# mantasu/face-crop-plus

Measured on AMD Instinct MI355X. Metric: faces/sec end-to-end (detect+align+crop), higher is better.
Workload: dtype f16x3; 1 GPU; RetinaFace detect + 5-pt align/crop, batch=32/GPU synthetic 1024x1024 RGB, strategy=largest, det_threshold=0.6, output 256x256, detector on 2 HIP streams x 16 images; global_batch=32, image_size=1024, parallelism=dp1

## Files before the change

### face-crop-plus_amd/_native.py

```python
from __future__ import annotations

import ctypes as C
import os

_HERE = os.path.dirname(os.path.abspath(__file__))
LIB_PATH = os.path.join(_HERE, "csrc", "libfcp_hip.so")
ABI_VERSION = 15

c_f32p = C.c_void_p
_lib = None


class ConvDesc(C.Structure):
    _fields_ = [
        ("in_", C.c_void_p), ("w", C.c_void_p), ("bias", C.c_void_p), ("out", C.c_void_p),
        ("res1", C.c_void_p), ("res2", C.c_void_p), ("wscale", C.c_void_p), ("in2", C.c_void_p),
        ("n", C.c_int32), ("in_h", C.c_int32), ("in_w", C.c_int32),
        ("cin", C.c_int32), ("in_ld", C.c_int32), ("in_up2", C.c_int32),
        ("cout", C.c_int32), ("kh", C.c_int32), ("kw", C.c_int32),
        ("stride", C.c_int32), ("pad", C.c_int32),
        ("out_h", C.c_int32), ("out_w", C.c_int32), ("out_ld", C.c_int32),
        ("tile_n", C.c_int32), ("cin4", C.c_int32),
        ("act_slope", C.c_float), ("alpha", C.c_float), ("alpha2", C.c_float),
        ("res1_pre", C.c_int32), ("res1_ld", C.c_int32), ("res1_h", C.c_int32),
        ("res1_w", C.c_int32), ("res2_ld", C.c_int32), ("precision", C.c_int32),
        ("in_fmt", C.c_int32), ("out_fmt", C.c_int32), ("res1_fmt", C.c_int32), ("res2_fmt", C.c_int32),
        ("tile_m", C.c_int32), ("cin2", C.c_int32), ("in2_ld", C.c_int32), ("in2_h", C.c_int32),
        ("in2_w", C.c_int32), ("in2_stride", C.c_int32), ("flags", C.c_int32), ("cu_budget", C.c_int32),
        ("band_top", C.c_int32), ("band_bottom", C.c_int32),
    ]


CONV_FLAT_ADDR = 1
CONV_BALANCE_TAIL = 2
CHAIN_OUT_EVEN_ONLY = 1


class ChainDesc(C.Structure):
    _fields_ = [(k, C.c_void_p) for k in ("t1", "w2", "ws2", "b2", "w3", "ws3", "b3", "res", "out", "w1n", "ws1n",
                                          "b1n", "t1n", "t1b")] + \
               [(k, C.c_int32) for k in ("n", "h", "w", "c", "cn", "t1_ld", "res_ld", "out_ld", "t1n_ld", "nout", "tile_m", "flags",
                                         "cb", "t1b_ld", "t1b_h", "t1b_w", "t1b_stride")]


_P, _I, _F, _L = C.c_void_p, C.c_int, C.c_float, C.c_int64
SIGNATURES = {
    "fcp_conv2d_nhwc_f32": [C.POINTER(ConvDesc), _P],
    "fcp_bottleneck_chain_f16x3": [C.POINTER(ChainDesc), _P],
    "fcp_u8_to_nhwc4_f32": [_P, _P, _L, C.POINTER(C.c_float), _F, _P],
    "fcp_f32nchw_to_nhwc4_f32": [_P, _P, _I, _I, _I, C.POINTER(C.c_float), _F, _P],
    "fcp_maxpool3x3s2_nhwc_f32": [_P, _P, _I, _I, _I, _I, _I, _I, _I, _P],
    "fcp_maxpool3x3s2_split32": [_P, _P, _I, _I, _I, _I, _I, _I, _I, _P],
    "fcp_stem7x7s2_relu_pool_u8": [_P, _I, _I, _I, C.POINTER(C.c_int32), _P, _P, _P, _P, _I, _I, _P],
    "fcp_stem7x7s2_relu_pool_conv1_u8": [_P, _I, _I, _I, C.POINTER(C.c_int32), _P, _P, _P, _P, _I, _I, _P, _P, _P, _P, _I, _P],
    "fcp_stem7x7s2_relu_pool_f32": [_P, _I, _I, _I, _P, _P, _P, _P, _I, _I, _P],
    "fcp_f32_to_split32": [_P, _P, _L, _I, _P],
    "fcp_split32_to_f32": [_P, _P, _L, _I, _P],
    "fcp_absmax_nhwc": [_P, _L, _I, _I, _I, _P, _P],
    "fcp_retina_decode": [_P, _P, _P, _I, _I, _I, _F, _F, _F, _P, _P, _P, _P, _P, _P, _P, _P, _P],
    "fcp_retina_nms_select": [_P, _P, _P, _I, _I, _F, _I, _P, _P, _P, _P, _P, _P],
    "fcp_retina_gather_faces": [_P, _P, _P, _I, _I, _P, _I, _P, _P, _P, _P],
    "fcp_estimate_transform": [_P, _P, _I, _I, _I, _P, _P, _P],
    "fcp_estimate_transform_counted": [_P, _P, _I, _I, _I, _P, _P, _P, _P, _P],
    "fcp_bise_preprocess_u8": [_P, _I, _I, _I, _P, _I, _I, C.POINTER(C.c_float), C.POINTER(C.c_float), _P],
    "fcp_avgpool_nhwc_f32": [_P, _I, _I, _I, _I, _P, _P],
    "fcp_fc_f32": [_P, _P, _P, _P, _I, _I, _I, _I, _P, _P],
    "fcp_scale_add_nhwc_f32": [_P, _I, _P, _P, _P, _I, _I, _I, _I, _P, _I, _P],
    "fcp_parse_tail": [_P, _I, _I, _I, _I, _I, _I, _I, _I, _I, _P, _P, _P],
    "fcp_label_mask_u8": [_P, _L, C.c_uint32, _P, _P],
    "fcp_bicubic_down4_u8": [_P, _I, _I, _I, _P, _P],
    "fcp_warp_affine_u8": [_P, _I, _I, _I, _P, _P, _P, _P, _I, _I, _I, _I, _P, _P],
    "fcp_warp_affine_u8_float": [_P, _I, _I, _I, _P, _P, _P, _P, _I, _I, _I, _I, _P, _P],
    "fcp_build_batch_u8": [_P, _L, _P, _P, _I, _I, _I, _I, _P, _P],
    "fcp_warp_affine_u8_ragged": [_P, _L, _P, _P, _P, _P, _I, _I, _I, _I, _P, _P],
    "fcp_warp_affine_u8_float_ragged": [_P, _L, _P, _P, _P, _P, _I, _I, _I, _I, _P, _P],
    "fcp_resize_area_ragged_u8": [_P, _L, _P, _P, _I, _P, _L, _P],
    "fcp_warp_affine_u8_interp": [_P, _I, _I, _I, _P, _P, _P, _P, _I, _I, _I, _I, _I, _P, _P],
    "fcp_warp_affine_u8_interp_ragged": [_P, _L, _P, _P, _P, _P, _I, _I, _I, _I, _I, _P, _P],
    "fcp_warp_interp_weights": [_I, _P],
    "fcp_crop_sharpness_u8": [_P, _I, _I, _I, _P, _P, _P],
    "fcp_jpeg_encode_u8": [_P, _I, _I, _I, _I, _I, _I, _P, _L, _L, _P, _P, _L, _P],
    "fcp_jpeg_encode_ex_u8": [_P, _I, _I, _I, _I, _I, _I, _I, _P, _L, _L, _P, _P, _P, _L, _P],
    "fcp_jpeg_huffman_tables": [_P, _I, _P, _P, _P],
    "fcp_png_encode_u8": [_P, _I, _I, _I, _I, _P, _L, _L, _P, _P, _L, _P],
    "fcp_png_huffman_lengths": [_P, _I, _P, _P, _P],
    "fcp_matte_u8": [_P, _P, _I, _I, _I, C.c_uint32, _I, _I, _I, _I, _P, _P, _P],
    "fcp_clahe_u8": [_P, _I, _I, _I, _I, C.c_double, _P, _P, _P],
    "fcp_matte_blur_u8": [_P, _P, _I, _I, _I, C.c_uint32, _I, _P, _I, _P, _P, _P, _L, _P],
    "fcp_matte_refine_u8": [_P, _P, _I, _I, _I, C.c_uint32, _I, _I, _P, _P, _L, _P],
    "fcp_matte_alpha_u8": [_P, _P, _I, _I, _I, _I, _I, _I, _P, _P],
    "fcp_matte_blur_alpha_u8": [_P, _P, _P, _I, _I, _I, C.c_uint32, _P, _I, _P, _P, _L, _P],
    "fcp_subject_mask_u8": [_P, _I, _I, _I, C.c_uint32, _I, _I, _P, _P, _L, _P],
    "fcp_feather_alpha_u8": [_P, _I, _I, _I, C.c_uint32, _I, _P, _P],
    "fcp_cutout_u8": [_P, _P, _I, _I, _I, _I, _I, _I, _I, _P, _I, _P, _P, _L, _P],
    "fcp_mask_shift_u8": [_P, _I, _I, _I, C.c_uint32, _I, _P, _P],
    "fcp_nlm_denoise_u8": [_P, _I, _I, _I, _P, _I, _I, _P, _P],
    "fcp_unsharp_u8": [_P, _I, _I, _I, _P, _I, _I, _I, _P, _P],
    "fcp_matte_image_u8": [_P, _P, _I, _I, _I, C.c_uint32, _I, _P, _I, _P, _P, _P, _P],
    "fcp_matte_image_alpha_u8": [_P, _P, _I, _I, _I, _P, _I, _P, _P, _P],
    "fcp_cutout_image_u8": [_P, _P, _I, _I, _I, _P, _I, _P, _P, _I, _P, _P, _L, _P],
}
EXPORTS = ["fcp_abi_version", "fcp_last_error", "fcp_retina_nms_workspace_bytes", "fcp_jpeg_workspace_bytes",
           "fcp_jpeg_workspace_bytes_ex", "fcp_matte_blur_workspace_bytes", "fcp_matte_refine_workspace_bytes",
           "fcp_subject_mask_workspace_bytes", "fcp_png_workspace_bytes", "fcp_cutout_workspace_bytes"] + list(SIGNATURES)


def lib():
    global _lib
    if _lib is not None:
        return _lib
    if not os.path.isfile(LIB_PATH):
        raise RuntimeError(
            f"HIP extension not built: {LIB_PATH} is missing. Run "
            f"`python face-crop-plus_amd/build_native.py` (needs hipcc). There is no CPU fallback.")
    l = C.CDLL(LIB_PATH)
    l.fcp_abi_version.restype = C.c_int
    l.fcp_last_error.restype = C.c_char_p
    if l.fcp_abi_version() != ABI_VERSION:
        raise RuntimeError(f"libfcp_hip.so ABI {l.fcp_abi_version()} != expected {ABI_VERSION}; rebuild")
    l.fcp_retina_nms_workspace_bytes.argtypes = [C.c_int, C.c_int]
    l.fcp_retina_nms_workspace_bytes.restype = C.c_int64
    l.fcp_jpeg_workspace_bytes.argtypes = [C.c_int, C.c_int, C.c_int, C.c_int]
    l.fcp_jpeg_workspace_bytes.restype = C.c_int64
    l.fcp_jpeg_workspace_bytes_ex.argtypes = [C.c_int] * 6
    l.fcp_jpeg_workspace_bytes_ex.restype = C.c_int64
    l.fcp_png_workspace_bytes.argtypes = [C.c_int, C.c_int, C.c_int, C.c_int]
    l.fcp_png_workspace_bytes.restype = C.c_int64
    l.fcp_matte_blur_workspace_bytes.argtypes = [C.c_int, C.c_int, C.c_int]
    l.fcp_matte_blur_workspace_bytes.restype = C.c_int64
    l.fcp_matte_refine_workspace_bytes.argtypes = [C.c_int, C.c_int, C.c_int]
    l.fcp_matte_refine_workspace_bytes.restype = C.c_int64
    l.fcp_subject_mask_workspace_bytes.argtypes = [C.c_int, C.c_int, C.c_int]
    l.fcp_subject_mask_workspace_bytes.restype = C.c_int64
    l.fcp_cutout_workspace_bytes.argtypes = [C.c_int, C.c_int, C.c_int]
    l.fcp_cutout_workspace_bytes.restype = C.c_int64
    for name, args in SIGNATURES.items():
        fn = getattr(l, name)
        fn.argtypes = args
        fn.restype = C.c_int
    _lib = l
    return l


def check(rc: int, what: str = ""):
    if rc != 0:
        msg = lib().fcp_last_error().decode(errors="replace")
        raise RuntimeError(f"{what or 'fcp_hip'} failed ({rc}): {msg}")


def stream_ptr():
    import torch
    return C.c_void_p(torch.cuda.current_stream().cuda_stream)


def ptr(t, byte_offset: int = 0):
    if t is None:
        return C.c_void_p(0)
    return C.c_void_p(t.data_ptr() + byte_offset)


def encode_slots(who: str, entry: str, pixels_dev, out, op, workspace_bytes, call):
    import torch
    assert pixels_dev.dtype == torch.uint8 and pixels_dev.is_contiguous() and pixels_dev.dim() in (3, 4)
    assert out.dtype == torch.uint8 and out.dim() == 2 and out.shape[0] == pixels_dev.shape[0]
    if op is not None:
        return op()
    f, h, w = pixels_dev.shape[:3]
    c = pixels_dev.shape[3] if pixels_dev.dim() == 4 else 1
    capacity = out.shape[1]
    if capacity and out.stride(1) != 1:
        raise RuntimeError(f"{who}: the bytes of a row of out must be contiguous")
    lengths = torch.empty((f,), dtype=torch.int32, device=pixels_dev.device)
    need = workspace_bytes(f, h, w, c)
    check(-1 if need < 0 else 0, entry)
    work = torch.empty((need,), dtype=torch.uint8, device=pixels_dev.device)
    check(call((f, h, w, c), (ptr(out) if capacity else None, out.stride(0) if f > 1 else capacity, capacity, ptr(lengths)),
               (ptr(work), need, stream_ptr())), entry)
    return lengths
```

### face-crop-plus_amd/csrc/fcp_conv.hip

```cpp
#include "fcp_conv_common.h"

#include <cstdlib>

using namespace fcp_conv;

namespace {

constexpr int LDK = 32;


template <int BN, bool CIN4, bool BUF>
__global__ void __launch_bounds__(256, (BN == 128 ? 2 : (BN == 64 ? 3 : 4))) conv_igemm_f32(const ConvK p) {
  constexpr int WAVES_N = (BN == 32) ? 1 : 2;
  constexpr int WAVES_M = 4 / WAVES_N;
  constexpr int WTM = BM / WAVES_M;
  constexpr int WTN = BN / WAVES_N;
  constexpr int TM = WTM / 32, TN = WTN / 32;
  constexpr int A_LD = BM / 32;
  constexpr int B_LD = BN / 32;

  extern __shared__ __attribute__((aligned(16))) float smem[];
  float* As = smem;
  float* Bs = smem + 2 * BM * LDK;

  const int logical = xcd_tile_order(gridDim.x, blockIdx.x);
  const int tile_n = logical % p.grid_n;
  const int tile_m = logical / p.grid_n;

  const int tid = threadIdx.x;
  const int lane = tid & 63;
  const int wave = tid >> 6;
  const int wm = wave / WAVES_N, wn = wave % WAVES_N;
  const int chunk = tid & 7;
  const int lrow = tid >> 3;

  long nbase[A_LD];
  RowPiece pc[A_LD];
  const int hw = p.out_h * p.out_w;
#pragma unroll
  for (int i = 0; i < A_LD; ++i) {
    const ConvRow r = conv_row(p, tile_m * BM + lrow + 32 * i, p.M, hw, 0u);
    nbase[i] = (long)r.ni * p.ph * p.pw;
    pc[i] = make_row_piece<CIN4>(p, r, chunk, (unsigned)(chunk * 4));
  }
  const float* wbase = p.w + (long)(tile_n * BN + lrow) * p.wrow + chunk * 4;

  __amdgpu_buffer_rsrc_t rs_in, rs_w;
  unsigned rowoff[A_LD];
  unsigned woff[B_LD];
  if (BUF) {
    rs_in = __builtin_amdgcn_make_buffer_rsrc(const_cast<float*>(p.in), 0, p.in_bytes, 0x00020000);
    rs_w = __builtin_amdgcn_make_buffer_rsrc(const_cast<float*>(p.w), 0, p.w_bytes, 0x00020000);
#pragma unroll
    for (int i = 0; i < B_LD; ++i)
      woff[i] = (unsigned)(((tile_n * BN + lrow + 32 * i) * p.wrow + chunk * 4) * 4);
  }

  f32x4 ra0[A_LD], rb0[B_LD], ra1[A_LD], rb1[B_LD];

  auto load_slice = [&](f32x4 (&ra)[A_LD], f32x4 (&rb)[B_LD], int kt, int kh_i, int kw_i, int c0) {
    if (BUF) {
#pragma unroll
      for (int i = 0; i < A_LD; ++i) {
        const unsigned vo = rowoff[i] == 0xFFFFFFFFu ? 0xFFFFFFFFu : rowoff[i] + (unsigned)(c0 * 4);
        ra[i] = buf_load16(rs_in, vo);
      }
#pragma unroll
      for (int i = 0; i < B_LD; ++i) rb[i] = buf_load16(rs_w, woff[i] + (unsigned)(kt * BK * 4));
    } else {
#pragma unroll
      for (int i = 0; i < A_LD; ++i) {
        int hi = pc[i].hi0 + kh_i;
        int wi = pc[i].wi0 + (CIN4 ? chunk : kw_i);
        const bool ok = (unsigned)hi < (unsigned)p.in_h && (unsigned)wi < (unsigned)p.in_w;
        if (p.in_up2) { hi >>= 1; wi >>= 1; }
        const long pix = nbase[i] + (long)hi * p.pw + wi;
        const float* src = CIN4 ? p.in + pix * p.in_ld : p.in + pix * p.in_ld + c0 + chunk * 4;
        ra[i] = ok ? *reinterpret_cast<const f32x4*>(src) : f32x4{0.f, 0.f, 0.f, 0.f};
      }
#pragma unroll
      for (int i = 0; i < B_LD; ++i)
        rb[i] = *reinterpret_cast<const f32x4*>(wbase + (long)(32 * i) * p.wrow + kt * BK);
    }
  };
  const int schunk = chunk ^ ((lrow >> 1) & 7);
  auto store_slice = [&](const f32x4 (&ra)[A_LD], const f32x4 (&rb)[B_LD], int buf) {
    float* a = As + buf * BM * LDK + lrow * LDK + schunk * 4;
    float* b = Bs + buf * BN * LDK + lrow * LDK + schunk * 4;
#pragma unroll
    for (int i = 0; i < A_LD; ++i) *reinterpret_cast<f32x4*>(a + 32 * i * LDK) = ra[i];
#pragma unroll
    for (int i = 0; i < B_LD; ++i) *reinterpret_cast<f32x4*>(b + 32 * i * LDK) = rb[i];
  };

  f32x16 acc[TM][TN];
  clear_acc(acc);

  TapWalk tw;
  auto advance = [&]() {
    if (BUF) next_tap<CIN4, true>(p, tw, pc, rowoff);
    else tw.advance<CIN4>(p);
  };

  const int aoff = (wm * WTM + (lane & 31)) * LDK;
  const int boff = (wn * WTN + (lane & 31)) * LDK;
  const int rsw = ((lane & 31) >> 1) & 7;
  int koff[4];
#pragma unroll
  for (int pp = 0; pp < 4; ++pp) koff[pp] = (((2 * pp + (lane >> 5)) ^ rsw)) * 4;

  auto compute = [&](int buf) {
    const float* Ab = As + buf * BM * LDK + aoff;
    const float* Bb = Bs + buf * BN * LDK + boff;
#pragma unroll
    for (int pp = 0; pp < 4; ++pp) {
      f32x4 a[TM], b[TN];
#pragma unroll
      for (int i = 0; i < TM; ++i) a[i] = *reinterpret_cast<const f32x4*>(Ab + (i * 32 * LDK + koff[pp]));
#pragma unroll
      for (int j = 0; j < TN; ++j) b[j] = *reinterpret_cast<const f32x4*>(Bb + (j * 32 * LDK + koff[pp]));
#pragma unroll
      for (int e = 0; e < 4; ++e)
#pragma unroll
        for (int i = 0; i < TM; ++i)
#pragma unroll
          for (int j = 0; j < TN; ++j)
            acc[i][j] = __builtin_amdgcn_mfma_f32_32x32x2f32(a[i][e], b[j][e], acc[i][j], 0, 0, 0);
    }
  };
  auto step = [&](int kt, f32x4 (&ra_ld)[A_LD], f32x4 (&rb_ld)[B_LD], const f32x4 (&ra_st)[A_LD],
                  const f32x4 (&rb_st)[B_LD]) {
    if (kt + 2 < p.ktiles) {
      advance();
      load_slice(ra_ld, rb_ld, kt + 2, tw.kh_i, tw.kw_i, tw.c0);
    }
    compute(kt & 1);
    if (kt + 1 < p.ktiles) store_slice(ra_st, rb_st, (kt + 1) & 1);
    __syncthreads();
  };

  if (BUF) set_tap<CIN4, true>(p, tw, pc, rowoff);
  load_slice(ra0, rb0, 0, tw.kh_i, tw.kw_i, tw.c0);
  store_slice(ra0, rb0, 0);
  if (p.ktiles > 1) {
    advance();
    load_slice(ra1, rb1, 1, tw.kh_i, tw.kw_i, tw.c0);
  }
  __syncthreads();
  for (int kt = 0; kt < p.ktiles; kt += 2) {
    step(kt, ra0, rb0, ra1, rb1);
    if (kt + 1 < p.ktiles) step(kt + 1, ra1, rb1, ra0, rb0);
  }

  conv_epilogue<BN, TM, TN, WTM, WTN>(p, acc, smem, tile_m, tile_n, tid, lane, wm, wn, hw);
}

template <int BN, bool CIN4, bool BUF>
int launch(const ConvK& k, hipStream_t s) {
  const size_t lds = (size_t)2 * (BM + BN) * LDK * sizeof(float);
  FCP_LDS_OPT_IN((&conv_igemm_f32<BN, CIN4, BUF>), lds);
  const int blocks = k.grid_m * k.grid_n;
  hipLaunchKernelGGL((conv_igemm_f32<BN, CIN4, BUF>), dim3(blocks), dim3(256), lds, s, k);
  FCP_LAUNCH_OK();
  return 0;
}

}

extern "C" int fcp_conv2d_nhwc_f32(const fcp_conv_desc* d, fcp_stream_t stream) {
  FCP_REQUIRE(d != nullptr, "conv: null descriptor");
  FCP_REQUIRE(d->in && d->w && d->out, "conv: null tensor pointer");
  FCP_REQUIRE(d->n > 0 && d->in_h > 0 && d->in_w > 0 && d->cout > 0, "conv: bad sizes");
  const bool big = d->tile_m == 256, halo = d->tile_m == 1;
  FCP_REQUIRE(d->tile_m == 0 || d->tile_m == 128 || big || halo, "conv: tile_m must be 0/128/256 (or 1: halo-tile 3x3)");
  const bool halo_wide = halo && d->tile_n != 32;
  if (halo)
    FCP_REQUIRE(d->precision == 1 && d->in_fmt == 1 && !d->cin4 && d->kh == 3 && d->kw == 3 && d->stride == 1 &&
                d->pad == 1 && d->cout <= 64 && d->cout % 8 == 0 && d->cin >= 64 && !d->in2 &&
                (!d->res1 || (d->res1_h == d->out_h && d->res1_w == d->out_w)) || halo_wide,
                "conv: the halo-tile kernel needs a 3x3 / stride 1 / pad 1 conv with cin >= 64, cout <= 64 (cout %% 8 == 0) on the "
                "fp16x3 path with a split32 input, no second source, no resized residual");
  if (halo_wide)
    FCP_REQUIRE(d->precision == 1 && d->in_fmt == 1 && !d->cin4 && d->kh == 3 && d->kw == 3 && d->stride == 1 &&
                d->pad == 1 && d->cout % 8 == 0 && d->cin >= 64 && d->cin % 64 == 0 && !d->in2 &&
                ((d->tile_n == 64 && d->cout <= 64 && (!d->res1 || (d->res1_h == d->out_h && d->res1_w == d->out_w))) ||
                 (d->tile_n == 128 && d->cout <= 128 && !d->res1 && !d->res2)),
                "conv: the wide halo-tile kernel (tile_m 1, tile_n 64 / 128) needs a 3x3 / stride 1 / pad 1 conv with cin %% 64 == 0, "
                "cout <= tile_n (cout %% 8 == 0; no residuals above 64 filters) on the fp16x3 path with a split32 input");
  FCP_REQUIRE(d->tile_n == 32 || d->tile_n == 64 || d->tile_n == 128 || (big && (d->tile_n == 256 || d->tile_n == 192)),
              "conv: tile_n must be 32/64/128 (or 192 / 256 with tile_m 256)");
  if (big)
    FCP_REQUIRE(d->precision == 1 && d->in_fmt == 1 && !d->cin4 && !d->in_up2 && d->cout % 8 == 0 && d->tile_n >= 128,
                "conv: 256-row tiles need the fp16x3 path on a split32 input (no cin4 / in_up2), cout %% 8 == 0, tile_n 128/256");
  FCP_REQUIRE(d->kh >= 1 && d->kw >= 1 && d->stride >= 1 && d->pad >= 0, "conv: bad filter geometry");
  FCP_REQUIRE(d->kh * d->kw <= 32 || d->cin4, "conv: at most 32 filter taps (kh*kw) outside cin4 mode");
  FCP_REQUIRE(d->in_ld % 4 == 0 && ((uintptr_t)d->in & 15) == 0, "conv: input must be 16-byte aligned, in_ld %% 4 == 0");
  FCP_REQUIRE(((uintptr_t)d->w & 15) == 0, "conv: filter must be 16-byte aligned");
  if (d->cin4) {
    FCP_REQUIRE(d->cin <= 4 && d->in_ld == 4 && d->kw <= 8, "conv: cin4 mode needs cin<=4, in_ld==4, kw<=8");
  } else {
    FCP_REQUIRE(d->cin % 32 == 0 && d->cin > 0, "conv: cin must be a multiple of 32 (got %d)", d->cin);
  }
  FCP_REQUIRE(d->band_top >= 0 && d->band_bottom >= 0 && d->band_top <= d->pad && d->band_bottom <= d->pad &&
              ((d->band_top | d->band_bottom) == 0 || (d->stride == 1 && !d->in2)),
              "conv: band_top / band_bottom must lie in 0..pad (stride-1 convs without a second source only)");
  const int eh = (d->in_h - d->band_top - d->band_bottom + 2 * d->pad - d->kh) / d->stride + 1;
  const int ew = (d->in_w + 2 * d->pad - d->kw) / d->stride + 1;
  FCP_REQUIRE(eh == d->out_h && ew == d->out_w, "conv: output size %dx%d does not match geometry %dx%d",
              d->out_h, d->out_w, eh, ew);
  if (d->in_up2) FCP_REQUIRE(d->in_h % 2 == 0 && d->in_w % 2 == 0, "conv: in_up2 needs even logical size");
  const long M = (long)d->n * d->out_h * d->out_w;
  FCP_REQUIRE(M < (1L << 31), "conv: too many output pixels");

  ConvK k;
  k.in = d->in; k.w = reinterpret_cast<const float*>(d->w); k.bias = d->bias; k.wscale = d->wscale; k.out = d->out; k.res1 = d->res1; k.res2 = d->res2;
  k.n = d->n; k.in_h = d->in_h; k.in_w = d->in_w;
  k.ph = d->in_up2 ? d->in_h / 2 : d->in_h;
  k.pw = d->in_up2 ? d->in_w / 2 : d->in_w;
  k.cin = d->cin; k.in_ld = d->in_ld; k.in_up2 = d->in_up2;
  k.cout = d->cout; k.kh = d->kh; k.kw = d->kw; k.stride = d->stride; k.pad = d->pad; k.pad_h = d->pad - d->band_top;
  k.out_h = d->out_h; k.out_w = d->out_w; k.out_ld = d->out_ld;
  k.M = (int)M;
  if (d->cin4) {
    k.ktiles = d->kh; k.ctiles = 1; k.wrow = d->kh * 32;
  } else {
    k.ctiles = d->cin / 32; k.ktiles = d->kh * d->kw * k.ctiles; k.wrow = d->kh * d->kw * d->cin;
  }
  k.act_slope = d->act_slope; k.alpha = d->alpha; k.alpha2 = d->alpha2;
  k.res1_pre = d->res1_pre; k.res1_ld = d->res1_ld; k.res2_ld = d->res2_ld;
  k.res1_h = d->res1_h; k.res1_w = d->res1_w;
  k.res1_resize = 0; k.res1_sh = 1.f; k.res1_sw = 1.f;
  k.in_fmt = d->in_fmt; k.out_fmt = d->out_fmt; k.res1_fmt = d->res1 ? d->res1_fmt : 0; k.res2_fmt = d->res2 ? d->res2_fmt : 0;
  const int any_split = k.in_fmt | k.out_fmt | k.res1_fmt | k.res2_fmt;
  FCP_REQUIRE((unsigned)any_split <= 1u, "conv: tensor formats must be 0 (fp32) or 1 (split32)");
  if (any_split) {
    FCP_REQUIRE(d->precision == 1, "conv: split32 tensors need precision 1 (fp16x3 kernel)");
    FCP_REQUIRE(d->cout % 8 == 0, "conv: split32 epilogue needs cout %% 8 == 0");
    FCP_REQUIRE(!k.in_fmt || (!d->cin4 && d->in_ld % 32 == 0 && ((uintptr_t)d->in & 127) == 0),
                "conv: split32 input must be a 32-channel-group aligned view (in_ld %% 32 == 0), not cin4");
    FCP_REQUIRE(!k.out_fmt || (d->out_ld % 32 == 0 && ((uintptr_t)d->out & 127) == 0 && d->cout % 32 == 0),
                "conv: split32 output must be a 32-channel-group aligned view with cout %% 32 == 0");
    FCP_REQUIRE(!k.res1_fmt || (d->res1_ld % 32 == 0 && ((uintptr_t)d->res1 & 127) == 0), "conv: misaligned split32 res1");
    FCP_REQUIRE(!k.res2_fmt || (d->res2_ld % 32 == 0 && ((uintptr_t)d->res2 & 127) == 0), "conv: misaligned split32 res2");
    FCP_REQUIRE(((uintptr_t)d->out & 15) == 0 && d->out_ld % 4 == 0 && (!d->res1 || (((uintptr_t)d->res1 & 15) == 0 && d->res1_ld % 4 == 0)) &&
                (!d->res2 || (((uintptr_t)d->res2 & 15) == 0 && d->res2_ld % 4 == 0)), "conv: 8-channel epilogue needs 16-byte aligned tensors");
  }
  if (d->res1) {
    FCP_REQUIRE(d->res1_h > 0 && d->res1_w > 0 && d->res1_ld > 0, "conv: res1 geometry missing");
    if (d->res1_h != d->out_h || d->res1_w != d->out_w) {
      k.res1_resize = 1;
      k.res1_sh = (float)d->res1_h / (float)d->out_h;
      k.res1_sw = (float)d->res1_w / (float)d->out_w;
    }
  }
  if (d->res2) FCP_REQUIRE(d->res2_ld > 0, "conv: res2_ld missing");
  k.vec_ok = (d->out_ld % 4 == 0) && (((uintptr_t)d->out & 15) == 0);
  if (d->res1) k.vec_ok = k.vec_ok && (d->res1_ld % 4 == 0) && (((uintptr_t)d->res1 & 15) == 0);
  if (d->res2) k.vec_ok = k.vec_ok && (d->res2_ld % 4 == 0) && (((uintptr_t)d->res2 & 15) == 0);
  static const int nt_env = getenv("FCP_NT_STORE") ? atoi(getenv("FCP_NT_STORE")) : 1;
  k.nt_store = nt_env;
  k.balance = (d->flags & FCP_CONV_BALANCE_TAIL) ? 1 : 0;
  k.cu_budget = d->cu_budget;
  k.mfull = 0; k.tail_rows = 0; k.round_size = 0;
  k.in2 = nullptr; k.in2_bytes = 0; k.csplit = d->cin; k.in2_ld = 0; k.ph2 = 0; k.pw2 = 0; k.stride2 = 1;
  if (d->in2) {
    FCP_REQUIRE(d->precision == 1 && d->in_fmt == 1 && !d->cin4 && !d->in_up2 && d->kh == 1 && d->kw == 1 && d->pad == 0,
                "conv: a second source needs a 1x1 / pad 0 conv on the fp16x3 path with split32 inputs");
    FCP_REQUIRE(d->cin2 > 0 && d->cin2 < d->cin && d->cin2 % 32 == 0 && d->in2_ld % 32 == 0 && d->in2_ld >= d->cin2 &&
                ((uintptr_t)d->in2 & 127) == 0, "conv: in2 must be a 32-channel-group aligned split32 view, 0 < cin2 < cin");
    FCP_REQUIRE(d->in2_stride >= 1 && d->in2_h > 0 && d->in2_w > 0 && (long)(d->out_h - 1) * d->in2_stride < d->in2_h &&
                (long)(d->out_w - 1) * d->in2_stride < d->in2_w, "conv: in2 geometry does not cover the output grid");
    const unsigned long in2_bytes = (unsigned long)d->n * d->in2_h * d->in2_w * d->in2_ld * 4ul;
    FCP_REQUIRE(in2_bytes < 0xFFFFFFF0ul, "conv: in2 must be below 4 GiB");
    k.in2 = d->in2; k.in2_bytes = (unsigned)in2_bytes; k.csplit = d->cin - d->cin2; k.in2_ld = d->in2_ld;
    k.ph2 = d->in2_h; k.pw2 = d->in2_w; k.stride2 = d->in2_stride;
  }
  k.grid_m = fcp_cdiv(M, BM);
  k.grid_n = fcp_cdiv(d->cout, d->tile_n);
  hipStream_t s = (hipStream_t)stream;
  const unsigned long in_bytes = (unsigned long)d->n * k.ph * k.pw * d->in_ld * 4ul;
  const unsigned long w_bytes = (unsigned long)(k.grid_n * d->tile_n) * k.wrow * 4ul;
  FCP_REQUIRE(!(d->flags & FCP_CONV_FLAT_ADDR) || d->precision == 0, "conv: FCP_CONV_FLAT_ADDR is a precision-0 (fp32 kernel) option");
  const bool buf = in_bytes < 0xFFFFFFF0ul && w_bytes < 0xFFFFFFF0ul && !(d->flags & FCP_CONV_FLAT_ADDR);
  FCP_REQUIRE(d->precision == 0 || d->precision == 1, "conv: precision must be 0 (fp32) or 1 (fp16x3)");
  if (d->precision == 1) {
    FCP_REQUIRE(buf, "conv: the fp16x3 path needs tensors below 4 GiB (pack this layer with precision 0)");
    FCP_REQUIRE(d->wscale != nullptr, "conv: precision 1 needs wscale");
    k.in_bytes = (unsigned)in_bytes;
    k.w_bytes = (unsigned)w_bytes;
    if (halo) {
      k.grid_n = 1;
      const unsigned long out_bytes = (unsigned long)M * d->out_ld * 4ul;
      FCP_REQUIRE(out_bytes < 0xFFFFFFF0ul, "conv(halo): the output view must span less than 4 GiB");
      FCP_REQUIRE(d->wscale != nullptr && ((uintptr_t)d->wscale & 15) == 0 && ((uintptr_t)d->bias & 15) == 0,
                  "conv(halo): wscale / bias must be 16-byte aligned");
      k.in2_bytes = (unsigned)out_bytes;
      k.w_bytes = (unsigned)((unsigned long)fcp_cdiv(d->cout, 128) * 128ul * k.wrow * 4ul);
      return halo_wide ? launch_f16x3_halo_wide(k, s) : launch_f16x3_halo(k, s);
    }
    if (big) {
      k.w_bytes = (unsigned)((unsigned long)fcp_cdiv(d->cout, 128) * 128ul * k.wrow * 4ul);
      return launch_f16x3_big(k, d->tile_n, s);
    }
    if (k.in_fmt == 1 && !d->cin4) return launch_f16x3_dma(k, d->tile_n, s);
    return launch_f16x3(k, d->tile_n, d->cin4 != 0, s);
  }
  k.in_bytes = buf ? (unsigned)in_bytes : 0u;
  k.w_bytes = buf ? (unsigned)w_bytes : 0u;
#define FCP_DISPATCH(BN_)                                                             \
  do {                                                                                \
    if (d->cin4) return buf ? launch<BN_, true, true>(k, s) : launch<BN_, true, false>(k, s); \
    return buf ? launch<BN_, false, true>(k, s) : launch<BN_, false, false>(k, s);   \
  } while (0)
  switch (d->tile_n) {
    case 32: FCP_DISPATCH(32);
    case 64: FCP_DISPATCH(64);
    default: FCP_DISPATCH(128);
  }
#undef FCP_DISPATCH
}
```

### face-crop-plus_amd/csrc/fcp_conv_common.h

```cpp
#pragma once
#include <type_traits>
#include "fcp_common.h"
#include "fcp_hip.h"

typedef float f32x16 __attribute__((ext_vector_type(16)));
typedef float f32x4 __attribute__((ext_vector_type(4)));


constexpr int FCP_AUX_A = 0;
constexpr int FCP_AUX_B = 0;

namespace fcp_conv {

constexpr int BM = 128;
constexpr int BK = 32;

struct ConvK {
  const float* in;
  const float* w;
  const float* bias;
  float* out;
  const float* res1;
  const float* res2;
  int n, in_h, in_w, ph, pw, cin, in_ld, in_up2;
// ... 264 lines not shown
    float* dst = base + pix * ld + c;
    *reinterpret_cast<u32x4_t*>(dst) = a;
    *reinterpret_cast<u32x4_t*>(dst + 4) = b;
  }
}
__device__ __forceinline__ void pack_store8(float* base, long pix, int ld, int c, int fmt, int nt, const float (&v)[8]) {
  u32x4_t a, b;
  if (fmt == 1) {
    pack8(v, 1, a, b);
    store8(base, pix, ld, c, 1, nt, a, b);
  } else {
    pack8(v, 0, a, b);
    store8(base, pix, ld, c, 0, 0, a, b);
  }
}

__device__ __forceinline__ float conv_scale_bias(float acc, float ws, float b) { return acc * ws + b; }

struct ConvEpi {
  bool res1, res1_pre, res2;
  float act_slope, alpha, alpha2;
};
template <typename E>
__device__ __forceinline__ float conv_finish(const E e, float x, float r1, float r2) {
  if (e.res1 && e.res1_pre) x += r1;
  x = x >= 0.f ? x : x * e.act_slope;
  x = x * e.alpha;
  if (e.res1 && !e.res1_pre) x += r1;
  if (e.res2) x = x * e.alpha2 + r2;
  return x;
}
template <typename E>
__device__ __forceinline__ float conv_value(const E& e, float acc, float ws, float b, float r1, float r2) {
  return conv_finish(e, conv_scale_bias(acc, ws, b), r1, r2);
}
__device__ __forceinline__ float conv_finish_relu(float x) { return conv_finish(ConvEpi{false, false, false, 0.f, 1.f, 1.f}, x, 0.f, 0.f); }
__device__ __forceinline__ float conv_finish_relu(float x, float r1) { return conv_finish(ConvEpi{true, true, false, 0.f, 1.f, 1.f}, x, r1, 0.f); }
__device__ __forceinline__ float conv_value_relu(float acc, float ws, float b) { return conv_finish_relu(conv_scale_bias(acc, ws, b)); }

__device__ __forceinline__ long res1_pixel(const ConvK& p, long m, int hw) {
  int ni, ho, wo;
  conv_out_pixel(p, m, hw, ni, ho, wo);
  int sh = (int)floorf(ho * p.res1_sh);
  int sw = (int)floorf(wo * p.res1_sw);
  sh = sh < p.res1_h - 1 ? sh : p.res1_h - 1;
  sw = sw < p.res1_w - 1 ? sw : p.res1_w - 1;
  return ((long)ni * p.res1_h + sh) * p.res1_w + sw;
}

__device__ __forceinline__ constexpr int mfma_c_row(int rr, int half) { return (rr & 3) + 8 * (rr >> 2) + 4 * half; }

template <int BN, int TM, int TN, int WTM, int WTN>
__device__ __forceinline__ void stage_acc_tile(const f32x16 (&acc)[TM][TN], float* Cs, int lane, int wm, int wn) {
  const int half = lane >> 5;
#pragma unroll
  for (int i = 0; i < TM; ++i)
#pragma unroll
    for (int j = 0; j < TN; ++j)
#pragma unroll
      for (int rr = 0; rr < 16; ++rr) {
        const int row = wm * WTM + i * 32 + mfma_c_row(rr, half);
        Cs[row * BN + wn * WTN + j * 32 + (lane & 31)] = acc[i][j][rr];
      }
  __syncthreads();
}

template <int BN, int TM, int TN, int WTM, int WTN>
__device__ __forceinline__ void conv_epilogue(const ConvK& p, f32x16 (&acc)[TM][TN], float* smem, int tile_m,
                                              int tile_n, int tid, int lane, int wm, int wn, int hw) {
  constexpr int CPR = BN / 4;
  constexpr int RPP = 256 / CPR;
  constexpr int PASSES = BM / RPP;
  float* Cs = smem;
  const int ccol = (tid % CPR) * 4;
  const int crow = tid / CPR;
  const int co = tile_n * BN + ccol;
  const bool vec = p.vec_ok && (co + 3 < p.cout);
  const long m0 = (long)tile_m * BM + crow;

  const bool pre1 = p.res1 != nullptr && !p.res1_resize && vec;
  const bool pre2 = p.res2 != nullptr && vec;
  stage_acc_tile<BN, TM, TN, WTM, WTN>(acc, Cs, lane, wm, wn);

  f32x4 bias4 = {0.f, 0.f, 0.f, 0.f}, ws4 = {1.f, 1.f, 1.f, 1.f};
  if (p.bias != nullptr) {
#pragma unroll
    for (int e = 0; e < 4; ++e)
      if (co + e < p.cout) bias4[e] = p.bias[co + e];
  }
  if (p.wscale != nullptr) {
#pragma unroll
    for (int e = 0; e < 4; ++e)
      if (co + e < p.cout) ws4[e] = p.wscale[co + e];
  }
  constexpr int EPC = PASSES < 4 ? PASSES : 4;
#pragma unroll 1
  for (int g = 0; g < PASSES; g += EPC) {
    f32x4 r1v[EPC], r2v[EPC];
    if (pre1) {
#pragma unroll
      for (int i = 0; i < EPC; ++i) {
        const long m = m0 + (long)(g + i) * RPP;
        r1v[i] = m < p.M ? *reinterpret_cast<const f32x4*>(p.res1 + m * p.res1_ld + co) : f32x4{0.f, 0.f, 0.f, 0.f};
      }
    }
    if (pre2) {
#pragma unroll
      for (int i = 0; i < EPC; ++i) {
        const long m = m0 + (long)(g + i) * RPP;
        r2v[i] = m < p.M ? *reinterpret_cast<const f32x4*>(p.res2 + m * p.res2_ld + co) : f32x4{0.f, 0.f, 0.f, 0.f};
      }
    }
#pragma unroll
    for (int i = 0; i < EPC; ++i) {
      const int row = crow + (g + i) * RPP;
      const long m = m0 + (long)(g + i) * RPP;
      if (m >= p.M || co >= p.cout) continue;
      f32x4 v = *reinterpret_cast<const f32x4*>(Cs + row * BN + ccol);
      f32x4 r1 = {0.f, 0.f, 0.f, 0.f}, r2 = {0.f, 0.f, 0.f, 0.f};
      if (pre1) {
        r1 = r1v[i];
      } else if (p.res1 != nullptr) {
        const long roff = (p.res1_resize ? res1_pixel(p, m, hw) : m) * p.res1_ld + co;
        if (vec) {
          r1 = *reinterpret_cast<const f32x4*>(p.res1 + roff);
        } else {
#pragma unroll
          for (int e = 0; e < 4; ++e)
            if (co + e < p.cout) r1[e] = p.res1[roff + e];
        }
      }
      if (pre2) {
        r2 = r2v[i];
      } else if (p.res2 != nullptr) {
#pragma unroll
        for (int e = 0; e < 4; ++e)
          if (co + e < p.cout) r2[e] = p.res2[m * p.res2_ld + co + e];
      }
#pragma unroll
      for (int e = 0; e < 4; ++e) v[e] = conv_value(p, v[e], ws4[e], bias4[e], r1[e], r2[e]);
      float* dst = p.out + m * p.out_ld + co;
      if (vec) {
        *reinterpret_cast<f32x4*>(dst) = v;
      } else {
#pragma unroll
        for (int e = 0; e < 4; ++e)
          if (co + e < p.cout) dst[e] = v[e];
      }
    }
  }
}


template <int I, int N, typename F>
__device__ __forceinline__ void fcp_static_for(F&& f) {
  if constexpr (I < N) {
    f(std::integral_constant<int, I>{});
    fcp_static_for<I + 1, N>(f);
  }
}

template <int TM, int TN, int WTM, int WTN>
__device__ __forceinline__ void conv_epilogue_regs(const ConvK& p, f32x16 (&acc)[TM][TN], int m_start, int m_end, int tm_act, int co_tile,
                                                   int co_end, int wm, int wn, int lane, int hw) {
    const int lp = lane & 15, lg = lane >> 4;
  auto swap32 = [](float& x, float& y) {
    const auto r = __builtin_amdgcn_permlane32_swap(__float_as_uint(x), __float_as_uint(y), false, false);
    const unsigned r0 = r[0], r1 = r[1];
    x = __uint_as_float(r0); y = __uint_as_float(r1);
  };
  auto swap16 = [](float& x, float& y) {
    const auto r = __builtin_amdgcn_permlane16_swap(__float_as_uint(x), __float_as_uint(y), false, false);
    const unsigned r0 = r[0], r1 = r[1];
    x = __uint_as_float(r0); y = __uint_as_float(r1);
  };
  constexpr int GI = TM < 2 ? TM : 2;
  constexpr int NGI = (TM + GI - 1) / GI;
  constexpr int NG = TN * NGI;
  u32x4_t pend_a[GI][2], pend_b[GI][2];
  auto row_of = [&](int i, int set) { return m_start + wm * WTM + i * 32 + 16 * set + lp; };
  auto chan_of = [&](int jj) { return co_tile + wn * WTN + jj * 32 + 8 * lg; };
  auto flush = [&](auto gc) {
    constexpr int g = decltype(gc)::value, jj = g / NGI, i0 = (g % NGI) * GI;
    const int co = chan_of(jj);
    fcp_static_for<0, GI>([&](auto ic) {
      constexpr int i = i0 + decltype(ic)::value;
      if constexpr (i < TM) {
        fcp_static_for<0, 2>([&](auto sc) {
          constexpr int set = decltype(sc)::value;
          const int mi = row_of(i, set);
          if (i < tm_act && mi < m_end && co < co_end) store8(p.out, mi, p.out_ld, co, p.out_fmt, 0, pend_a[i - i0][set], pend_b[i - i0][set]);
        });
      }
    });
  };
  fcp_static_for<0, NG>([&](auto gc) {
    constexpr int g = decltype(gc)::value, j = g / NGI, i0 = (g % NGI) * GI;
    const int co = chan_of(j);
    const bool cok = co < co_end;
    const int cc = cok ? co : co_tile;
    u32x4_t r1a[GI][2], r1b[GI][2];
    if (p.res1 != nullptr) {
      fcp_static_for<0, GI>([&](auto ic) {
        constexpr int i = i0 + decltype(ic)::value;
        if constexpr (i < TM) {
          fcp_static_for<0, 2>([&](auto sc) {
            constexpr int set = decltype(sc)::value;
            const int mi = row_of(i, set);
            const long m = (i < tm_act && mi < m_end && cok) ? (long)mi : (long)m_start;
            const long rpix = p.res1_resize ? res1_pixel(p, m, hw) : m;
            if (p.res1_fmt == 1) {
              const char* pb = reinterpret_cast<const char*>(p.res1) + rpix * p.res1_ld * 4 + split_chan_off(cc);
              r1a[i - i0][set] = *reinterpret_cast<const u32x4_t*>(pb);
              r1b[i - i0][set] = *reinterpret_cast<const u32x4_t*>(pb + 64);
            } else {
              r1a[i - i0][set] = *reinterpret_cast<const u32x4_t*>(p.res1 + rpix * p.res1_ld + cc);
              r1b[i - i0][set] = *reinterpret_cast<const u32x4_t*>(p.res1 + rpix * p.res1_ld + cc + 4);
            }
          });
        }
      });
    }
    __builtin_amdgcn_sched_barrier(0);
    if constexpr (g > 0) flush(std::integral_constant<int, g - 1>{});
    __builtin_amdgcn_sched_barrier(0);
    float bias8[8], ws8[8];
    {
      const f32x4 w0 = *reinterpret_cast<const f32x4*>(p.wscale + cc), w1 = *reinterpret_cast<const f32x4*>(p.wscale + cc + 4);
      f32x4 b0 = {0.f, 0.f, 0.f, 0.f}, b1 = b0;
      if (p.bias != nullptr) { b0 = *reinterpret_cast<const f32x4*>(p.bias + cc); b1 = *reinterpret_cast<const f32x4*>(p.bias + cc + 4); }
#pragma unroll
      for (int e = 0; e < 4; ++e) { ws8[e] = w0[e]; ws8[4 + e] = w1[e]; bias8[e] = b0[e]; bias8[4 + e] = b1[e]; }
    }
    fcp_static_for<0, GI>([&](auto ic) {
      constexpr int i = i0 + decltype(ic)::value;
      if constexpr (i < TM) {
        float va[8], vb[8];
        fcp_static_for<0, 4>([&](auto ec) {
          constexpr int e = decltype(ec)::value;
          float q0 = acc[i][j][e], q1 = acc[i][j][4 + e], q2 = acc[i][j][8 + e], q3 = acc[i][j][12 + e];
          swap32(q0, q1);
          swap32(q2, q3);
          swap32(q0, q2); swap16(q0, q2);
          swap32(q1, q3); swap16(q1, q3);
          va[e] = q0; va[4 + e] = q1; vb[e] = q2; vb[4 + e] = q3;
        });
        fcp_static_for<0, 2>([&](auto sc) {
          constexpr int set = decltype(sc)::value;
          float (&v)[8] = set == 0 ? va : vb;
          float r1[8], r2[8];
          if (p.res1 != nullptr) {
            if (p.res1_fmt == 1) {
              join8(r1a[i - i0][set], r1b[i - i0][set], r1);
            } else {
              const f32x4 fa = __builtin_bit_cast(f32x4, r1a[i - i0][set]), fb = __builtin_bit_cast(f32x4, r1b[i - i0][set]);
              r1[0] = fa[0]; r1[1] = fa[1]; r1[2] = fa[2]; r1[3] = fa[3]; r1[4] = fb[0]; r1[5] = fb[1]; r1[6] = fb[2]; r1[7] = fb[3];
            }
          }
          if (p.res2 != nullptr) {
            const int mi = row_of(i, set);
            load8(p.res2, (i < tm_act && mi < m_end && cok) ? (long)mi : (long)m_start, p.res2_ld, cc, p.res2_fmt, r2);
          }
#pragma unroll
          for (int e = 0; e < 8; ++e) v[e] = conv_value(p, v[e], ws8[e], bias8[e], r1[e], r2[e]);
          pack8(v, p.out_fmt, pend_a[i - i0][set], pend_b[i - i0][set]);
        });
      }
    });
  });
  flush(std::integral_constant<int, NG - 1>{});
}

template <int BN, int TM, int TN, int WTM, int WTN>
__device__ __forceinline__ void conv_epilogue8(const ConvK& p, f32x16 (&acc)[TM][TN], float* smem, int tile_m,
                                               int tile_n, int tid, int lane, int wm, int wn, int hw) {
  constexpr int CPR = BN / 8;
  constexpr int RPP = 256 / CPR;
  constexpr int PASSES = BM / RPP;
  float* Cs = smem;
  const int ccol = (tid % CPR) * 8;
  const int crow = tid / CPR;
  const int co = tile_n * BN + ccol;
  const long m0 = (long)tile_m * BM + crow;
  stage_acc_tile<BN, TM, TN, WTM, WTN>(acc, Cs, lane, wm, wn);
  if (co >= p.cout) return;
  float bias8[8], ws8[8];
#pragma unroll
  for (int e = 0; e < 8; ++e) {
    bias8[e] = p.bias != nullptr ? p.bias[co + e] : 0.f;
    ws8[e] = p.wscale != nullptr ? p.wscale[co + e] : 1.f;
  }
#pragma unroll
  for (int g = 0; g < PASSES; ++g) {
    const int row = crow + g * RPP;
    const long m = m0 + (long)g * RPP;
    if (m >= p.M) continue;
    float v[8], r1[8], r2[8];
    {
      const f32x4 a = *reinterpret_cast<const f32x4*>(Cs + row * BN + ccol);
      const f32x4 b = *reinterpret_cast<const f32x4*>(Cs + row * BN + ccol + 4);
      v[0] = a[0]; v[1] = a[1]; v[2] = a[2]; v[3] = a[3]; v[4] = b[0]; v[5] = b[1]; v[6] = b[2]; v[7] = b[3];
    }
    if (p.res1 != nullptr) load8(p.res1, p.res1_resize ? res1_pixel(p, m, hw) : m, p.res1_ld, co, p.res1_fmt, r1);
    if (p.res2 != nullptr) load8(p.res2, m, p.res2_ld, co, p.res2_fmt, r2);
#pragma unroll
    for (int e = 0; e < 8; ++e) v[e] = conv_value(p, v[e], ws8[e], bias8[e], r1[e], r2[e]);
    pack_store8(p.out, m, p.out_ld, co, p.out_fmt, p.nt_store, v);
  }
}

int launch_f16x3(const ConvK& k, int tile_n, bool cin4, hipStream_t s);
int launch_f16x3_dma(const ConvK& k, int tile_n, hipStream_t s);
int launch_f16x3_halo(const ConvK& k, hipStream_t s);
int launch_f16x3_halo_wide(const ConvK& k, hipStream_t s);
int launch_f16x3_big(const ConvK& k, int tile_n, hipStream_t s);

}
```

### face-crop-plus_amd/csrc/fcp_conv_f16x3_big.hip

```cpp
#include "fcp_conv_common.h"

#include <type_traits>

using namespace fcp_conv;

namespace {

constexpr int BMB = 256;
constexpr int NT = 512;
constexpr int ROWB = 128;
constexpr int STAGE = 1 << 16;

template <int BN>
__global__ void __launch_bounds__(NT, 1) conv_igemm_f16x3_big(const ConvK p) {
  constexpr int WAVES_N = BN == 256 ? 4 : 2;
  constexpr int WAVES_M = 8 / WAVES_N;
  constexpr int WTM = BMB / WAVES_M, WTN = BN / WAVES_N;
  constexpr int TM = WTM / 32, TN = WTN / 32;
  constexpr int A_LD = BMB / 64, B_LD = BN / 64;

  extern __shared__ __attribute__((aligned(16))) float smem[];
  char* lds = reinterpret_cast<char*>(smem);

  const int nb = p.big_tiles;
  int vb = blockIdx.x;
  int tile_n = 0, m_start = 0, m_end = 0;
  auto decode = [&](int bid) {
    const int rbase = (bid / p.round_size) * p.round_size;
    const int nr = nb - rbase < p.round_size ? nb - rbase : p.round_size;
    const int bi = bid - rbase;
    const int logical = rbase + xcd_tile_order(nr, bi);
    tile_n = logical % p.grid_n;
    const int tile_m = logical / p.grid_n;
    m_start = tile_m < p.mfull ? tile_m * BMB : p.mfull * BMB + (tile_m - p.mfull) * p.tail_rows;
    const int m_rows = tile_m < p.mfull ? BMB : p.tail_rows;
    m_end = m_start + m_rows < p.M ? m_start + m_rows : p.M;
  };
  decode(vb);

  const int tid = threadIdx.x;
  const int lane = tid & 63;
  const int wave_u = __builtin_amdgcn_readfirstlane(tid >> 6);
  const int wm = wave_u / WAVES_N, wn = wave_u % WAVES_N;
  const int lrow = tid >> 3;
  const int csrc = (tid & 7) ^ (((lrow >> 1) & 7) ^ ((lrow & 1) << 2));

  const int hw = p.out_h * p.out_w;
  RowPiece pc[A_LD];
  unsigned base2[A_LD];
  unsigned rowoff[A_LD], woff[B_LD];
  auto setup_tile = [&]() {
#pragma unroll
    for (int i = 0; i < A_LD; ++i) {
      const int m = m_start + lrow + 64 * i;
      unsigned pbase = 0;
      int hi0 = -(1 << 28), wi0 = 0;
      base2[i] = 0xFFFFFFFFu;
      if (m < m_end) {
        int ni, ho, wo;
        conv_out_pixel(p, m, hw, ni, ho, wo);
        pbase = (unsigned)(ni * p.ph * p.pw);
        hi0 = ho * p.stride - p.pad_h;
        wi0 = wo * p.stride - p.pad;
        if (p.in2 != nullptr)
          base2[i] = (((unsigned)(ni * p.ph2 + ho * p.stride2) * (unsigned)p.pw2 + (unsigned)(wo * p.stride2)) * (unsigned)p.in2_ld +
                      (unsigned)(csrc * 4)) * 4u;
      }
      pc[i].tp = make_tap_piece<false>(p, pbase, hi0, wi0, (unsigned)(csrc * 4));
    }
#pragma unroll
    for (int i = 0; i < B_LD; ++i) woff[i] = (unsigned)(((tile_n * BN + lrow + 64 * i) * p.wrow + csrc * 4) * 4);
  };
  setup_tile();
  __amdgpu_buffer_rsrc_t rs_in2 = __builtin_amdgcn_make_buffer_rsrc(const_cast<float*>(p.in2 ? p.in2 : p.in), 0, p.in2_bytes, 0x00020000);
  __amdgpu_buffer_rsrc_t rs_in = __builtin_amdgcn_make_buffer_rsrc(const_cast<float*>(p.in), 0, p.in_bytes, 0x00020000);
  __amdgpu_buffer_rsrc_t rs_w = __builtin_amdgcn_make_buffer_rsrc(const_cast<float*>(p.w), 0, p.w_bytes, 0x00020000);
  TapWalk tw;
  auto advance = [&]() { next_tap<false, false>(p, tw, pc, rowoff); };
  auto dma = [&](int kt, int stage) {
    char* a = lds + stage * STAGE + wave_u * 8 * ROWB;
    dma_slice<64>(p, rs_in, rs_in2, rs_w, a, a + BMB * ROWB, rowoff, base2, woff, tw.c0, kt);
  };

  f32x16 acc[TM][TN];

  const unsigned lds0 = (unsigned)(size_t)(__attribute__((address_space(3))) char*)lds;
  int offH[2], offL[2];
  frag_offsets(lane, offH, offL);
  const unsigned arow = lds0 + (unsigned)((wm * WTM + (lane & 31)) * ROWB);
  const unsigned brow = lds0 + (unsigned)((BMB + wn * WTN + (lane & 31)) * ROWB);
  unsigned aH[2], aL[2], bH[2], bL[2];
#pragma unroll
  for (int s = 0; s < 2; ++s) {
    aH[s] = arow + (unsigned)offH[s]; aL[s] = arow + (unsigned)offL[s];
    bH[s] = brow + (unsigned)offH[s]; bL[s] = brow + (unsigned)offL[s];
  }

  auto prefetch_tile = [&]() {
    tw = TapWalk();
    set_tap<false, false>(p, tw, pc, rowoff);
    dma(0, 0);
    if (p.ktiles > 1) {
      advance();
      dma(1, 1);
    }
  };
  prefetch_tile();
  int tm_act = 0;
  auto main_loop = [&](auto tma_c) {
    constexpr int TMA = decltype(tma_c)::value;
    f16x8 fah[2][TMA > 0 ? TMA : 1], fal[2][TMA > 0 ? TMA : 1], fbh[2][TN], fbl[2][TN];
  auto read_frags = [&](auto set_c, unsigned stage_xor) {
    constexpr int set = decltype(set_c)::value;
    fcp_static_for<0, TMA>([&](auto ic) {
      constexpr int i = decltype(ic)::value;
      fah[set][i] = lds_read128i<i * 32 * ROWB>(aH[set] ^ stage_xor);
      fal[set][i] = lds_read128i<i * 32 * ROWB>(aL[set] ^ stage_xor);
    });
    fcp_static_for<0, TN>([&](auto jc) {
      constexpr int j = decltype(jc)::value;
      fbh[set][j] = lds_read128i<j * 32 * ROWB>(bH[set] ^ stage_xor);
      fbl[set][j] = lds_read128i<j * 32 * ROWB>(bL[set] ^ stage_xor);
    });
  };
  constexpr std::integral_constant<int, 0> SET0{};
  constexpr std::integral_constant<int, 1> SET1{};
  auto mfmas_reads = [&](auto cs_c, auto ls_c, unsigned stage_xor) {
    constexpr int cs = decltype(cs_c)::value, ls = decltype(ls_c)::value;
    constexpr int NM = 3 * TMA * TN, NR = 2 * TMA + 2 * TN;
    fcp_static_for<0, NM>([&](auto mc) {
      constexpr int m = decltype(mc)::value;
      constexpr int g = m / (TMA * TN), i = (m % (TMA * TN)) / TN, j = m % TN;
      if constexpr (g == 0) acc[i][j] = __builtin_amdgcn_mfma_f32_32x32x16_f16(fbh[cs][j], fal[cs][i], acc[i][j], 0, 0, 0);
      else if constexpr (g == 1) acc[i][j] = __builtin_amdgcn_mfma_f32_32x32x16_f16(fbl[cs][j], fah[cs][i], acc[i][j], 0, 0, 0);
      else acc[i][j] = __builtin_amdgcn_mfma_f32_32x32x16_f16(fbh[cs][j], fah[cs][i], acc[i][j], 0, 0, 0);
      __builtin_amdgcn_sched_barrier(0);
      fcp_static_for<0, NR>([&](auto rc) {
        constexpr int r = decltype(rc)::value;
        if constexpr (((r + 1) * NM) / NR - 1 == m
        ) {
          if constexpr (r < 2 * TMA) {
            constexpr int ii = r / 2;
            if constexpr (r % 2 == 0) fah[ls][ii] = lds_read128i<ii * 32 * ROWB>(aH[ls] ^ stage_xor);
            else fal[ls][ii] = lds_read128i<ii * 32 * ROWB>(aL[ls] ^ stage_xor);
          } else {
            constexpr int jj = (r - 2 * TMA) / 2;
            if constexpr (r % 2 == 0) fbh[ls][jj] = lds_read128i<jj * 32 * ROWB>(bH[ls] ^ stage_xor);
            else fbl[ls][jj] = lds_read128i<jj * 32 * ROWB>(bL[ls] ^ stage_xor);
          }
          __builtin_amdgcn_sched_barrier(0);
        }
      });
    });
  };

  read_frags(SET0, 0u);
  asm volatile("s_waitcnt lgkmcnt(0)" ::: "memory");
  __builtin_amdgcn_sched_barrier(0);

  unsigned sx = 0u;
  for (int kt = 0; kt < p.ktiles; ++kt) {
    mfmas_reads(SET0, SET1, sx);
    __builtin_amdgcn_sched_barrier(0);
    asm volatile("s_waitcnt lgkmcnt(0)" ::: "memory");
    asm volatile("s_waitcnt vmcnt(0)" ::: "memory");
    __builtin_amdgcn_s_barrier();
    __builtin_amdgcn_sched_barrier(0);
    const bool dma_first = wave_u >= 4;
    if (dma_first && kt + 2 < p.ktiles) {
      advance();
      dma(kt + 2, kt & 1);
    }
    __builtin_amdgcn_sched_barrier(0);
    mfmas_reads(SET1, SET0, sx ^ (unsigned)STAGE);
    __builtin_amdgcn_sched_barrier(0);
    if (!dma_first && kt + 2 < p.ktiles) {
      advance();
      dma(kt + 2, kt & 1);
    }
    __builtin_amdgcn_sched_barrier(0);
    asm volatile("s_waitcnt lgkmcnt(0)" ::: "memory");
    __builtin_amdgcn_sched_barrier(0);
    sx ^= (unsigned)STAGE;
  }
  };
  for (;;) {
  asm volatile("s_waitcnt vmcnt(0)" ::: "memory");
  __builtin_amdgcn_s_barrier();
  __builtin_amdgcn_sched_barrier(0);
  tm_act = (m_end - m_start - wm * WTM + 31) >> 5;
  tm_act = __builtin_amdgcn_readfirstlane(tm_act < 0 ? 0 : (tm_act > TM ? TM : tm_act));
  clear_acc(acc);
  fcp_static_for<0, TM + 1>([&](auto tc) {
    if (tm_act == decltype(tc)::value) main_loop(tc);
  });
  asm volatile("s_waitcnt vmcnt(0)" ::: "memory");
  __builtin_amdgcn_s_barrier();

  const int e_tile_n = tile_n, e_m_start = m_start, e_m_end = m_end, e_tm_act = tm_act;
  const bool more = p.big_persist && vb + p.round_size < nb;
  if (more) {
    vb += p.round_size;
    decode(vb);
    setup_tile();
    prefetch_tile();
  }
  conv_epilogue_regs<TM, TN, WTM, WTN>(p, acc, e_m_start, e_m_end, e_tm_act, e_tile_n * BN,
                                       (e_tile_n + 1) * BN < p.cout ? (e_tile_n + 1) * BN : p.cout, wm, wn, lane, hw);
  if (!more) break;
  }
}

template <int BN>
int launch(ConvK k, hipStream_t s) {
  const size_t lds = 2 * (size_t)STAGE;
  FCP_LDS_OPT_IN((&conv_igemm_f16x3_big<BN>), lds);
  k.grid_n = fcp_cdiv(k.cout, BN);
  int cus = k.cu_budget > 0 ? k.cu_budget : fcp_cu_count();
  cus = cus < 8 ? 8 : (cus & ~7);
  k.round_size = cus;
  const int mt = fcp_cdiv(k.M, BMB);
  k.mfull = mt;
  k.tail_rows = BMB;
  k.grid_m = mt;
  if (k.balance) {
    const long tiles = (long)mt * k.grid_n;
    const long full_rounds = tiles / cus;
    const int mfull = (int)((full_rounds * cus) / k.grid_n);
    const long rem = (long)k.M - (long)mfull * BMB;
    if (rem > 0) {
      const long slots = cus / k.grid_n > 0 ? cus / k.grid_n : 1;
      long r = ((rem + slots - 1) / slots + 31) / 32 * 32;
      r = r < 32 ? 32 : r;
      if (r < BMB) {
        k.mfull = mfull;
        k.tail_rows = (int)r;
        k.grid_m = mfull + (int)((rem + r - 1) / r);
      }
    }
  }
  k.big_tiles = k.grid_m * k.grid_n;
  static const int persist_env = getenv("FCP_BIG_PERSIST") ? atoi(getenv("FCP_BIG_PERSIST")) : -1;
  k.big_persist = persist_env < 0 ? (k.cu_budget == 0) : (persist_env != 0);
  hipLaunchKernelGGL((conv_igemm_f16x3_big<BN>), dim3(k.big_persist && k.big_tiles > k.round_size ? k.round_size : k.big_tiles), dim3(NT), lds, s, k);
  FCP_LAUNCH_OK();
  return 0;
}

}

namespace fcp_conv {

int launch_f16x3_big(const ConvK& k, int tile_n, hipStream_t s) {
  return tile_n == 256 ? launch<256>(k, s) : tile_n == 192 ? launch<192>(k, s) : launch<128>(k, s);
}

}
```

### face-crop-plus_amd/csrc/fcp_conv_f16x3_dma.hip

```cpp
#include "fcp_conv_common.h"

using namespace fcp_conv;

namespace {

constexpr int NST = 2;

template <int BN, bool EP8>
__global__ void __launch_bounds__(256, (BN == 128 ? 2 : 3)) conv_igemm_f16x3_dma(const ConvK p) {
  constexpr int WAVES_N = (BN == 32) ? 1 : 2;
  constexpr int WAVES_M = 4 / WAVES_N;
  constexpr int WTM = BM / WAVES_M;
  constexpr int WTN = BN / WAVES_N;
  constexpr int TM = WTM / 32, TN = WTN / 32;
  constexpr int A_LD = BM / 32;
  constexpr int B_LD = BN / 32;
  constexpr int ROWB = 128;
  constexpr int STAGE = (BM + BN) * ROWB;

  extern __shared__ __attribute__((aligned(16))) float smem[];
  char* lds = reinterpret_cast<char*>(smem);

  const int logical = xcd_tile_order(gridDim.x, blockIdx.x);
  const int tile_n = logical % p.grid_n;
  const int tile_m = logical / p.grid_n;

  const int tid = threadIdx.x;
  const int lane = tid & 63;
  const int wave = tid >> 6;
  const int wave_u = __builtin_amdgcn_readfirstlane(wave);
  const int wm = wave / WAVES_N, wn = wave % WAVES_N;
  const int lrow = tid >> 3;
  const int csrc = (tid & 7) ^ (((lrow >> 1) & 7) ^ ((lrow & 1) << 2));

  const int hw = p.out_h * p.out_w;
  __amdgpu_buffer_rsrc_t rs_in = __builtin_amdgcn_make_buffer_rsrc(const_cast<float*>(p.in), 0, p.in_bytes, 0x00020000);
  __amdgpu_buffer_rsrc_t rs_w = __builtin_amdgcn_make_buffer_rsrc(const_cast<float*>(p.w), 0, p.w_bytes, 0x00020000);
  __amdgpu_buffer_rsrc_t rs_in2 = __builtin_amdgcn_make_buffer_rsrc(const_cast<float*>(p.in2 ? p.in2 : p.in), 0, p.in2_bytes, 0x00020000);
  RowPiece pc[A_LD];
  unsigned base2[A_LD], rowoff[A_LD], woff[B_LD];
#pragma unroll
  for (int i = 0; i < A_LD; ++i) {
    const ConvRow r = conv_row(p, tile_m * BM + lrow + 32 * i, p.M, hw, (unsigned)(csrc * 4));
    pc[i] = make_row_piece<false>(p, r, 0, (unsigned)(csrc * 4));
    base2[i] = r.base2;
  }
#pragma unroll
  for (int i = 0; i < B_LD; ++i) woff[i] = (unsigned)(((tile_n * BN + lrow + 32 * i) * p.wrow + csrc * 4) * 4);
  TapWalk tw;
  auto dma = [&](int kt, int stage) {
    char* a = lds + stage * STAGE + wave_u * 8 * ROWB;
    dma_slice<32>(p, rs_in, rs_in2, rs_w, a, a + BM * ROWB, rowoff, base2, woff, tw.c0, kt);
  };

  f32x16 acc[TM][TN];
  clear_acc(acc);

  const int aoff = (wm * WTM + (lane & 31)) * ROWB;
  const int boff = BM * ROWB + (wn * WTN + (lane & 31)) * ROWB;
  int offH[2], offL[2];
  frag_offsets(lane, offH, offL);

  set_tap<false, true>(p, tw, pc, rowoff);
  dma(0, 0);
  asm volatile("s_waitcnt vmcnt(0)" ::: "memory");
  __builtin_amdgcn_s_barrier();

  int stage = 0;
  const int kt_end = p.ktiles;
  for (int kt = 0; kt < kt_end; ++kt) {
    const char* Ab = lds + stage * STAGE + aoff;
    const char* Bb = lds + stage * STAGE + boff;
    f16x8 ah[2][TM], al[2][TM], bh[2][TN], bl[2][TN];
#pragma unroll
    for (int s = 0; s < 2; ++s) {
#pragma unroll
      for (int i = 0; i < TM; ++i) {
        ah[s][i] = *reinterpret_cast<const f16x8*>(Ab + i * 32 * ROWB + offH[s]);
        al[s][i] = *reinterpret_cast<const f16x8*>(Ab + i * 32 * ROWB + offL[s]);
      }
#pragma unroll
      for (int j = 0; j < TN; ++j) {
        bh[s][j] = *reinterpret_cast<const f16x8*>(Bb + j * 32 * ROWB + offH[s]);
        bl[s][j] = *reinterpret_cast<const f16x8*>(Bb + j * 32 * ROWB + offL[s]);
      }
    }
    asm volatile("s_waitcnt lgkmcnt(0)" ::: "memory");
    __builtin_amdgcn_sched_barrier(0);
    const int ahead = kt + NST - 1;
    const bool issue = ahead < p.ktiles;
    if (issue) {
      next_tap<false, true>(p, tw, pc, rowoff);
      int st = stage + NST - 1;
      if (st >= NST) st -= NST;
      dma(ahead, st);
    }
    __builtin_amdgcn_sched_barrier(0);
#pragma unroll
    for (int s = 0; s < 2; ++s)
#pragma unroll
      for (int i = 0; i < TM; ++i)
#pragma unroll
        for (int j = 0; j < TN; ++j) {
          if constexpr (EP8) {
            acc[i][j] = __builtin_amdgcn_mfma_f32_32x32x16_f16(bh[s][j], al[s][i], acc[i][j], 0, 0, 0);
            acc[i][j] = __builtin_amdgcn_mfma_f32_32x32x16_f16(bl[s][j], ah[s][i], acc[i][j], 0, 0, 0);
            acc[i][j] = __builtin_amdgcn_mfma_f32_32x32x16_f16(bh[s][j], ah[s][i], acc[i][j], 0, 0, 0);
          } else {
            acc[i][j] = __builtin_amdgcn_mfma_f32_32x32x16_f16(al[s][i], bh[s][j], acc[i][j], 0, 0, 0);
            acc[i][j] = __builtin_amdgcn_mfma_f32_32x32x16_f16(ah[s][i], bl[s][j], acc[i][j], 0, 0, 0);
            acc[i][j] = __builtin_amdgcn_mfma_f32_32x32x16_f16(ah[s][i], bh[s][j], acc[i][j], 0, 0, 0);
          }
        }
    __builtin_amdgcn_sched_barrier(0);
    asm volatile("s_waitcnt vmcnt(0)" ::: "memory");
    __builtin_amdgcn_s_barrier();
    __builtin_amdgcn_sched_barrier(0);
    if (++stage >= NST) stage = 0;
  }

  if constexpr (EP8) {
    const int m_end = (tile_m + 1) * BM < p.M ? (tile_m + 1) * BM : p.M;
    conv_epilogue_regs<TM, TN, WTM, WTN>(p, acc, tile_m * BM, m_end, TM, tile_n * BN, (tile_n + 1) * BN < p.cout ? (tile_n + 1) * BN : p.cout,
                                         wm, wn, lane, hw);
  } else {
    conv_epilogue<BN, TM, TN, WTM, WTN>(p, acc, smem, tile_m, tile_n, tid, lane, wm, wn, hw);
  }
}

template <int BN, bool EP8>
int launch_ep(const ConvK& k, hipStream_t s) {
  size_t lds = (size_t)NST * (BM + BN) * 128;
  const size_t epi = EP8 ? 0 : (size_t)BM * BN * 4;
  if (lds < epi) lds = epi;
  FCP_LDS_OPT_IN((&conv_igemm_f16x3_dma<BN, EP8>), lds);
  hipLaunchKernelGGL((conv_igemm_f16x3_dma<BN, EP8>), dim3(k.grid_m * k.grid_n), dim3(256), lds, s, k);
  FCP_LAUNCH_OK();
  return 0;
}
template <int BN>
int launch(const ConvK& k, hipStream_t s) {
  const bool ep8 = (k.out_fmt | k.res1_fmt | k.res2_fmt) != 0;
  return ep8 ? launch_ep<BN, true>(k, s) : launch_ep<BN, false>(k, s);
}

}

namespace fcp_conv {

int launch_f16x3_dma(const ConvK& k, int tile_n, hipStream_t s) {
  switch (tile_n) {
    case 32: return launch<32>(k, s);
    case 64: return launch<64>(k, s);
    default: return launch<128>(k, s);
  }
}

}
```

### face-crop-plus_amd/csrc/fcp_conv_f16x3_halo.hip

```cpp
#include "fcp_conv_common.h"

#include <type_traits>

using namespace fcp_conv;

namespace {

constexpr int TH = 8, TW = 32;
constexpr int HW_ = TW + 2;
constexpr int HROWS = 344;
constexpr int ROWB = 128;
constexpr int A_BYTES = HROWS * ROWB;
constexpr int B_BYTES = 9 * 32 * ROWB;
constexpr int B_OFF = 2 * A_BYTES;
constexpr int LDS_TOTAL = 2 * A_BYTES + 2 * B_BYTES;
constexpr int A_LD = 11;
constexpr int HALO_I = A_LD - 1;

__device__ __forceinline__ void lds_write32(unsigned addr, float v) { asm volatile("ds_write_b32 %0, %1" ::"v"(addr), "v"(v) : "memory"); }
__device__ __forceinline__ f32x4 lds_read128f(unsigned addr) {
  f32x4 v;
  asm volatile("ds_read_b128 %0, %1" : "=v"(v) : "v"(addr));
  return v;
}


struct HaloTiles {
  int tiles_x, tiles_y, ntiles, per_x, xcd, slot, slots;
  struct Next { int nit, ntile; bool more; };
  __device__ __forceinline__ HaloTiles(const ConvK& p, int nb, int bid)
      : tiles_x((p.out_w + TW - 1) / TW), tiles_y((p.out_h + TH - 1) / TH), ntiles(p.n * tiles_x * tiles_y), per_x((ntiles + 7) / 8),
        xcd(bid & 7), slot(bid >> 3), slots((nb + 7 - xcd) / 8) {}
  __device__ __forceinline__ int tile(int it) const { return xcd * per_x + it; }
  __device__ __forceinline__ bool has(int it) const { return it < per_x && tile(it) < ntiles; }
  __device__ __forceinline__ Next next(int it) const { return {it + slots, tile(it + slots), has(it + slots)}; }
  __device__ __forceinline__ void coords(int tile, int& ni, int& y0, int& x0) const {
    const int tx = tile % tiles_x;
    const int ty = (tile / tiles_x) % tiles_y;
    ni = tile / (tiles_x * tiles_y);
    y0 = ty * TH; x0 = tx * TW;
  }
};

__device__ __forceinline__ void halo_frag_addrs(unsigned (&aaddr)[4][3], unsigned lds0, int wave_u, int xl, int half) {
#pragma unroll
  for (int d = 0; d < 4; ++d)
#pragma unroll
    for (int kw = 0; kw < 3; ++kw) {
      const int hr = (2 * wave_u + d) * HW_ + xl + kw;
      aaddr[d][kw] = lds0 + (unsigned)(hr * ROWB + ((half ^ swz(hr)) << 4));
    }
}

__device__ __forceinline__ void halo_epi_consts(const ConvK& p, int ccol, bool cvalid, f32x4 (&b8)[2], f32x4 (&w8)[2]) {
  b8[0] = b8[1] = w8[0] = w8[1] = f32x4{0.f, 0.f, 0.f, 0.f};
  if (cvalid) {
    if (p.bias != nullptr) { b8[0] = *reinterpret_cast<const f32x4*>(p.bias + ccol); b8[1] = *reinterpret_cast<const f32x4*>(p.bias + ccol + 4); }
    w8[0] = *reinterpret_cast<const f32x4*>(p.wscale + ccol); w8[1] = *reinterpret_cast<const f32x4*>(p.wscale + ccol + 4);
  }
}

template <int TN>
__global__ void __launch_bounds__(512, 1) conv3x3_halo_f16x3(const ConvK p) {
  extern __shared__ __attribute__((aligned(16))) float smem[];
  char* lds = reinterpret_cast<char*>(smem);
  const unsigned lds0 = (unsigned)(size_t)(__attribute__((address_space(3))) char*)lds;

  const HaloTiles ts(p, gridDim.x, blockIdx.x);

  const int lane = threadIdx.x & 63;
  const int wave8 = __builtin_amdgcn_readfirstlane(threadIdx.x >> 6);
  const bool loader = wave8 >= 4;
  const int wave_u = wave8 & 3;
  const int tid = threadIdx.x & 255;
  const int nslices = p.ctiles;
  const int nblocks = nslices * TN;

  int it = ts.slot;
  if (!ts.has(it)) return;

  if (loader) {
    const int lrow = tid >> 3;
    const int csrc = (tid & 7) ^ swz(lrow);
    __amdgpu_buffer_rsrc_t rs_in = __builtin_amdgcn_make_buffer_rsrc(const_cast<float*>(p.in), 0, p.in_bytes, 0x00020000);
    __amdgpu_buffer_rsrc_t rs_w = __builtin_amdgcn_make_buffer_rsrc(const_cast<float*>(p.w), 0, p.w_bytes, 0x00020000);
    const unsigned wbase = (unsigned)((lrow * p.wrow) * 4 + csrc * 16);
    unsigned abase[A_LD];
    int hyx[A_LD];
#pragma unroll
    for (int i = 0; i < A_LD; ++i) {
      const int hr = lrow + 32 * i;
      const int hy = hr / HW_, hx = hr - hy * HW_;
      hyx[i] = hr < (TH + 2) * HW_ ? (hy << 8 | hx) : -1;
    }
    auto tile_setup = [&](int tile) {
      int ni, y0, x0;
      ts.coords(tile, ni, y0, x0);
#pragma unroll
      for (int i = 0; i < A_LD; ++i) {
        const int y = y0 - p.pad_h + (hyx[i] >> 8), x = x0 - 1 + (hyx[i] & 255);
        const bool ok = hyx[i] >= 0 && (unsigned)y < (unsigned)p.in_h && (unsigned)x < (unsigned)p.in_w;
        const int yp = p.in_up2 ? y >> 1 : y, xp = p.in_up2 ? x >> 1 : x;
        abase[i] = ok ? ((unsigned)((ni * p.ph + yp) * p.pw + xp) * (unsigned)p.in_ld + (unsigned)(csrc * 4)) * 4u : 0xFFFFFFFFu;
      }
    };
    auto dma_halo = [&](int cs, int stage) {
      char* a = lds + stage * A_BYTES + wave_u * 8 * ROWB;
#pragma unroll
      for (int i = 0; i < A_LD - 1; ++i) {
        const unsigned ro = abase[i];
        __builtin_amdgcn_raw_ptr_buffer_load_lds(rs_in, (__attribute__((address_space(3))) void*)(a + 32 * i * ROWB), 16,
                                                 (int)(ro == 0xFFFFFFFFu ? 0xFFFFFFFFu : ro + (unsigned)(cs * 128)), 0, 0, 0);
      }
      if (wave_u < 3) {
        const unsigned ro = abase[A_LD - 1];
        __builtin_amdgcn_raw_ptr_buffer_load_lds(rs_in, (__attribute__((address_space(3))) void*)(a + 32 * (A_LD - 1) * ROWB), 16,
                                                 (int)(ro == 0xFFFFFFFFu ? 0xFFFFFFFFu : ro + (unsigned)(cs * 128)), 0, 0, 0);
      }
    };
    auto dma_filter = [&](int blk, int buf) {
      const int cs = blk / TN, pass = blk - cs * TN;
      char* b = (lds + wave_u * 8 * ROWB) + B_OFF + buf * B_BYTES;
      const unsigned wo = wbase + (unsigned)(pass * 32 * p.wrow * 4 + cs * 9 * 128);
#pragma unroll
      for (int t = 0; t < 9; ++t)
        __builtin_amdgcn_raw_ptr_buffer_load_lds(rs_w, (__attribute__((address_space(3))) void*)(b + 32 * t * ROWB), 16,
                                                 (int)(wo + (unsigned)(t * 128)), 0, 0, 0);
    };

    tile_setup(ts.tile(it));
    dma_halo(0, 0);
    dma_filter(0, 0);
    dma_halo(1, 1);
    dma_filter(1, 1);
    int blk = 0;
    unsigned bbuf = 0, astage = 0;
    asm volatile("s_waitcnt vmcnt(0)" ::: "memory");
    __builtin_amdgcn_s_barrier();
    for (;;) {
      const bool new_slice = TN == 1 || (blk & 1) != 0;
      const int cs = blk / TN;
      const bool last_of_tile = blk == nblocks - 1;
      const HaloTiles::Next nx = ts.next(it);
      asm volatile("s_waitcnt vmcnt(0)" ::: "memory");
      __builtin_amdgcn_s_barrier();
      bool halo_delayed = false;
      const int b2 = blk + 2;
      if (b2 < nblocks) dma_filter(b2, (int)bbuf);
      else if (nx.more) dma_filter(b2 - nblocks, (int)bbuf);
      if (new_slice) {
        const int s2 = cs + 2;
        if (s2 < nslices) dma_halo(s2, (int)astage);
        else if (nx.more) {
          if (s2 == nslices) {
            tile_setup(nx.ntile);
            dma_halo(0, (int)astage);
          } else {
            halo_delayed = true;
          }
        }
      }
      const unsigned freed = astage;
      bbuf ^= 1u;
      if (new_slice) astage ^= 1u;
      ++blk;
      if (new_slice && last_of_tile) {
        __builtin_amdgcn_s_barrier();
        if (!nx.more) return;
        if (halo_delayed) dma_halo(1, (int)freed);
        it = nx.nit;
        blk = 0;
      }
    }
  }

  const int xl = lane & 31, half = lane >> 5;
  unsigned aaddr[4][3];
  halo_frag_addrs(aaddr, lds0, wave_u, xl, half);
  const unsigned baddr0 = lds0 + (unsigned)(B_OFF + xl * ROWB + ((half ^ swz(xl)) << 4));

  f16x8 fah[2][2], fal[2][2], fbh[2], fbl[2];

  auto read_one = [&](auto tap_c, auto idx_c, unsigned aoff, unsigned boff) {
    constexpr int tap = decltype(tap_c)::value, idx = decltype(idx_c)::value;
    constexpr int kh = tap / 3, kw = tap % 3;
    constexpr int s = idx / 6, r = idx % 6;
    if constexpr (r == 0) fbh[s] = lds_read128i<tap * 4096>((baddr0 + boff) ^ (unsigned)(s ? 0x20 : 0));
    else if constexpr (r == 3) fbl[s] = lds_read128i<tap * 4096>((baddr0 + boff) ^ (unsigned)(s ? 0x60 : 0x40));
    else {
      constexpr int i = (r == 1 || r == 4) ? 0 : 1;
      constexpr bool lo = r < 3;
      const unsigned a = (aaddr[i + kh][kw] + aoff) ^ (unsigned)((lo ? 0x40 : 0) | (s ? 0x20 : 0));
      if constexpr (lo) fal[i][s] = lds_read128i<0>(a);
      else fah[i][s] = lds_read128i<0>(a);
    }
  };

  __amdgpu_buffer_rsrc_t rs_out = __builtin_amdgcn_make_buffer_rsrc(p.out, 0, p.in2_bytes, 0x00020000);

  int e_ni = 0, e_y0 = 0, e_x0 = 0;
  ts.coords(ts.tile(it), e_ni, e_y0, e_x0);

  f32x16 acc[TN][2];
  clear_acc(acc);

  __builtin_amdgcn_s_barrier();
  __builtin_amdgcn_sched_barrier(0);

  fcp_static_for<0, 12>([&](auto ic) { read_one(std::integral_constant<int, 0>{}, ic, 0u, 0u); });

  auto tap_step = [&](auto tap_c, auto pass_c, unsigned aoff_n, unsigned boff_n) {
    constexpr int tap = decltype(tap_c)::value, pass = decltype(pass_c)::value;
    constexpr int ntap = (tap + 1) % 9;
    fcp_static_for<0, 2>([&](auto sc) {
      constexpr int s = decltype(sc)::value;
      asm volatile("s_waitcnt lgkmcnt(6)" ::: "memory");
      __builtin_amdgcn_sched_barrier(0);
      auto rd = [&](auto rc) {
        read_one(std::integral_constant<int, ntap>{}, std::integral_constant<int, 6 * s + decltype(rc)::value>{}, aoff_n, boff_n);
        __builtin_amdgcn_sched_barrier(0);
      };
      auto mm = [&](int i, const f16x8& a, const f16x8& b) {
        acc[pass][i] = __builtin_amdgcn_mfma_f32_32x32x16_f16(a, b, acc[pass][i], 0, 0, 0);
        __builtin_amdgcn_sched_barrier(0);
      };
      mm(0, fal[0][s], fbh[s]); rd(std::integral_constant<int, 1>{});
      mm(1, fal[1][s], fbh[s]); rd(std::integral_constant<int, 2>{});
      mm(0, fah[0][s], fbl[s]);
      mm(1, fah[1][s], fbl[s]); rd(std::integral_constant<int, 3>{});
      mm(0, fah[0][s], fbh[s]); rd(std::integral_constant<int, 4>{});
      mm(1, fah[1][s], fbh[s]); rd(std::integral_constant<int, 5>{}); rd(std::integral_constant<int, 0>{});
    });
  };

  auto epilogue = [&](int stage) {
    const unsigned cs0 = lds0 + (unsigned)(stage * A_BYTES + wave_u * 64 * 128);
    const int eq = lane & 3, er = lane >> 2;
#pragma unroll
    for (int n = 0; n < TN; ++n) {
      const int ccol = n * 32 + eq * 8;
      const bool cvalid = ccol < p.cout;
      f32x4 b8[2], w8[2];
      halo_epi_consts(p, ccol, cvalid, b8, w8);
#pragma unroll
      for (int i = 0; i < 2; ++i)
#pragma unroll
        for (int rr = 0; rr < 16; ++rr) {
          const int row = i * 32 + mfma_c_row(rr, half);
          lds_write32(cs0 + (unsigned)((row * 32 + xl) * 4), acc[n][i][rr]);
        }
      __builtin_amdgcn_sched_barrier(0);
#pragma unroll
      for (int gp = 0; gp < 2; ++gp) {
        f32x4 va[2], vb[2];
#pragma unroll
        for (int g = 0; g < 2; ++g) {
          const unsigned ra = cs0 + (unsigned)(((er + 16 * (2 * gp + g)) * 32 + eq * 8) * 4);
          va[g] = lds_read128f(ra);
          vb[g] = lds_read128f(ra + 16);
        }
        asm volatile("s_waitcnt lgkmcnt(0)" ::: "memory");
        __builtin_amdgcn_sched_barrier(0);
#pragma unroll
        for (int g = 0; g < 2; ++g) {
          const int row = wave_u * 64 + er + 16 * (2 * gp + g);
          const int y = e_y0 + (row >> 5), x = e_x0 + (row & 31);
          const bool ok = cvalid && y < p.out_h && x < p.out_w;
          const long m = ok ? ((long)e_ni * p.out_h + y) * p.out_w + x : 0;
          float v[8] = {va[g][0], va[g][1], va[g][2], va[g][3], vb[g][0], vb[g][1], vb[g][2], vb[g][3]};
          float r1[8], r2[8];
          if (p.res1 != nullptr) load8(p.res1, m, p.res1_ld, cvalid ? ccol : 0, p.res1_fmt, r1);
          if (p.res2 != nullptr) load8(p.res2, m, p.res2_ld, cvalid ? ccol : 0, p.res2_fmt, r2);
#pragma unroll
          for (int e = 0; e < 8; ++e) v[e] = conv_value(p, v[e], w8[e >> 2][e & 3], b8[e >> 2][e & 3], r1[e], r2[e]);
          u32x4_t s0, s1;
          unsigned o0, o1;
          if (p.out_fmt == 1) {
            pack8(v, 1, s0, s1);
            o0 = (unsigned)(m * p.out_ld * 4 + split_chan_off(ccol));
            o1 = o0 + 64u;
          } else {
            pack8(v, 0, s0, s1);
            o0 = (unsigned)((m * p.out_ld + ccol) * 4);
            o1 = o0 + 16u;
          }
          __builtin_amdgcn_raw_buffer_store_b128(s0, rs_out, ok ? o0 : 0xFFFFFFFFu, 0, 0);
          __builtin_amdgcn_raw_buffer_store_b128(s1, rs_out, ok ? o1 : 0xFFFFFFFFu, 0, 0);
        }
      }
      __builtin_amdgcn_sched_barrier(0);
    }
    __builtin_amdgcn_s_barrier();
    __builtin_amdgcn_sched_barrier(0);
  };

  int blk = 0;
  unsigned bbuf = 0, astage = 0;
  auto run_block = [&](auto pass_c) -> bool {
    constexpr int pass = decltype(pass_c)::value;
    constexpr bool new_slice = pass == TN - 1;
    const unsigned aoff = astage * (unsigned)A_BYTES, boff = bbuf * (unsigned)B_BYTES;
    const bool last_of_tile = blk == nblocks - 1;
    const HaloTiles::Next nx = ts.next(it);
    fcp_static_for<0, 8>([&](auto tc) { tap_step(tc, pass_c, aoff, boff); });
    asm volatile("s_waitcnt lgkmcnt(0)" ::: "memory");
    __builtin_amdgcn_s_barrier();
    __builtin_amdgcn_sched_barrier(0);
    const unsigned aoff_next = new_slice ? (astage ^ 1u) * (unsigned)A_BYTES : aoff;
    const unsigned boff_next = (bbuf ^ 1u) * (unsigned)B_BYTES;
    tap_step(std::integral_constant<int, 8>{}, pass_c, aoff_next, boff_next);
    const unsigned freed = astage;
    bbuf ^= 1u;
    if constexpr (new_slice) astage ^= 1u;
    ++blk;
    if constexpr (new_slice) {
      if (last_of_tile) {
        __builtin_amdgcn_sched_barrier(0);
        epilogue((int)freed);
        if (!nx.more) return true;
        it = nx.nit;
        blk = 0;
        ts.coords(nx.ntile, e_ni, e_y0, e_x0);
        clear_acc(acc);
      }
    }
    return false;
  };
  for (;;) {
    if constexpr (TN == 2) {
      if (run_block(std::integral_constant<int, 0>{})) break;
      if (run_block(std::integral_constant<int, 1>{})) break;
    } else {
      if (run_block(std::integral_constant<int, 0>{})) break;
    }
  }
}


template <int TN, bool RES, int BT, int RS>
__global__ void __launch_bounds__(512, 1) conv3x3_halo_wide_f16x3(const ConvK p) {
  constexpr int TAPB = TN * 32 * ROWB;
  constexpr int PRE = RS - BT;
  constexpr bool SLACK2 = (RS - BT - 1) / BT >= 2;
  static_assert(18 % BT == 0 && 18 % RS == 2 && (RS & (RS - 1)) == 0 && PRE >= BT + 1, "block / ring geometry");
  extern __shared__ __attribute__((aligned(16))) float smem[];
  char* lds = reinterpret_cast<char*>(smem);
  const unsigned lds0 = (unsigned)(size_t)(__attribute__((address_space(3))) char*)lds;

  const HaloTiles ts(p, gridDim.x, blockIdx.x);

  const int lane = threadIdx.x & 63;
  const int wave8 = __builtin_amdgcn_readfirstlane(threadIdx.x >> 6);
  const bool loader = wave8 >= 4;
  const int wave_u = wave8 & 3;
  const int tid = threadIdx.x & 255;
  const int nslices = p.ctiles;
  const int T = 9 * nslices;

  int it = ts.slot;
  if (!ts.has(it)) return;

  if (loader) {
    const int lrow = tid >> 3;
    const int csrc = (tid & 7) ^ swz(lrow);
    __amdgpu_buffer_rsrc_t rs_in = __builtin_amdgcn_make_buffer_rsrc(const_cast<float*>(p.in), 0, p.in_bytes, 0x00020000);
    __amdgpu_buffer_rsrc_t rs_w = __builtin_amdgcn_make_buffer_rsrc(const_cast<float*>(p.w), 0, p.w_bytes, 0x00020000);
    const unsigned wbase = (unsigned)((lrow * p.wrow) * 4 + csrc * 16);
    unsigned abase[A_LD];
    int hyx[A_LD];
#pragma unroll
    for (int i = 0; i < A_LD; ++i) {
      const int hr = lrow + 32 * i;
      const int hy = hr / HW_, hx = hr - hy * HW_;
      hyx[i] = hr < (TH + 2) * HW_ ? (hy << 8 | hx) : -1;
    }
    auto tile_setup = [&](int tile) {
      int ni, y0, x0;
      ts.coords(tile, ni, y0, x0);
#pragma unroll
      for (int i = 0; i < A_LD; ++i) {
        const int y = y0 - p.pad_h + (hyx[i] >> 8), x = x0 - 1 + (hyx[i] & 255);
        const bool ok = hyx[i] >= 0 && (unsigned)y < (unsigned)p.in_h && (unsigned)x < (unsigned)p.in_w;
        const int yp = p.in_up2 ? y >> 1 : y, xp = p.in_up2 ? x >> 1 : x;
        abase[i] = ok ? ((unsigned)((ni * p.ph + yp) * p.pw + xp) * (unsigned)p.in_ld + (unsigned)(csrc * 4)) * 4u : 0xFFFFFFFFu;
      }
    };
    auto dma_halo = [&](int cs, int stage) {
      char* a = lds + stage * A_BYTES + wave_u * 8 * ROWB;
#pragma unroll
      for (int i = 0; i < A_LD - 1; ++i) {
        const unsigned ro = abase[i];
        __builtin_amdgcn_raw_ptr_buffer_load_lds(rs_in, (__attribute__((address_space(3))) void*)(a + 32 * i * ROWB), 16,
                                                 (int)(ro == 0xFFFFFFFFu ? 0xFFFFFFFFu : ro + (unsigned)(cs * 128)), 0, 0, 0);
      }
      if (wave_u < 3) {
        const unsigned ro = abase[A_LD - 1];
        __builtin_amdgcn_raw_ptr_buffer_load_lds(rs_in, (__attribute__((address_space(3))) void*)(a + 32 * (A_LD - 1) * ROWB), 16,
                                                 (int)(ro == 0xFFFFFFFFu ? 0xFFFFFFFFu : ro + (unsigned)(cs * 128)), 0, 0, 0);
      }
    };
    auto dma_tap = [&](int gt, int rs) {
      const int cs = gt / 9, tap = gt - cs * 9;
      char* b = (lds + wave_u * 8 * ROWB) + B_OFF + rs * TAPB;
      const unsigned wo = wbase + (unsigned)(cs * 9 * 128 + tap * 128);
#pragma unroll
      for (int k = 0; k < TN; ++k)
        __builtin_amdgcn_raw_ptr_buffer_load_lds(rs_w, (__attribute__((address_space(3))) void*)(b + 32 * k * ROWB), 16,
                                                 (int)(wo + (unsigned)(k * 32 * p.wrow * 4)), 0, 0, 0);
    };

    tile_setup(ts.tile(it));
    dma_halo(0, 0);
    dma_halo(1, 1);
#pragma unroll
    for (int e = 0; e < PRE; ++e) dma_tap(e, e);
    int g = 0;
    unsigned G = 0;
    int pend = 0;
    asm volatile("s_waitcnt vmcnt(0)" ::: "memory");
    __builtin_amdgcn_s_barrier();
    for (;;) {
      const HaloTiles::Next nx = ts.next(it);
      if constexpr (SLACK2) {
        if (pend >= BT * TN + HALO_I) asm volatile("s_waitcnt vmcnt(%0)" ::"n"(BT * TN + HALO_I) : "memory");
        else if (pend >= BT * TN) asm volatile("s_waitcnt vmcnt(%0)" ::"n"(BT * TN) : "memory");
        else asm volatile("s_waitcnt vmcnt(0)" ::: "memory");
      } else {
        asm volatile("s_waitcnt vmcnt(0)" ::: "memory");
      }
      __builtin_amdgcn_s_barrier();
      pend = 0;
#pragma unroll
      for (int e = 0; e < BT; ++e) {
        const int ta = g + PRE + e;
        if (ta < T) { dma_tap(ta, (int)((G + (unsigned)(PRE + e)) & (unsigned)(RS - 1))); pend += TN; }
        else if (nx.more) { dma_tap(ta - T, (int)((G + (unsigned)(PRE + e)) & (unsigned)(RS - 1))); pend += TN; }
      }
      const int t8 = (g / 9) * 9 - 1;
      if (t8 >= 0 && t8 >= g - BT) {
        const int died = t8 / 9, s2 = died + 2, stage = died & 1;
        if (s2 < nslices) { dma_halo(s2, stage); pend += HALO_I; }
        else if (nx.more) {
          tile_setup(nx.ntile);
          dma_halo(0, stage);
          pend += HALO_I;
        }
      }
      g += BT; G += (unsigned)BT;
      if (g == T) {
        __builtin_amdgcn_s_barrier();
        if (!nx.more) return;
        dma_halo(1, 1);
        pend += HALO_I;
        it = nx.nit;
        g = 0;
      }
    }
  }

  const int xl = lane & 31, half = lane >> 5;
  unsigned aaddr[4][3];
  auto make_aaddr = [&]() {
    int xo = xl;
    asm volatile("" : "+v"(xo));
    halo_frag_addrs(aaddr, lds0, wave_u, xo, half);
  };
  make_aaddr();
  unsigned bslot[RS];
#pragma unroll
  for (int k = 0; k < RS; ++k) bslot[k] = lds0 + (unsigned)(B_OFF + k * TAPB + xl * ROWB + ((half ^ swz(xl)) << 4));

  f16x8 fah[2][2], fal[2][2], fbh[2], fbl[2];

  auto read_a = [&](auto tap_c, auto s_c, auto i_c, auto lo_c, auto aoff_c) {
    constexpr int tap = decltype(tap_c)::value, sk = decltype(s_c)::value, i = decltype(i_c)::value;
    constexpr bool lo = decltype(lo_c)::value != 0;
    constexpr int kh = tap / 3, kw = tap % 3;
    const unsigned a = aaddr[i + kh][kw] ^ (unsigned)((lo ? 0x40 : 0) | (sk ? 0x20 : 0));
    if constexpr (lo) fal[sk][i] = lds_read128i<decltype(aoff_c)::value>(a);
    else fah[sk][i] = lds_read128i<decltype(aoff_c)::value>(a);
  };
  auto read_b = [&](unsigned base, auto j_c, auto s_c, auto lo_c, auto set_c) {
    constexpr int j = decltype(j_c)::value, sk = decltype(s_c)::value, set = decltype(set_c)::value;
    constexpr bool lo = decltype(lo_c)::value != 0;
    const unsigned b = base ^ (unsigned)((lo ? 0x40 : 0) | (sk ? 0x20 : 0));
    if constexpr (lo) fbl[set] = lds_read128i<j * 4096>(b);
    else fbh[set] = lds_read128i<j * 4096>(b);
  };

  __amdgpu_buffer_rsrc_t rs_out = __builtin_amdgcn_make_buffer_rsrc(p.out, 0, p.in2_bytes, 0x00020000);

  f32x16 acc[TN][2];
  clear_acc(acc);

  __builtin_amdgcn_s_barrier();
  __builtin_amdgcn_sched_barrier(0);

  using I0 = std::integral_constant<int, 0>;
  using I1 = std::integral_constant<int, 1>;
  auto first_frags = [&]() {
    read_a(I0{}, I0{}, I0{}, I1{}, I0{}); read_a(I0{}, I0{}, I1{}, I1{}, I0{});
    read_a(I0{}, I0{}, I0{}, I0{}, I0{}); read_a(I0{}, I0{}, I1{}, I0{}, I0{});
    read_b(bslot[0], I0{}, I0{}, I0{}, I0{}); read_b(bslot[0], I0{}, I0{}, I1{}, I0{});
  };
  first_frags();

  auto tap_step = [&](auto first_c, auto tap_c, auto aoff_x, unsigned bx, auto ntap_c, auto aoff_n, unsigned bn) {
    if constexpr (decltype(first_c)::value != 0) {
      __builtin_amdgcn_s_barrier();
      __builtin_amdgcn_sched_barrier(0);
    }
    fcp_static_for<0, 2>([&](auto sc) {
      constexpr int s = decltype(sc)::value;
      fcp_static_for<0, TN>([&](auto jc) {
        constexpr int j = decltype(jc)::value;
        constexpr int gi = s * TN + j, set = gi & 1, nset = set ^ 1;
        if constexpr (j == 1 || (j == 2 && TN == 4)) asm volatile("s_waitcnt lgkmcnt(2)" ::: "memory");
        else asm volatile("s_waitcnt lgkmcnt(0)" ::: "memory");
        __builtin_amdgcn_sched_barrier(0);
        auto mm = [&](int i, const f16x8& a, const f16x8& b) {
          acc[j][i] = __builtin_amdgcn_mfma_f32_32x32x16_f16(a, b, acc[j][i], 0, 0, 0);
          __builtin_amdgcn_sched_barrier(0);
        };
        auto rd_b = [&](auto lo_c) {
          if constexpr (j + 1 < TN) read_b(bx, std::integral_constant<int, j + 1>{}, sc, lo_c, std::integral_constant<int, nset>{});
          else if constexpr (s == 0) read_b(bx, I0{}, I1{}, lo_c, std::integral_constant<int, nset>{});
          else read_b(bn, I0{}, I0{}, lo_c, std::integral_constant<int, nset>{});
          __builtin_amdgcn_sched_barrier(0);
        };
        auto rd_a = [&](auto idx_c) {
          constexpr int idx = decltype(idx_c)::value;
          if constexpr (idx < 4) {
            using IC = std::integral_constant<int, idx & 1>;
            using LO = std::integral_constant<int, idx < 2 ? 1 : 0>;
            if constexpr (s == 0) read_a(tap_c, I1{}, IC{}, LO{}, aoff_x);
            else read_a(ntap_c, I0{}, IC{}, LO{}, aoff_n);
            __builtin_amdgcn_sched_barrier(0);
          }
        };
        mm(0, fal[s][0], fbh[set]); rd_b(I0{});
        mm(1, fal[s][1], fbh[set]); rd_b(I1{});
        mm(0, fah[s][0], fbl[set]); rd_a(std::integral_constant<int, j < 2 ? 2 * j : 4>{});
        mm(1, fah[s][1], fbl[set]); rd_a(std::integral_constant<int, j < 2 ? 2 * j + 1 : 4>{});
        mm(0, fah[s][0], fbh[set]);
        mm(1, fah[s][1], fbh[set]);
      });
    });
  };

  auto epilogue = [&]() {
    int e_ni, e_y0, e_x0;
    ts.coords(ts.tile(it), e_ni, e_y0, e_x0);
    const unsigned cs0 = lds0 + (unsigned)(A_BYTES + wave_u * 64 * 128);
    const int eq = lane & 3, er = lane >> 2;
    asm volatile("s_waitcnt lgkmcnt(0)" ::: "memory");
#pragma unroll
    for (int n = 0; n < TN; ++n) {
      asm volatile("" ::: "memory");
      __builtin_amdgcn_sched_barrier(0);
      const int ccol = n * 32 + eq * 8;
      const bool cvalid = ccol < p.cout;
      f32x4 b8[2], w8[2];
      halo_epi_consts(p, ccol, cvalid, b8, w8);
#pragma unroll
      for (int i = 0; i < 2; ++i)
#pragma unroll
        for (int rr = 0; rr < 16; ++rr) {
          const int row = i * 32 + mfma_c_row(rr, half);
          lds_write32(cs0 + (unsigned)((row * 32 + xl) * 4), acc[n][i][rr]);
        }
      __builtin_amdgcn_sched_barrier(0);
#pragma unroll
      for (int gp = 0; gp < (RES ? 2 : 4); ++gp) {
        constexpr int GN = RES ? 2 : 1;
        f32x4 va[GN], vb[GN];
#pragma unroll
        for (int g = 0; g < GN; ++g) {
          const unsigned ra = cs0 + (unsigned)(((er + 16 * (GN * gp + g)) * 32 + eq * 8) * 4);
          va[g] = lds_read128f(ra);
          vb[g] = lds_read128f(ra + 16);
        }
        asm volatile("s_waitcnt lgkmcnt(0)" ::: "memory");
        __builtin_amdgcn_sched_barrier(0);
#pragma unroll
        for (int g = 0; g < GN; ++g) {
          const int row = wave_u * 64 + er + 16 * (GN * gp + g);
          const int y = e_y0 + (row >> 5), x = e_x0 + (row & 31);
          const bool ok = cvalid && y < p.out_h && x < p.out_w;
          const long m = ok ? ((long)e_ni * p.out_h + y) * p.out_w + x : 0;
          float v[8] = {va[g][0], va[g][1], va[g][2], va[g][3], vb[g][0], vb[g][1], vb[g][2], vb[g][3]};
          if constexpr (RES) {
            float r1[8], r2[8];
            if (p.res1 != nullptr) load8(p.res1, m, p.res1_ld, cvalid ? ccol : 0, p.res1_fmt, r1);
            if (p.res2 != nullptr) load8(p.res2, m, p.res2_ld, cvalid ? ccol : 0, p.res2_fmt, r2);
#pragma unroll
            for (int e = 0; e < 8; ++e) v[e] = conv_value(p, v[e], w8[e >> 2][e & 3], b8[e >> 2][e & 3], r1[e], r2[e]);
          } else {
            const ConvEpi plain{false, false, false, p.act_slope, p.alpha, 1.f};
#pragma unroll
            for (int e = 0; e < 8; ++e) v[e] = conv_value(plain, v[e], w8[e >> 2][e & 3], b8[e >> 2][e & 3], 0.f, 0.f);
          }
          u32x4_t s0, s1;
          unsigned o0, o1;
          if (p.out_fmt == 1) {
            pack8(v, 1, s0, s1);
            o0 = (unsigned)(m * p.out_ld * 4 + split_chan_off(ccol));
            o1 = o0 + 64u;
          } else {
            pack8(v, 0, s0, s1);
            o0 = (unsigned)((m * p.out_ld + ccol) * 4);
            o1 = o0 + 16u;
          }
          __builtin_amdgcn_raw_buffer_store_b128(s0, rs_out, ok ? o0 : 0xFFFFFFFFu, 0, 0);
          __builtin_amdgcn_raw_buffer_store_b128(s1, rs_out, ok ? o1 : 0xFFFFFFFFu, 0, 0);
        }
      }
      __builtin_amdgcn_sched_barrier(0);
    }
    __builtin_amdgcn_s_barrier();
    __builtin_amdgcn_sched_barrier(0);
  };

  int unit = 0;
  const int nunits = nslices / 2;
  for (;;) {
    if (unit != 0 || it != ts.slot) make_aaddr();
    fcp_static_for<0, 18>([&](auto tc) {
      constexpr int t = decltype(tc)::value, tn = (t + 1) % 18;
      using OX = std::integral_constant<int, (t / 9) * A_BYTES>;
      using ON = std::integral_constant<int, (tn / 9) * A_BYTES>;
      tap_step(std::integral_constant<int, t % BT == 0 ? 1 : 0>{}, std::integral_constant<int, t % 9>{}, OX{}, bslot[t % RS],
               std::integral_constant<int, tn % 9>{}, ON{}, bslot[(t + 1) % RS]);
    });
    {
      const unsigned b0 = bslot[0], b1 = bslot[1];
      fcp_static_for<0, RS - 2>([&](auto kc) { bslot[decltype(kc)::value] = bslot[decltype(kc)::value + 2]; });
      bslot[RS - 2] = b0; bslot[RS - 1] = b1;
    }
    if (++unit == nunits) {
      const HaloTiles::Next nx = ts.next(it);
      __builtin_amdgcn_sched_barrier(0);
      epilogue();
      if (!nx.more) break;
      it = nx.nit;
      unit = 0;
      clear_acc(acc);
      first_frags();
    }
  }
}

}

namespace fcp_conv {

static int halo_grid(const ConvK& k, unsigned* grid) {
  const long tiles = (long)k.n * ((k.out_h + TH - 1) / TH) * ((k.out_w + TW - 1) / TW);
  FCP_REQUIRE(tiles < (1L << 31), "conv(halo): too many tiles");
  const int cus = fcp_cu_count();
  *grid = (unsigned)(tiles < cus ? tiles : cus);
  return 0;
}

int launch_f16x3_halo(const ConvK& k, hipStream_t s) {
  const size_t lds = (size_t)LDS_TOTAL;
  unsigned grid = 0;
  if (const int e = halo_grid(k, &grid)) return e;
  if (k.cout <= 32) {
    FCP_LDS_OPT_IN(&conv3x3_halo_f16x3<1>, lds);
    hipLaunchKernelGGL(conv3x3_halo_f16x3<1>, dim3(grid), dim3(512), lds, s, k);
  } else {
    FCP_LDS_OPT_IN(&conv3x3_halo_f16x3<2>, lds);
    hipLaunchKernelGGL(conv3x3_halo_f16x3<2>, dim3(grid), dim3(512), lds, s, k);
  }
  FCP_LAUNCH_OK();
  return 0;
}

constexpr int WIDE2_BT = 2;

int launch_f16x3_halo_wide(const ConvK& k, hipStream_t s) {
  const int tn = k.cout <= 64 ? 2 : 4;
  const size_t lds = (size_t)(2 * A_BYTES + (tn == 2 ? 8 : 4) * tn * 32 * ROWB);
  unsigned grid = 0;
  if (const int e = halo_grid(k, &grid)) return e;
  FCP_REQUIRE(k.ctiles >= 2 && k.ctiles % 2 == 0 && k.cout <= 128, "conv(halo, wide): cin must be a multiple of 64, cout <= 128");
  FCP_REQUIRE(tn == 2 || (k.res1 == nullptr && k.res2 == nullptr), "conv(halo, wide): no residual inputs with more than 64 filters");
  if (tn == 2) {
    FCP_LDS_OPT_IN((&conv3x3_halo_wide_f16x3<2, true, WIDE2_BT, 8>), lds);
    hipLaunchKernelGGL((conv3x3_halo_wide_f16x3<2, true, WIDE2_BT, 8>), dim3(grid), dim3(512), lds, s, k);
  } else {
    FCP_LDS_OPT_IN((&conv3x3_halo_wide_f16x3<4, false, 1, 4>), lds);
    hipLaunchKernelGGL((conv3x3_halo_wide_f16x3<4, false, 1, 4>), dim3(grid), dim3(512), lds, s, k);
  }
  FCP_LAUNCH_OK();
  return 0;
}

}
```

### face-crop-plus_amd/engine.py

```python
from __future__ import annotations

import contextlib
import ctypes as C
import os
import threading
from dataclasses import dataclass

import numpy as np
import torch

from . import _native as N
from . import torch_ops as T

BN_EPS = 1e-5
COUT_PAD = 128


class Act:
    __slots__ = ("buf", "c0", "c", "fmt")

    def __init__(self, buf: torch.Tensor, c0: int = 0, c: int | None = None, fmt: int = 0):
        assert buf.dim() == 4 and buf.dtype == torch.float32 and buf.is_contiguous()
        self.buf, self.c0, self.fmt = buf, c0, fmt
        self.c = buf.shape[3] - c0 if c is None else c
# ... 388 lines not shown
                    e1.synchronize()
                    best_t = min(best_t, e0.elapsed_time(e1) / 2)
                times.append(best_t)
            tmin = min(times)
            best = next(c for c, t in zip(candidates, times) if t <= 1.02 * tmin)
            if os.environ.get("FCP_AUTOTUNE_LOG"):
                print("autotune", key, {str(c): round(t * 1e3, 1) for c, t in zip(candidates, times)}, "->", best, flush=True)
            cls.cache[key] = best
            cls._disk_dirty = True
        if os.environ.get("FCP_TUNE_CACHE") != "0":
            cls._save_soon()
        return best

    _last_save = 0.0
    _atexit = False

    @classmethod
    def _save_soon(cls):
        import time
        if not cls._atexit:
            import atexit
            cls._atexit = True
            atexit.register(cls._save_quietly)
        if time.monotonic() - cls._last_save >= 2.0:
            cls._save_quietly()

    @classmethod
    def _save_quietly(cls):
        import time
        if not cls._disk_dirty or os.environ.get("FCP_TUNE_CACHE") == "0":
            return
        try:
            cls.save()
        except Exception:
            pass
        cls._last_save = time.monotonic()


class ConvStats:
    timing = None
    replay = None


class RangeMonitor:
    active = None
    LIMIT = 32768.0

    def __init__(self):
        self.rows = []

    def __enter__(self):
        assert RangeMonitor.active is None, "RangeMonitor is not re-entrant"
        RangeMonitor.active = self
        return self

    def __exit__(self, *exc):
        RangeMonitor.active = None

    def see(self, label: str, t: Act):
        m = torch.zeros((), dtype=torch.float32, device=t.buf.device)
        N.check(N.lib().fcp_absmax_nhwc(t.ptr(), t.n * t.h * t.w, t.c, t.ld, t.fmt, N.ptr(m), N.stream_ptr()), "fcp_absmax_nhwc")
        self.rows.append((label, m))

    def report(self):
        return [(label, float(m.item())) for label, m in self.rows]

    def check(self, what: str):
        rep = self.report()
        bad = [(label, v) for label, v in rep if not v < self.LIMIT]
        if bad:
            worst = max(bad, key=lambda r: r[1])
            raise FloatingPointError(
                f"{what}: activations leave the range of the fp16x3 (split binary16) conv path: |x| reaches {worst[1]:.4g} "
                f"after '{worst[0]}' ({len(bad)} of {len(rep)} launches at or above 2^15 = {self.LIMIT:.0f}; binary16 "
                f"saturates at 65504).  Load the model with precision='f32' (exact fp32 MFMA path) for these weights.")
        return rep


def selfcheck_mode(weights) -> bool:
    mode = os.environ.get("FCP_SELFCHECK", "auto")
    from_checkpoint = weights is None or (isinstance(weights, str) and weights != "generated")
    return mode == "1" or (mode == "auto" and from_checkpoint)


SELFCHECK_HARD_TOL = 1e-2


def selfcheck_compare(what: str, got: torch.Tensor, ref: torch.Tensor, rel_tol: float) -> float:
    scale = float(ref.abs().max().item())
    diff = float((got - ref).abs().max().item()) / max(scale, 1e-30)
    if not diff <= rel_tol:
        msg = (f"{what}: the fp16x3 path and the exact-fp32 path disagree by {diff:.3g} of the output's "
               f"largest value (tolerance {rel_tol:g}, hard limit {SELFCHECK_HARD_TOL:g}) with these weights; load with precision='f32'.")
        if os.environ.get("FCP_SELFCHECK", "auto") == "1" or not diff <= SELFCHECK_HARD_TOL:
            raise FloatingPointError(msg)
        import warnings
        warnings.warn(msg)
    return diff


def selfcheck_at_load(model, sd, weights, precision, repack_f32):
    if model.precision != 1 or not selfcheck_mode(weights):
        return
    try:
        model.selfcheck(sd)
    except FloatingPointError as e:
        if precision is not None or os.environ.get("FCP_SELFCHECK", "auto") == "1":
            raise
        import warnings
        warnings.warn(f"{e}  Falling back to precision='f32' for this model.", RuntimeWarning)
        repack_f32()
        model.selfcheck_report = {"fallback": "f32", "reason": str(e)}


def _c_launch(fn: str, *args):
    N.check(getattr(N.lib(), fn)(*args, N.stream_ptr()), fn)


def _filter(pc: PackedConv | None):
    return (None, None, None) if pc is None else (pc.w, pc.wscale, pc.bias)


def _alias_safe_out(out: Act, *ins: Act | None) -> Act:
    st = out.buf.untyped_storage().data_ptr()
    if any(t is not None and t.buf.untyped_storage().data_ptr() == st and t.c0 < out.c0 + out.c and out.c0 < t.c0 + t.c
           for t in ins):
        return Act.empty(out.n, out.h, out.w, out.c, out.buf.device, out.fmt)
    return out


def _accounted(go, describe, relaunch):
    timing, replay = ConvStats.timing, ConvStats.replay
    if timing is not None:
        e0, e1 = torch.cuda.Event(enable_timing=True), torch.cuda.Event(enable_timing=True)
        e0.record()
    outs = go()
    if timing is None and replay is None and RangeMonitor.active is None:
        return outs
    label, mon_label, flops, byts = describe()
    if timing is not None:
        e1.record()
        timing.append((e0, e1, flops, label, byts))
    if replay is not None:
        fn, args, keep = relaunch(*outs)
        replay.append((label, flops, byts, lambda keep=keep: _c_launch(fn, *args)))
    mon = RangeMonitor.active
    if mon is not None:
        for i, t in enumerate(outs):
            if t is not None and t.c % 8 == 0:
                mon.see(mon_label if i == 0 else f"{mon_label} [output {i}]", t)
    return outs


def _conv_desc(pc: PackedConv, x: Act, out: Act, x2, x2_stride, res1, res1_pre, res2, alpha, alpha2, act_slope, in_up2, band,
               tile_m, tile_n, flags, cu_budget) -> N.ConvDesc:
    in_h, in_w = (x.h * 2, x.w * 2) if in_up2 else (x.h, x.w)
    d = N.ConvDesc()
    d.in_, d.w, d.out = x.ptr(), N.ptr(pc.w), out.ptr()
    if x2 is not None:
        d.in2, d.cin2, d.in2_ld, d.in2_h, d.in2_w, d.in2_stride = x2.ptr(), x2.c, x2.ld, x2.h, x2.w, x2_stride
    d.bias = N.ptr(pc.bias)
    d.wscale = N.ptr(pc.wscale)
    d.precision = pc.precision
    d.in_fmt, d.out_fmt = x.fmt, out.fmt
    d.res1_fmt = res1.fmt if res1 is not None else 0
    d.res2_fmt = res2.fmt if res2 is not None else 0
    d.res1 = res1.ptr() if res1 is not None else None
    d.res2 = res2.ptr() if res2 is not None else None
    d.n, d.in_h, d.in_w = x.n, in_h, in_w
    d.cin, d.in_ld, d.in_up2 = pc.cin, x.ld, int(in_up2)
    d.cout, d.kh, d.kw, d.stride, d.pad = pc.cout, pc.kh, pc.kw, pc.stride, pc.pad
    d.out_h, d.out_w, d.out_ld = out.h, out.w, out.ld
    d.tile_m, d.tile_n = tile_m, tile_n
    d.cin4 = int(pc.cin4)
    d.act_slope, d.alpha, d.alpha2 = act_slope, alpha, alpha2
    d.res1_pre = int(res1_pre)
    d.flags = flags
    d.cu_budget = cu_budget
    d.band_top, d.band_bottom = band
    if res1 is not None:
        d.res1_ld, d.res1_h, d.res1_w = res1.ld, res1.h, res1.w
    if res2 is not None:
        d.res2_ld = res2.ld
    return d


def conv(pc: PackedConv, x: Act, out: Act | None = None, *, act_slope: float = 1.0,
         alpha: float = 1.0, res1: Act | None = None, res1_pre: bool = True,
         res2: Act | None = None, alpha2: float = 1.0, in_up2: bool = False,
         tile_n: int | None = None, out_fmt: int = 0, tile_m: int | None = None,
         x2: Act | None = None, x2_stride: int = 1, flat: bool = False, balance_tail: bool = False,
         band: tuple[int, int] = (0, 0)) -> Act:
    assert x.c + (x2.c if x2 is not None else 0) == pc.cin, f"conv expects {pc.cin} input channels, got {x.c}"
    in_h, in_w = (x.h * 2, x.w * 2) if in_up2 else (x.h, x.w)
    oh = (in_h - band[0] - band[1] + 2 * pc.pad - pc.kh) // pc.stride + 1
    ow = (in_w + 2 * pc.pad - pc.kw) // pc.stride + 1
    if out is None:
        out = Act.empty(x.n, oh, ow, pc.cout, x.buf.device, out_fmt)
    assert (out.n, out.h, out.w, out.c) == (x.n, oh, ow, pc.cout), "conv: bad output view"
    if (x.fmt or out.fmt or (res1 is not None and res1.fmt) or (res2 is not None and res2.fmt)) and pc.precision != 1:
        raise ValueError("split32 tensors can only be used with filters packed for the fp16x3 path")
    assert x2 is None or (x2.fmt == 1 and x.fmt == 1 and x2.n == x.n), "two-source convs take split32 tensors"
    assert res1 is None or (res1.c == pc.cout and res1.n == x.n)
    assert res2 is None or (res2.n, res2.h, res2.w, res2.c) == (x.n, oh, ow, pc.cout)
    m = x.n * oh * ow
    tm, tn = tile_m or 128, tile_n or _pick_tile_n(pc.cout, m)
    flags = (N.CONV_FLAT_ADDR if flat else 0) | (N.CONV_BALANCE_TAIL if balance_tail else 0)
    cu = getattr(_budget, "cus", 0)
    desc = lambda o: _conv_desc(pc, x, o, x2, x2_stride, res1, res1_pre, res2, alpha, alpha2, act_slope, in_up2, band,
                                tm, tn, flags, cu)
    big_ok = (pc.precision == 1 and x.fmt == 1 and not pc.cin4 and not in_up2 and pc.cout % 8 == 0
              and pc.cout >= 128 and m >= 256 * 64)
    halo_ok = (pc.precision == 1 and x.fmt == 1 and not pc.cin4 and (pc.kh, pc.kw, pc.stride, pc.pad) == (3, 3, 1, 1)
               and pc.cout <= 64 and pc.cout % 8 == 0 and pc.cin >= 64 and x2 is None and (res1 is None or (res1.h, res1.w) == (oh, ow)))
    wide_ok = (pc.precision == 1 and x.fmt == 1 and not pc.cin4 and (pc.kh, pc.kw, pc.stride, pc.pad) == (3, 3, 1, 1)
               and pc.cout % 8 == 0 and pc.cin % 64 == 0 and x2 is None and 64 < pc.cout <= 128 and res1 is None and res2 is None)
    if tile_n is None and tile_m is None and (pc.cout > 64 or halo_ok):
        key = (pc.cin, pc.cout, pc.kh, pc.kw, pc.stride, m, int(in_up2), res1 is not None, res2 is not None,
               pc.precision, x.fmt, out.fmt, None if x2 is None else (x2.c, x2_stride), cu)
        best = Autotune.choose(key, tile_candidates(pc.cout, halo_ok, wide_ok, big_ok),
                               lambda: desc(_alias_safe_out(out, x, x2, res1, res2)))
        if best is not None:
            tm, tn = best[0], best[1]
            flags |= best[2] if len(best) > 2 else 0

    def go():
        if T.ENABLED:
            T.load().conv2d_out(x.buf, x.c0, pc.cin, pc.w, pc.bias, pc.wscale, None if res1 is None else res1.buf,
                                0 if res1 is None else res1.c0, None if res2 is None else res2.buf, 0 if res2 is None else res2.c0,
                                out.buf, out.c0, pc.cout, pc.kh, pc.kw, pc.stride, pc.pad, float(act_slope), float(alpha),
                                float(alpha2), bool(res1_pre), pc.precision, x.fmt, out.fmt, 0 if res1 is None else res1.fmt,
                                0 if res2 is None else res2.fmt, bool(in_up2), bool(pc.cin4), int(tm), int(tn),
                                None if x2 is None else x2.buf, 0 if x2 is None else x2.c0, 0 if x2 is None else x2.c,
                                int(x2_stride), int(flags), int(cu), int(band[0]), int(band[1]))
        else:
            _c_launch("fcp_conv2d_nhwc_f32", C.byref(desc(out)))
        return (out,)

    def describe():
        byts = 4 * (m * (pc.cout + (pc.cout if res1 is not None else 0) + (pc.cout if res2 is not None else 0))
                    + x.n * in_h * in_w * x.c // (4 if in_up2 else 1) + (m * x2.c if x2 is not None else 0)
                    + pc.cout * pc.cin * pc.kh * pc.kw)
        head = f"conv {pc.kh}x{pc.kw} s{pc.stride} {pc.cin}->{pc.cout} @{oh}x{ow}"
        return (f"{head} tile {tm}x{tn}{' bal' if flags & N.CONV_BALANCE_TAIL else ''}{' +res' if res1 is not None else ''}",
                head, pc.flops_per_pixel * m, byts)

    def relaunch(o):
        o = _alias_safe_out(o, x, x2, res1, res2)
        return "fcp_conv2d_nhwc_f32", (C.byref(desc(o)),), (pc, x, x2, res1, res2, o)
    return _accounted(go, describe, relaunch)[0]


def tile_candidates(cout: int, halo_ok: bool, wide_ok: bool, big_ok: bool):
    cands = [(128, 128), (128, 64)]
    if halo_ok:
        cands = ([(128, 32)] if cout <= 32 else []) + [(128, 64), (1, 32)]
    if wide_ok:
        cands = cands + [(1, 128)]
    if big_ok:
        big = [(256, 128)] + ([(256, 256)] if cout >= 256 else []) + ([(256, 192)] if 128 < cout <= 192 else [])
        cands += big
        cands += [(tm, tn, N.CONV_BALANCE_TAIL) for tm, tn in big]
    return cands


def chain_supported(pc2: PackedConv | None, pc3: PackedConv, pc1n: PackedConv | None, residual: bool = True, cb: int = 0) -> bool:
    convs = [pc for pc in (pc2, pc3, pc1n) if pc is not None]
    if not all(pc.precision == 1 and pc.bias is not None and not pc.cin4 for pc in convs):
        return False
    one = lambda pc, cin, cout: (pc.cin, pc.cout, pc.kh, pc.kw, pc.stride, pc.pad) == (cin, cout, 1, 1, 1, 0)
    if pc1n is None:
        return pc2 is None and residual and not cb and one(pc3, 256, 1024)
    if cb:
        return pc2 is None and not residual and cb == 256 and one(pc3, 384, 512) and one(pc1n, 512, 128)
    if pc2 is not None:
        return ((pc2.cin, pc2.cout, pc2.kh, pc2.kw, pc2.stride, pc2.pad) == (64, 64, 3, 3, 1, 1) and residual
                and one(pc3, 64, 256) and (one(pc1n, 256, 64) or one(pc1n, 256, 128)))
    if residual:
        return ((one(pc3, 128, 512) and (one(pc1n, 512, 128) or one(pc1n, 512, 256)))
                or (one(pc3, 256, 1024) and one(pc1n, 1024, 256)))
    return one(pc3, 128, 256) and one(pc1n, 256, 64)



def _chain_desc(pc2, pc3, pc1n, t1, res, out, t1n, tile_m, flags, t1b, t1b_stride) -> N.ChainDesc:
    d = N.ChainDesc()
    d.t1, d.res, d.out = t1.ptr(), (res.ptr() if res is not None else None), out.ptr()
    d.t1n = t1n.ptr() if t1n is not None else None
    d.w2, d.ws2, d.b2 = map(N.ptr, _filter(pc2))
    d.w3, d.ws3, d.b3 = map(N.ptr, _filter(pc3))
    d.w1n, d.ws1n, d.b1n = map(N.ptr, _filter(pc1n))
    d.n, d.h, d.w, d.c, d.nout = t1.n, t1.h, t1.w, pc3.cin, pc3.cout
    d.cn = pc1n.cout if pc1n is not None else 0
    d.t1_ld, d.res_ld, d.out_ld = t1.ld, (res.ld if res is not None else 0), out.ld
    d.t1n_ld = t1n.ld if t1n is not None else 0
    d.tile_m, d.flags = tile_m, flags
    if t1b is not None:
        d.t1b, d.cb, d.t1b_ld, d.t1b_h, d.t1b_w, d.t1b_stride = t1b.ptr(), t1b.c, t1b.ld, t1b.h, t1b.w, t1b_stride
    return d


def bottleneck_chain(pc2: PackedConv | None, pc3: PackedConv, pc1n: PackedConv, t1: Act, res: Act | None,
                     out: Act | None = None, t1n: Act | None = None, tile_m: int = 0, out_even_only: bool = False,
                     t1b: Act | None = None, t1b_stride: int = 1):
    cb = t1b.c if t1b is not None else 0
    assert chain_supported(pc2, pc3, pc1n, res is not None, cb), "bottleneck_chain: unsupported shapes"
    assert t1.fmt == 1 and t1.c + cb == pc3.cin and (res is None or (res.fmt == 1 and res.c == pc3.cout))
    assert t1b is None or (t1b.fmt == 1 and t1b.n == t1.n and (t1.h - 1) * t1b_stride < t1b.h and (t1.w - 1) * t1b_stride < t1b.w)
    assert res is None or (t1.n, t1.h, t1.w) == (res.n, res.h, res.w)
    c, nout, cn = pc3.cin, pc3.cout, (pc1n.cout if pc1n is not None else 0)
    flags = N.CHAIN_OUT_EVEN_ONLY if (out_even_only and pc2 is not None and RangeMonitor.active is None) else 0
    via_op = T.ENABLED and out is None and t1n is None
    if not via_op:
        if out is None:
            out = Act.empty(t1.n, t1.h, t1.w, nout, t1.buf.device, 1)
        if t1n is None and pc1n is not None:
            t1n = Act.empty(t1.n, t1.h, t1.w, cn, t1.buf.device, 1)
        assert out.fmt == 1 and (out.n, out.h, out.w, out.c) == (t1.n, t1.h, t1.w, nout)
        assert pc1n is None or (t1n.fmt == 1 and (t1n.n, t1n.h, t1n.w, t1n.c) == (t1.n, t1.h, t1.w, cn))
    desc = lambda o, o1n: _chain_desc(pc2, pc3, pc1n, t1, res, o, o1n, tile_m, flags, t1b, t1b_stride)

    def go():
        if not via_op:
            _c_launch("fcp_bottleneck_chain_f16x3", C.byref(desc(out, t1n)))
            return out, t1n
        o, t = T.load().bottleneck_chain(t1.buf, t1.c0, None if res is None else res.buf, 0 if res is None else res.c0,
                                         *_filter(pc2), *_filter(pc3), *_filter(pc1n), c, nout, cn, tile_m, flags,
                                         None if t1b is None else t1b.buf, 0 if t1b is None else t1b.c0, cb, int(t1b_stride))
        return Act(o, fmt=1), (Act(t, fmt=1) if pc1n is not None else None)

    def describe():
        m = t1.n * t1.h * t1.w
        flops = ((pc2.flops_per_pixel if pc2 is not None else 0) + pc3.flops_per_pixel
                 + (pc1n.flops_per_pixel if pc1n is not None else 0)) * m
        byts = 4 * (m * (c + (nout if not flags else nout // 4) + (nout if res is not None else 0) + cn) + (0 if pc2 is None else 9 * c * c)
                    + c * nout + nout * cn)
        if pc1n is None:
            head = f"expand {c}->{nout} @{t1.h}x{t1.w}"
            return f"{head} +res", head, flops, byts
        head = f"chain {'3x3 ' if pc2 is not None else ''}{c}->{nout}->{cn} @{t1.h}x{t1.w}"
        return (f"{head}{' +res' if res is not None else ''}{' out@even' if flags else ''}{' two-source' if t1b is not None else ''}",
                head, flops, byts)

    def relaunch(o, o1n):
        o = _alias_safe_out(o, t1, res, t1b)
        o1n = o1n if o1n is None else _alias_safe_out(o1n, t1, res, t1b)
        return "fcp_bottleneck_chain_f16x3", (C.byref(desc(o, o1n)),), (pc2, pc3, pc1n, t1, res, o, o1n, t1b)
    return _accounted(go, describe, relaunch)


def u8_to_nhwc4(images_u8: torch.Tensor, sub=(0.0, 0.0, 0.0), div: float = 1.0) -> Act:
    assert images_u8.dtype == torch.uint8 and images_u8.dim() == 4 and images_u8.shape[3] == 3
    assert images_u8.is_contiguous()
    n, h, w, _ = images_u8.shape
    out = Act.empty(n, h, w, 4, images_u8.device)
    sub_arr = (C.c_float * 3)(*[float(s) for s in sub])
    N.check(N.lib().fcp_u8_to_nhwc4_f32(N.ptr(images_u8), out.ptr(), n * h * w, sub_arr, float(div),
                                        N.stream_ptr()), "fcp_u8_to_nhwc4_f32")
    return out


@dataclass
class PackedStem:
    wfrag: torch.Tensor
    bias: torch.Tensor
    wscale: torch.Tensor
    flops_per_pixel: int


def pack_stem_fused(weight, bn, device, cin_perm=None) -> PackedStem:
    if isinstance(weight, torch.Tensor):
        weight = weight.detach().cpu().numpy()
    bn = {k: (v.detach().cpu().numpy() if isinstance(v, torch.Tensor) else np.asarray(v)) for k, v in bn.items()}
    w, b = fold_bn(weight, bn, None)
    if cin_perm is not None:
        w = w[:, cin_perm]
    assert w.shape == (64, 3, 7, 7), "the fused stem is the ResNet 7x7 / 64-filter stem"
    wk = np.zeros((64, 22 * 8), np.float32)
    wk.reshape(64, 22, 8)
    for kh in range(7):
        wk[:, kh * 24:kh * 24 + 21] = w[:, :, kh, :].transpose(0, 2, 1).reshape(64, 21)
    amax = np.abs(wk).max(1)
    e = np.where(amax > 0, np.floor(np.log2(np.maximum(amax, 1e-38))), 0.0)
    scale = np.exp2(e).astype(np.float32)
    ws = wk / scale[:, None]
    hi = ws.astype(np.float16)
    lo = (ws - hi.astype(np.float32)).astype(np.float16)
    frag = np.zeros((2, 11, 2, 64, 8), np.float16)
    lane = np.arange(64)
    for ct in range(2):
        n = ct * 32 + (lane & 31)
        for q in range(11):
            ch = 2 * q + (lane >> 5)
            k = ch[:, None] * 8 + np.arange(8)[None, :]
            frag[ct, q, 0] = hi[n[:, None], k]
            frag[ct, q, 1] = lo[n[:, None], k]
    return PackedStem(torch.from_numpy(np.ascontiguousarray(frag.view(np.int16))).to(device),
                      torch.from_numpy(np.ascontiguousarray(b)).to(device), torch.from_numpy(scale).to(device),
                      2 * 64 * 3 * 49)


def stem_conv1_supported(pc1: PackedConv | None) -> bool:
    return (pc1 is not None and pc1.precision == 1 and pc1.bias is not None and not pc1.cin4
# ... 99 lines not shown
```

### face-crop-plus_amd/retinaface.py

```python
from __future__ import annotations


import os
import threading

import numpy as np
import torch

from . import _native as N
from . import engine as E
from . import torch_ops as T
from .weights import load_state_dict

STRATEGIES = {"all": 0, "best": 1, "largest": 2}


class RetinaFace:
    WEIGHTS_FILENAME = "retinaface_detector.pth"

    def __init__(self, strategy: str = "all", vis: float = 0.6):
        self.strategy = strategy
        self.vis_threshold = vis
        self.nms_threshold = 0.4
        self.variance = [0.1, 0.2]
        self.device = None
        self._p = None
        self.precision = 0
        self.fused_chain = True
        self.streams = int(os.environ.get("FCP_DET_STREAMS", "2"))
        self.min_images_per_stream = 6
        self._tls = threading.local()

    def load(self, device: str | torch.device = "cuda:0", weights=None, precision=None):
        device = torch.device(device)
        if device.type != "cuda":
            raise RuntimeError("face_crop_plus_amd runs on an AMD GPU only (device must be cuda:N / hip); "
                               "there is no CPU fallback")
        N.lib()
        self.device = device
        sd = load_state_dict("retinaface", weights, device=device)
        self._repack(sd, precision)
        E.device_props(device)
        E.selfcheck_at_load(self, sd, weights, precision, lambda: self._repack(sd, "f32"))
        return self

    def _repack(self, sd, precision):
        with torch.cuda.device(self.device), E.default_precision(precision):
            self._p = self._pack(sd, self.device)
        self.precision = E.resolve_precision(precision)

    @torch.no_grad()
    def selfcheck(self, sd=None, images_u8: torch.Tensor | None = None, rel_tol: float = 1e-4):
        if self.precision != 1:
            self.selfcheck_report = {"skipped": "exact-fp32 path: nothing to guard"}
            return self.selfcheck_report
        dev = self.device
        with torch.cuda.device(dev):
            if images_u8 is None:
                g = torch.Generator(device="cpu").manual_seed(20260928)
                s = 256
                ramp = (torch.arange(s)[:, None] + torch.arange(s)[None, :]).clamp(max=255).to(torch.uint8)
                images_u8 = torch.stack([torch.randint(0, 256, (s, s, 3), generator=g, dtype=torch.uint8),
                                         torch.full((s, s, 3), 255, dtype=torch.uint8), torch.zeros((s, s, 3), dtype=torch.uint8),
                                         ramp[..., None].expand(s, s, 3).contiguous()]).to(dev)
            images_u8 = images_u8.to(dev).contiguous()
            tuning, E.Autotune.enabled = E.Autotune.enabled, False
            try:
                with E.RangeMonitor() as mon:
                    heads = self.forward_heads(None, images_u8) if "stem_fused" in self._p else \
                        self.forward_heads(E.u8_to_nhwc4(images_u8, sub=(123.0, 117.0, 104.0)))
                rep = {"launch_absmax": mon.check("RetinaFace"), "limit": E.RangeMonitor.LIMIT, "head_rel_diff": None}
                if sd is not None:
                    twin = RetinaFace(self.strategy, self.vis_threshold)
                    twin.device, twin.precision = dev, 0
                    with E.default_precision("f32"):
                        twin._p = self._pack(sd, dev)
                    ref = twin.forward_heads(E.u8_to_nhwc4(images_u8, sub=(123.0, 117.0, 104.0)))
                    rep["head_rel_diff"] = [E.selfcheck_compare("RetinaFace head maps", a.buf, b.buf, rel_tol)
                                            for a, b in zip(heads, ref)]
                    del twin, ref
                    torch.cuda.empty_cache()
            finally:
                E.Autotune.enabled = tuning
        self.selfcheck_report = rep
        return rep

    @staticmethod
    def _pack(sd, dev):
        p = {}
        pc, bn = E.pack_conv, E.bn_of
        p["stem"] = pc(sd["body.conv1.weight"], None, bn(sd, "body.bn1"), 2, 3, dev, cin_perm=[2, 1, 0])
        if E.DEFAULT_PRECISION == 1:
            p["stem_fused"] = E.pack_stem_fused(sd["body.conv1.weight"], bn(sd, "body.bn1"), dev, cin_perm=[2, 1, 0])
        blocks = []
        for li, nb in enumerate((3, 4, 6, 3), 1):
            for b in range(nb):
                pre = f"body.layer{li}.{b}"
                stride = 2 if (b == 0 and li > 1) else 1
                blk = {
                    "c1": pc(sd[pre + ".conv1.weight"], None, bn(sd, pre + ".bn1"), 1, 0, dev),
                    "c2": pc(sd[pre + ".conv2.weight"], None, bn(sd, pre + ".bn2"), stride, 1, dev),
                    "c3": pc(sd[pre + ".conv3.weight"], None, bn(sd, pre + ".bn3"), 1, 0, dev),
                    "ds": None, "feat": (b == nb - 1 and li >= 2),
                }
                if (pre + ".downsample.0.weight") in sd:
                    blk["ds"] = pc(sd[pre + ".downsample.0.weight"], None, bn(sd, pre + ".downsample.1"),
                                   stride, 0, dev)
                    if stride == 1 or E.DEFAULT_PRECISION == 1:
                        fold = lambda cw, cb: E.fold_bn(sd[pre + cw].numpy(), {q: v.numpy() for q, v in bn(sd, pre + cb).items()}, None)
                        (w3, b3), (wd, bd) = fold(".conv3.weight", ".bn3"), fold(".downsample.0.weight", ".downsample.1")
                        blk["c3ds"] = pc(np.concatenate([w3, wd], 1), b3 + bd, None, 1, 0, dev)
                blocks.append(blk)
        p["blocks"] = blocks
        for i in (1, 2, 3):
            p[f"fpn.output{i}"] = pc(sd[f"fpn.output{i}.0.weight"], None, bn(sd, f"fpn.output{i}.1"), 1, 0, dev)
        for i in (1, 2):
            p[f"fpn.merge{i}"] = pc(sd[f"fpn.merge{i}.0.weight"], None, bn(sd, f"fpn.merge{i}.1"), 1, 1, dev)
        head_perm = list(range(0, 128)) + list(range(192, 256)) + list(range(128, 192))
        for k in (1, 2, 3):
            def folded(nm):
                return E.fold_bn(sd[f"ssh{k}.{nm}.0.weight"].numpy(), {q: v.numpy() for q, v in bn(sd, f"ssh{k}.{nm}.1").items()}, None)
            w_b, b_b = folded("conv5X5_1")
            w_a, b_a = folded("conv3X3")
            p[f"ssh{k}.ab"] = pc(np.concatenate([w_b, w_a]), np.concatenate([b_b, b_a]), None, 1, 1, dev)
            w_c, b_c = folded("conv5X5_2")
            w_d, b_d = folded("conv7X7_2")
            p[f"ssh{k}.cd"] = pc(np.concatenate([w_c, w_d]), np.concatenate([b_c, b_d]), None, 1, 1, dev)
            w_e, b_e = folded("conv7x7_3")
            p[f"ssh{k}.e"] = pc(w_e, b_e, None, 1, 1, dev)
            i = k - 1
            hw = np.concatenate([sd[f"{h}.{i}.conv1x1.weight"].numpy() for h in ("ClassHead", "BboxHead", "LandmarkHead")])
            hb = np.concatenate([sd[f"{h}.{i}.conv1x1.bias"].numpy() for h in ("ClassHead", "BboxHead", "LandmarkHead")])
            p[f"head{k}"] = pc(hw, hb, None, 1, 0, dev, cin_perm=head_perm)
        return p

    def forward_heads(self, x4: E.Act | None, images_u8: torch.Tensor | None = None, heads_out=None):
        p = self._p
        f = 1 if self.precision == 1 else 0
        stem_t1 = None
        if images_u8 is not None and "stem_fused" in p:
            n, h, w, _ = images_u8.shape
            hp, wp = ((h - 1) // 2) // 2 + 1, ((w - 1) // 2) // 2 + 1
            cat = E.Act.empty(n, hp, wp, 128, images_u8.device, f)
            c1 = p["blocks"][0]["c1"]
            if f == 1 and E.stem_conv1_supported(c1):
                x, stem_t1 = E.stem_relu_pool_u8(p["stem_fused"], images_u8, cat.slice(64, 64), conv1=c1)
            else:
                x = E.stem_relu_pool_u8(p["stem_fused"], images_u8, cat.slice(64, 64))
        else:
            x = E.conv(p["stem"], x4, act_slope=0.0, out_fmt=f)
            cat = E.Act.empty(x.n, (x.h + 1) // 2, (x.w + 1) // 2, 2 * x.c, x.buf.device, f)
            x = E.maxpool3x3s2(x, cat.slice(x.c, x.c))
        feats = []
        blocks, pre = p["blocks"], stem_t1
        chain = bool(f) and self.fused_chain
        for bi, blk in enumerate(blocks):
            o = pre if pre is not None else E.conv(blk["c1"], x, act_slope=0.0, out_fmt=f)
            pre = None
            nxt = blocks[bi + 1] if bi + 1 < len(blocks) else None
            if (chain and blk["ds"] is None and not blk["feat"] and nxt is not None
                    and E.chain_supported(blk["c2"], blk["c3"], nxt["c1"])):
                sparse = "c3ds" in nxt and nxt["c2"].stride == 2 and not blk["feat"]
                x, pre = E.bottleneck_chain(blk["c2"], blk["c3"], nxt["c1"], o, x, out_even_only=sparse)
                continue
            if "c3ds" in blk and blk["c2"].stride == 1:
                E.conv(blk["c2"], o, cat.slice(0, o.c), act_slope=0.0)
                if chain and nxt is not None and E.chain_supported(None, blk["c3ds"], nxt["c1"], residual=False):
                    x, pre = E.bottleneck_chain(None, blk["c3ds"], nxt["c1"], cat, None)
                else:
                    x = E.conv(blk["c3ds"], cat, act_slope=0.0, out_fmt=f)
                del cat
                continue
            if "c3ds" in blk:
                o = E.conv(blk["c2"], o, act_slope=0.0, out_fmt=f)
                if (chain and not blk["feat"] and nxt is not None
                        and E.chain_supported(None, blk["c3ds"], nxt["c1"], residual=False, cb=x.c)):
                    x, pre = E.bottleneck_chain(None, blk["c3ds"], nxt["c1"], o, None, t1b=x, t1b_stride=blk["c2"].stride)
                    continue
                x = E.conv(blk["c3ds"], o, act_slope=0.0, out_fmt=f, x2=x, x2_stride=blk["c2"].stride)
                if blk["feat"]:
                    feats.append(x)
                continue
            o = E.conv(blk["c2"], o, act_slope=0.0, out_fmt=f)
            if (chain and blk["ds"] is None and nxt is not None and E.chain_supported(None, blk["c3"], nxt["c1"])):
                x, pre = E.bottleneck_chain(None, blk["c3"], nxt["c1"], o, x)
                if blk["feat"]:
                    feats.append(x)
                continue
            idt = x if blk["ds"] is None else E.conv(blk["ds"], x, out_fmt=f)
            x = E.conv(blk["c3"], o, act_slope=0.0, res1=idt, res1_pre=True, out_fmt=f)
            if blk["feat"]:
                feats.append(x)
        if getattr(self, "_debug_feats", None) is not None:
            self._debug_feats.extend(feats)
        o3 = E.conv(p["fpn.output3"], feats[2], act_slope=0.0, out_fmt=f)
        o2 = E.conv(p["fpn.output2"], feats[1], act_slope=0.0, res1=o3, res1_pre=False, out_fmt=f)
        o2 = E.conv(p["fpn.merge2"], o2, act_slope=0.0, out_fmt=f)
        o1 = E.conv(p["fpn.output1"], feats[0], act_slope=0.0, res1=o2, res1_pre=False, out_fmt=f)
        o1 = E.conv(p["fpn.merge1"], o1, act_slope=0.0, out_fmt=f)
        heads = []
        for k, ft in zip((1, 2, 3), (o1, o2, o3)):
            s = E.Act.empty(ft.n, ft.h, ft.w, 384, ft.buf.device, f)
            E.conv(p[f"ssh{k}.ab"], ft, s.slice(0, 192), act_slope=0.0)
            E.conv(p[f"ssh{k}.cd"], s.slice(0, 64), s.slice(256, 128), act_slope=0.0)
            E.conv(p[f"ssh{k}.e"], s.slice(320, 64), s.slice(192, 64), act_slope=0.0)
            heads.append(E.conv(p[f"head{k}"], s.slice(64, 256),
                                None if heads_out is None else heads_out[k - 1]))
        return heads

    def _side_streams(self, dev, k):
        main = E.thread_streams(dev)["main"]
        return E.thread_side_streams(dev, k, with_main=main is not None and torch.cuda.current_stream(dev) == main)

    MAX_OPERAND_BYTES = 0xFFFFFFF0

    def _images_per_launch(self, h: int, w: int) -> int | None:
        if self.precision != 1:
            return None
        hp, wp = ((h - 1) // 2) // 2 + 1, ((w - 1) // 2) // 2 + 1
        return max(1, (self.MAX_OPERAND_BYTES - 1) // (4 * 256 * hp * wp))

    def _streams_for(self, n: int) -> int:
        k = min(self.streams, n // max(1, self.min_images_per_stream))
        return 1 if k < 2 or torch.cuda.is_current_stream_capturing() else k

    def _chunked(self, n: int, h: int, w: int, dev, run, split: bool = True):
        per = self._images_per_launch(h, w)
        q = 1
        while True:
            bounds = [n * i // q for i in range(q + 1)]
            sub = lambda c: -(-c // (self._streams_for(c) if split else 1))
            if per is None or all(sub(b - a) <= per for a, b in zip(bounds[:-1], bounds[1:])):
                break
            q += 1
        if q == 1:
            return run(0, n, None)
        heads = [E.Act.empty(n, -(-h // s), -(-w // s), 32, dev) for s in (8, 16, 32)]
        for a, b in zip(bounds[:-1], bounds[1:]):
            run(a, b, [E.Act(hd.buf[a:b]) for hd in heads])
        return heads

    def _forward_heads_split(self, images_u8: torch.Tensor, heads_out=None):
        n, h, w, _ = images_u8.shape
        k = self._streams_for(n)
        if k < 2:
            return self.forward_heads(None, images_u8, heads_out)
        dev = images_u8.device
        heads = heads_out if heads_out is not None else [E.Act.empty(n, -(-h // s), -(-w // s), 32, dev) for s in (8, 16, 32)]
        cur = torch.cuda.current_stream(dev)
        bounds = [n * i // k for i in range(k + 1)]
        side = self._side_streams(dev, k)
        cus = E.device_props(dev).multi_processor_count // k
        for st, a, b in zip(side, bounds[:-1], bounds[1:]):
            tuned = len(E.Autotune.cache)
            if st != cur:
                st.wait_stream(cur)
            with torch.cuda.stream(st), E.cu_budget(cus):
                self.forward_heads(None, images_u8[a:b], [E.Act(hd.buf[a:b]) for hd in heads])
            if len(E.Autotune.cache) != tuned:
                st.synchronize()
        for st in side:
            if st != cur:
                cur.wait_stream(st)
        return heads

    def detect(self, images_u8: torch.Tensor | None = None, *, x4: E.Act | None = None,
               paddings: torch.Tensor | None = None, max_faces: int | None = None, want_dense: bool = False):
        if self.strategy not in STRATEGIES:
            raise ValueError(f"Unsupported startegy: {self.strategy}")
        fused = x4 is None and "stem_fused" in self._p
        if x4 is None and not fused:
            x4 = E.u8_to_nhwc4(images_u8, sub=(123.0, 117.0, 104.0))
        if fused:
            images_u8 = images_u8.contiguous()
            (n, h, w), dev = images_u8.shape[:3], images_u8.device
            heads = self._chunked(n, h, w, dev, lambda a, b, ho: self._forward_heads_split(images_u8[a:b], ho))
        else:
            n, h, w = x4.n, x4.h, x4.w
            dev = x4.buf.device
            heads = self._chunked(n, h, w, dev, lambda a, b, ho: self.forward_heads(x4 if (a, b) == (0, n) else E.Act(x4.buf[a:b]),
                                                                                    None, ho), split=False)
        P = sum(2 * (-(-h // s)) * (-(-w // s)) for s in (8, 16, 32))
        f32, i32 = torch.float32, torch.int32
        cand_score = torch.empty((n, P), dtype=f32, device=dev)
        cand_box = torch.empty((n, P, 4), dtype=f32, device=dev)
        cand_ldm = torch.empty((n, P, 10), dtype=f32, device=dev)
        cand_prior = torch.empty((n, P), dtype=i32, device=dev)
        cand_count = torch.empty((n,), dtype=i32, device=dev)
        dense = (None, None, None)
        if want_dense:
            dense = (torch.empty((n, P), dtype=f32, device=dev), torch.empty((n, P, 4), dtype=f32, device=dev),
                     torch.empty((n, P, 10), dtype=f32, device=dev))
        if T.ENABLED and not want_dense:
            return self._postprocess_ops(heads, n, h, w, P, paddings, max_faces)
        st = N.stream_ptr()
        lib = N.lib()
        N.check(lib.fcp_retina_decode(heads[0].ptr(), heads[1].ptr(), heads[2].ptr(), n, h, w,
                                      float(self.vis_threshold), float(self.variance[0]), float(self.variance[1]),
                                      N.ptr(cand_score), N.ptr(cand_box), N.ptr(cand_ldm), N.ptr(cand_prior),
                                      N.ptr(cand_count), N.ptr(dense[0]), N.ptr(dense[1]), N.ptr(dense[2]), st),
                "fcp_retina_decode")
        out = nms_select(cand_score, cand_box, cand_count, self.nms_threshold, self.strategy)
        if max_faces is None:
            max_faces = n if self.strategy != "all" else int(out["sel_count"].sum().item())
        max_faces = max(int(max_faces), 1)
        landmarks = torch.empty((max_faces, 5, 2), dtype=f32, device=dev)
        img_idx = torch.empty((max_faces,), dtype=i32, device=dev)
        face_offset = torch.empty((n + 1,), dtype=i32, device=dev)
        if paddings is not None:
            paddings = paddings.to(device=dev, dtype=i32).contiguous()
        N.check(lib.fcp_retina_gather_faces(N.ptr(cand_ldm), N.ptr(out["sel_pos"]), N.ptr(out["sel_count"]), n, P,
                                            N.ptr(paddings), max_faces, N.ptr(face_offset), N.ptr(landmarks),
                                            N.ptr(img_idx), st), "fcp_retina_gather_faces")
        out.update(landmarks=landmarks, img_idx=img_idx, face_offset=face_offset, cand_score=cand_score,
                   cand_box=cand_box, cand_ldm=cand_ldm, cand_prior=cand_prior, cand_count=cand_count,
                   heads=heads, dense=dense, max_faces=max_faces)
        return out

    def _postprocess_ops(self, heads, n, h, w, P, paddings, max_faces):
        ops = T.load()
        dev = heads[0].buf.device
        cand_score, cand_box, cand_ldm, cand_prior, cand_count = ops.retina_decode(
            heads[0].buf, heads[1].buf, heads[2].buf, h, w, float(self.vis_threshold), float(self.variance[0]),
            float(self.variance[1]))
        keep_pos, keep_count, sel_pos, sel_count = ops.nms_select(cand_score, cand_box, cand_count, float(self.nms_threshold),
                                                                  STRATEGIES[self.strategy])
        if max_faces is None:
            max_faces = n if self.strategy != "all" else int(sel_count.sum().item())
        max_faces = max(int(max_faces), 1)
        if paddings is not None:
            paddings = paddings.to(device=dev, dtype=torch.int32).contiguous()
        landmarks, img_idx, face_offset = ops.gather_faces(cand_ldm, sel_pos, sel_count, paddings, max_faces)
        return dict(keep_pos=keep_pos, keep_count=keep_count, sel_pos=sel_pos, sel_count=sel_count, landmarks=landmarks,
                    img_idx=img_idx, face_offset=face_offset, cand_score=cand_score, cand_box=cand_box, cand_ldm=cand_ldm,
                    cand_prior=cand_prior, cand_count=cand_count, heads=heads, dense=(None, None, None), max_faces=max_faces)

    def graphed(self, n: int, h: int, w: int, paddings: torch.Tensor | None = None):
        if self.strategy == "all":
            raise ValueError('graph capture needs a bounded face count: strategy "best" or "largest"')
        key = (n, h, w, None if paddings is None else tuple(paddings.flatten().tolist()))
        cache = self.__dict__.setdefault("_graphs", {})
        if key in cache:
            return cache[key]
        with torch.cuda.device(self.device):
            static = torch.zeros((n, h, w, 3), dtype=torch.uint8, device=self.device)
            prev, E.Autotune.enabled = E.Autotune.enabled, True
            side = torch.cuda.Stream(device=self.device)
            side.wait_stream(torch.cuda.current_stream())
            with torch.cuda.stream(side):
                for _ in range(2):
                    self.detect(static, paddings=paddings, max_faces=n)
            torch.cuda.current_stream().wait_stream(side)
            E.Autotune.enabled = False
            graph = torch.cuda.CUDAGraph()
            with torch.cuda.graph(graph):
                res = self.detect(static, paddings=paddings, max_faces=n)
            E.Autotune.enabled = prev
        cache[key] = (static, res, graph)
        return cache[key]

    @torch.no_grad()
# ... 32 lines not shown
```

### include/fcp_hip.h

```cpp
#ifndef FCP_HIP_H
#define FCP_HIP_H

#include <stdint.h>

#ifdef __cplusplus
extern "C" {
#endif

#define FCP_ABI_VERSION 15

typedef void* fcp_stream_t;

int fcp_abi_version(void);
const char* fcp_last_error(void);

typedef struct fcp_conv_desc {
  const float* in;
  const void* w;
  const float* bias;
  float* out;
  const float* res1;
  const float* res2;
  const float* wscale;
  const float* in2;
  int32_t n, in_h, in_w;
  int32_t cin, in_ld;
  int32_t in_up2;
  int32_t cout, kh, kw, stride, pad;
  int32_t out_h, out_w, out_ld;
  int32_t tile_n;
  int32_t cin4;
  float act_slope, alpha, alpha2;
  int32_t res1_pre, res1_ld, res1_h, res1_w, res2_ld;
  int32_t precision;
  int32_t in_fmt, out_fmt, res1_fmt, res2_fmt;
  int32_t tile_m;
  int32_t cin2, in2_ld, in2_h, in2_w, in2_stride;
  int32_t flags;
  int32_t cu_budget;
  int32_t band_top, band_bottom;
} fcp_conv_desc;

#define FCP_CONV_FLAT_ADDR 1
#define FCP_CONV_BALANCE_TAIL 2

int fcp_conv2d_nhwc_f32(const fcp_conv_desc* desc, fcp_stream_t stream);

typedef struct fcp_chain_desc {
  const float* t1;
  const void* w2;  const float* ws2;  const float* b2;
  const void* w3;  const float* ws3;  const float* b3;
  const float* res;
  float* out;
  const void* w1n; const float* ws1n; const float* b1n;
  float* t1n;
  const float* t1b;
  int32_t n, h, w, c, cn;
  int32_t t1_ld, res_ld, out_ld, t1n_ld;
  int32_t nout;
  int32_t tile_m;
  int32_t flags;
  int32_t cb, t1b_ld, t1b_h, t1b_w, t1b_stride;
} fcp_chain_desc;
#define FCP_CHAIN_OUT_EVEN_ONLY 1

int fcp_bottleneck_chain_f16x3(const fcp_chain_desc* desc, fcp_stream_t stream);

int fcp_u8_to_nhwc4_f32(const uint8_t* in, float* out, int64_t npix,
                        const float* sub_host, float div, fcp_stream_t stream);

int fcp_f32nchw_to_nhwc4_f32(const float* in, float* out, int n, int h, int w,
                             const float* sub_host, float div, fcp_stream_t stream);

int fcp_maxpool3x3s2_nhwc_f32(const float* in, float* out, int n, int h, int w, int c, int out_ld,
                              int out_h, int out_w, fcp_stream_t stream);
int fcp_maxpool3x3s2_split32(const float* in, float* out, int n, int h, int w, int c, int out_ld,
                             int out_h, int out_w, fcp_stream_t stream);
int fcp_stem7x7s2_relu_pool_u8(const uint8_t* images, int n, int h, int w, const int32_t* mean_rgb,
                               const void* wfrag, const float* bias, const float* wscale, float* out,
                               int out_ld, int out_fmt, fcp_stream_t stream);
int fcp_stem7x7s2_relu_pool_conv1_u8(const uint8_t* images, int n, int h, int w, const int32_t* mean_rgb,
                                     const void* wfrag, const float* bias, const float* wscale, float* out,
                                     int out_ld, int out_fmt, const void* w1, const float* ws1, const float* b1,
                                     float* t1, int t1_ld, fcp_stream_t stream);
int fcp_stem7x7s2_relu_pool_f32(const float* x4, int n, int h, int w, const void* wfrag, const float* bias,
                                const float* wscale, float* out, int out_ld, int out_fmt, fcp_stream_t stream);
int fcp_f32_to_split32(const float* in, float* out, int64_t npix, int c, fcp_stream_t stream);
int fcp_split32_to_f32(const float* in, float* out, int64_t npix, int c, fcp_stream_t stream);
int fcp_absmax_nhwc(const float* x, int64_t npix, int c, int ld, int fmt, float* out_max, fcp_stream_t stream);


int fcp_retina_decode(const float* head0, const float* head1, const float* head2,
                      int n, int img_h, int img_w, float vis_threshold,
                      float var0, float var1,
                      float* cand_score, float* cand_box, float* cand_ldm,
                      int32_t* cand_prior, int32_t* cand_count,
                      float* dense_score, float* dense_box, float* dense_ldm,
                      fcp_stream_t stream);

int64_t fcp_retina_nms_workspace_bytes(int n, int cap);
int fcp_retina_nms_select(const float* cand_score, const float* cand_box,
                          const int32_t* cand_count, int n, int cap,
                          float nms_threshold, int strategy, void* workspace,
                          int32_t* keep_pos, int32_t* keep_count,
                          int32_t* sel_pos, int32_t* sel_count, fcp_stream_t stream);

int fcp_retina_gather_faces(const float* cand_ldm, const int32_t* sel_pos,
                            const int32_t* sel_count, int n, int cap,
                            const int32_t* paddings, int max_faces,
                            int32_t* face_offset, float* out_ldm, int32_t* out_img,
                            fcp_stream_t stream);


int fcp_estimate_transform(const float* src, const float* dst, int f, int k,
                           int allow_skew, double* mat, int32_t* ok, fcp_stream_t stream);

int fcp_estimate_transform_counted(const float* src, const float* dst, int f, int k,
                                   int allow_skew, const int32_t* face_count,
                                   double* mat, int32_t* ok, int64_t* valid_total,
                                   fcp_stream_t stream);

int fcp_warp_affine_u8(const uint8_t* images, int n, int h, int w,
                       const int32_t* img_idx, const double* mat, const int32_t* ok,
                       const int32_t* paddings, int f, int out_h, int out_w, int border,
                       uint8_t* out, fcp_stream_t stream);

int fcp_warp_affine_u8_float(const uint8_t* images, int n, int h, int w,
                             const int32_t* img_idx, const double* mat, const int32_t* ok,
                             const int32_t* paddings, int f, int out_h, int out_w, int border,
                             uint8_t* out, fcp_stream_t stream);

typedef struct fcp_warp_src {
  int64_t off;
  int32_t h, w;
} fcp_warp_src;

int fcp_warp_affine_u8_ragged(const uint8_t* blob, int64_t blob_bytes,
                              const fcp_warp_src* srcs_host, const fcp_warp_src* srcs_dev,
                              const double* mat, const int32_t* ok, int f, int out_h, int out_w,
                              int border, uint8_t* out, fcp_stream_t stream);
int fcp_warp_affine_u8_float_ragged(const uint8_t* blob, int64_t blob_bytes,
                                    const fcp_warp_src* srcs_host, const fcp_warp_src* srcs_dev,
                                    const double* mat, const int32_t* ok, int f, int out_h,
                                    int out_w, int border, uint8_t* out, fcp_stream_t stream);

int fcp_warp_affine_u8_interp(const uint8_t* images, int n, int h, int w,
                              const int32_t* img_idx, const double* mat, const int32_t* ok,
                              const int32_t* paddings, int f, int out_h, int out_w, int border,
                              int interp, uint8_t* out, fcp_stream_t stream);
int fcp_warp_affine_u8_interp_ragged(const uint8_t* blob, int64_t blob_bytes,
                                     const fcp_warp_src* srcs_host, const fcp_warp_src* srcs_dev,
                                     const double* mat, const int32_t* ok, int f, int out_h,
                                     int out_w, int border, int interp, uint8_t* out,
                                     fcp_stream_t stream);

int fcp_warp_interp_weights(int interp, int16_t* out);

int fcp_crop_sharpness_u8(const uint8_t* crops, int f, int h, int w, const int32_t* ok,
                          int64_t* sums, fcp_stream_t stream);

int64_t fcp_jpeg_workspace_bytes(int f, int h, int w, int channels);
int fcp_jpeg_encode_u8(const uint8_t* crops, int f, int h, int w, int channels, int quality, int subsampling,
                       uint8_t* out, int64_t out_stride, int64_t capacity, int32_t* lengths,
                       void* workspace, int64_t workspace_bytes, fcp_stream_t stream);

int64_t fcp_jpeg_workspace_bytes_ex(int f, int h, int w, int channels, int subsampling, int optimize);
int fcp_jpeg_encode_ex_u8(const uint8_t* crops, int f, int h, int w, int channels, int quality,
                          int subsampling, int optimize,
                          uint8_t* out, int64_t out_stride, int64_t capacity, int32_t* lengths,
                          uint8_t* tables, void* workspace, int64_t workspace_bytes, fcp_stream_t stream);

int fcp_jpeg_huffman_tables(const uint32_t* freq, int n, uint8_t* tables, uint32_t* codes, fcp_stream_t stream);

int64_t fcp_png_workspace_bytes(int f, int h, int w, int channels);
int fcp_png_encode_u8(const uint8_t* pixels, int f, int h, int w, int channels,
                      uint8_t* out, int64_t out_stride, int64_t capacity, int32_t* lengths,
                      void* workspace, int64_t workspace_bytes, fcp_stream_t stream);

int fcp_png_huffman_lengths(const uint32_t* freq, int n, uint8_t* lengths, uint32_t* codes, fcp_stream_t stream);

int fcp_matte_u8(const uint8_t* crops, const uint8_t* labels, int f, int h, int w, uint32_t class_bits, int feather,
                 int bg_r, int bg_g, int bg_b, uint8_t* out, uint8_t* alpha, fcp_stream_t stream);

int64_t fcp_matte_blur_workspace_bytes(int f, int h, int w);
int fcp_matte_blur_u8(const uint8_t* crops, const uint8_t* labels, int f, int h, int w, uint32_t class_bits, int feather,
                      const uint16_t* taps, int radius, uint8_t* out, uint8_t* alpha, void* workspace, int64_t workspace_bytes,
                      fcp_stream_t stream);

int64_t fcp_matte_refine_workspace_bytes(int f, int h, int w);
int fcp_matte_refine_u8(const uint8_t* crops, const uint8_t* labels, int f, int h, int w, uint32_t class_bits, int radius, int eps,
                        uint8_t* alpha_out, void* workspace, int64_t workspace_bytes, fcp_stream_t stream);

int fcp_matte_alpha_u8(const uint8_t* crops, const uint8_t* alpha, int f, int h, int w, int bg_r, int bg_g, int bg_b, uint8_t* out,
                       fcp_stream_t stream);
int fcp_matte_blur_alpha_u8(const uint8_t* crops, const uint8_t* labels, const uint8_t* alpha, int f, int h, int w,
                            uint32_t class_bits, const uint16_t* taps, int radius, uint8_t* out, void* workspace,
                            int64_t workspace_bytes, fcp_stream_t stream);

#define FCP_CUTOUT_RGBA 0
#define FCP_CUTOUT_FILL 1
// ... 84 lines not shown
```

Baseline: 1457 faces/s.

## Fuse RetinaFace 1x1 head convs into SSH conv epilogues as accumulated tails

Adds a 'tail' mode to the fp16x3 conv kernels. Each output tile is staged in LDS and a 1x1 head conv (cout 32) is run on it with MFMA, writing or accumulating into a shared fp32 head map. The SSH detector branches now fold the head computation into the ab, cd and e convs. This removes the separate head launch and avoids writing and re-reading some intermediate SSH activations. The cost is extra epilogue work, barriers and LDS pressure per tile, prefetch is serialized after the tail in the persistent kernel, and the head is split into partial sums with a new fallback path.

Result: no change. 1460 faces/s (median of 5 runs) (+0.2%).

```diff
diff --git a/face-crop-plus_amd/_native.py b/face-crop-plus_amd/_native.py
--- a/face-crop-plus_amd/_native.py
+++ b/face-crop-plus_amd/_native.py
@@ -31,6 +31,12 @@
     ]
 
 
+class ConvTail(C.Structure):
+    _fields_ = [("w", C.c_void_p), ("wscale", C.c_void_p), ("bias", C.c_void_p), ("map", C.c_void_p),
+                ("c0", C.c_int32), ("kt", C.c_int32), ("map_ld", C.c_int32), ("accumulate", C.c_int32),
+                ("write_out", C.c_int32)]
+
+
 CONV_FLAT_ADDR = 1
 CONV_BALANCE_TAIL = 2
 CHAIN_OUT_EVEN_ONLY = 1
@@ -46,6 +52,7 @@
 _P, _I, _F, _L = C.c_void_p, C.c_int, C.c_float, C.c_int64
 SIGNATURES = {
     "fcp_conv2d_nhwc_f32": [C.POINTER(ConvDesc), _P],
+    "fcp_conv2d_tail_f16x3": [C.POINTER(ConvDesc), C.POINTER(ConvTail), _P],
     "fcp_bottleneck_chain_f16x3": [C.POINTER(ChainDesc), _P],
     "fcp_u8_to_nhwc4_f32": [_P, _P, _L, C.POINTER(C.c_float), _F, _P],
     "fcp_f32nchw_to_nhwc4_f32": [_P, _P, _I, _I, _I, C.POINTER(C.c_float), _F, _P],
diff --git a/face-crop-plus_amd/csrc/fcp_conv.hip b/face-crop-plus_amd/csrc/fcp_conv.hip
--- a/face-crop-plus_amd/csrc/fcp_conv.hip
+++ b/face-crop-plus_amd/csrc/fcp_conv.hip
@@ -167,9 +167,24 @@
 
 }
 
-extern "C" int fcp_conv2d_nhwc_f32(const fcp_conv_desc* d, fcp_stream_t stream) {
+static int conv_entry(const fcp_conv_desc* d, const fcp_conv_tail* t, fcp_stream_t stream) {
   FCP_REQUIRE(d != nullptr, "conv: null descriptor");
-  FCP_REQUIRE(d->in && d->w && d->out, "conv: null tensor pointer");
+  ConvTail tl = {};
+  if (t != nullptr) {
+    FCP_REQUIRE(d->precision == 1 && d->in_fmt == 1 && d->out_fmt == 1 && !d->cin4,
+                "conv(tail): needs the fp16x3 path with split32 input and output");
+    FCP_REQUIRE(t->w && t->wscale && t->map && (t->kt == 64 || t->kt == 128) && t->c0 >= 0 && t->c0 % 32 == 0 && t->c0 + t->kt <= d->cout,
+                "conv(tail): needs filter, wscale and map, kt 64 | 128, a 32-aligned channel range within cout");
+    FCP_REQUIRE((((uintptr_t)t->w | (uintptr_t)t->wscale | (uintptr_t)t->bias | (uintptr_t)t->map) & 15) == 0 && t->map_ld % 4 == 0 && t->map_ld >= 32,
+                "conv(tail): filter, wscale, bias and map must be 16-byte aligned, map_ld %% 4 == 0, map_ld >= 32");
+    FCP_REQUIRE(d->out || (!t->write_out && t->c0 == 0 && t->kt == d->cout), "conv(tail): null output tensor");
+    tl.w = reinterpret_cast<const float*>(t->w); tl.wscale = t->wscale; tl.bias = t->bias; tl.map = t->map;
+    tl.c0 = t->c0; tl.kt = t->kt; tl.map_ld = t->map_ld; tl.accumulate = t->accumulate != 0; tl.write = t->write_out != 0;
+  } else {
+    FCP_REQUIRE(d->out, "conv: null tensor pointer");
+  }
+  const ConvTail* tlp = t != nullptr ? &tl : nullptr;
+  FCP_REQUIRE(d->in && d->w, "conv: null tensor pointer");
   FCP_REQUIRE(d->n > 0 && d->in_h > 0 && d->in_w > 0 && d->cout > 0, "conv: bad sizes");
   const bool big = d->tile_m == 256, halo = d->tile_m == 1;
   FCP_REQUIRE(d->tile_m == 0 || d->tile_m == 128 || big || halo, "conv: tile_m must be 0/128/256 (or 1: halo-tile 3x3)");
@@ -296,13 +311,13 @@
                   "conv(halo): wscale / bias must be 16-byte aligned");
       k.in2_bytes = (unsigned)out_bytes;
       k.w_bytes = (unsigned)((unsigned long)fcp_cdiv(d->cout, 128) * 128ul * k.wrow * 4ul);
-      return halo_wide ? launch_f16x3_halo_wide(k, s) : launch_f16x3_halo(k, s);
+      return halo_wide ? launch_f16x3_halo_wide(k, s, tlp) : launch_f16x3_halo(k, s, tlp);
     }
     if (big) {
       k.w_bytes = (unsigned)((unsigned long)fcp_cdiv(d->cout, 128) * 128ul * k.wrow * 4ul);
-      return launch_f16x3_big(k, d->tile_n, s);
-    }
-    if (k.in_fmt == 1 && !d->cin4) return launch_f16x3_dma(k, d->tile_n, s);
+      return launch_f16x3_big(k, d->tile_n, s, tlp);
+    }
+    if (k.in_fmt == 1 && !d->cin4) return launch_f16x3_dma(k, d->tile_n, s, tlp);
     return launch_f16x3(k, d->tile_n, d->cin4 != 0, s);
   }
   k.in_bytes = buf ? (unsigned)in_bytes : 0u;
@@ -319,3 +334,10 @@
   }
 #undef FCP_DISPATCH
 }
+
+extern "C" int fcp_conv2d_nhwc_f32(const fcp_conv_desc* d, fcp_stream_t stream) { return conv_entry(d, nullptr, stream); }
+
+extern "C" int fcp_conv2d_tail_f16x3(const fcp_conv_desc* d, const fcp_conv_tail* tail, fcp_stream_t stream) {
+  FCP_REQUIRE(tail != nullptr, "conv(tail): null tail descriptor");
+  return conv_entry(d, tail, stream);
+}
diff --git a/face-crop-plus_amd/csrc/fcp_conv_common.h b/face-crop-plus_amd/csrc/fcp_conv_common.h
--- a/face-crop-plus_amd/csrc/fcp_conv_common.h
+++ b/face-crop-plus_amd/csrc/fcp_conv_common.h
@@ -440,6 +440,87 @@
 }
 
 
+struct ConvTail {
+  const float* w;
+  const float* wscale;
+  const float* bias;
+  float* map;
+  int c0, kt;
+  int map_ld;
+  int accumulate;
+  int write;
+};
+
+struct NoTail {};
+template <bool TAIL> using TailArg = std::conditional_t<TAIL, ConvTail, NoTail>;
+
+__device__ __forceinline__ void lds_write128u(unsigned addr, const u32x4_t& v) { asm volatile("ds_write_b128 %0, %1" ::"v"(addr), "v"(v) : "memory"); }
+
+__device__ __forceinline__ void tail_put(unsigned img, int rows, int row, int tc, const u32x4_t& hi, const u32x4_t& lo) {
+  const unsigned base = img + (unsigned)(((tc >> 5) * rows + row) * 128);
+  const int ch = (tc & 31) >> 3, sw = swz(row);
+  lds_write128u(base + (unsigned)((ch ^ sw) << 4), hi);
+  lds_write128u(base + (unsigned)(((4 + ch) ^ sw) << 4), lo);
+}
+
+__device__ __forceinline__ void tail_slice(f32x16& acc, const ConvTail& t, int slice, unsigned arow, int lane, const int (&offH)[2], const int (&offL)[2]) {
+  const char* wr = reinterpret_cast<const char*>(t.w) + (long)(lane & 31) * t.kt * 4 + slice * 128 + (lane >> 5) * 16;
+  f16x8 bh[2], bl[2], ah[2], al[2];
+#pragma unroll
+  for (int s = 0; s < 2; ++s) {
+    bh[s] = *reinterpret_cast<const f16x8*>(wr + 32 * s);
+    bl[s] = *reinterpret_cast<const f16x8*>(wr + 64 + 32 * s);
+    ah[s] = lds_read128i<0>(arow + (unsigned)offH[s]);
+    al[s] = lds_read128i<0>(arow + (unsigned)offL[s]);
+  }
+  asm volatile("s_waitcnt lgkmcnt(0)" ::: "memory");
+  __builtin_amdgcn_sched_barrier(0);
+#pragma unroll
+  for (int s = 0; s < 2; ++s) {
+    acc = __builtin_amdgcn_mfma_f32_32x32x16_f16(bh[s], al[s], acc, 0, 0, 0);
+    acc = __builtin_amdgcn_mfma_f32_32x32x16_f16(bl[s], ah[s], acc, 0, 0, 0);
+    acc = __builtin_amdgcn_mfma_f32_32x32x16_f16(bh[s], ah[s], acc, 0, 0, 0);
+  }
+  __builtin_amdgcn_sched_barrier(0);
+}
+
+__device__ __forceinline__ void tail_out(const ConvTail& t, const f32x16& acc, long pix, int lane) {
+  if (pix < 0) return;
+  float* dst = t.map + pix * t.map_ld + 4 * (lane >> 5);
+#pragma unroll
+  for (int q = 0; q < 4; ++q) {
+    const f32x4 ws = *reinterpret_cast<const f32x4*>(t.wscale + 8 * q + 4 * (lane >> 5));
+    f32x4 b = {0.f, 0.f, 0.f, 0.f}, v;
+    if (t.bias != nullptr) b = *reinterpret_cast<const f32x4*>(t.bias + 8 * q + 4 * (lane >> 5));
+#pragma unroll
+    for (int e = 0; e < 4; ++e) v[e] = conv_scale_bias(acc[4 * q + e], ws[e], b[e]);
+    if (t.accumulate) {
+      const f32x4 o = *reinterpret_cast<const f32x4*>(dst + 8 * q);
+#pragma unroll
+      for (int e = 0; e < 4; ++e) v[e] = o[e] + v[e];
+    }
+    *reinterpret_cast<f32x4*>(dst + 8 * q) = v;
+  }
+}
+
+template <int NW>
+__device__ __forceinline__ void tail_tile(const ConvTail& t, unsigned img, int wave_u, int lane, int m_start, int m_end) {
+  asm volatile("s_waitcnt lgkmcnt(0)" ::: "memory");
+  __builtin_amdgcn_s_barrier();
+  __builtin_amdgcn_sched_barrier(0);
+  int offH[2], offL[2];
+  frag_offsets(lane, offH, offL);
+  f32x16 acc;
+#pragma unroll
+  for (int e = 0; e < 16; ++e) acc[e] = 0.f;
+  const int row = wave_u * 32 + (lane & 31);
+  for (int s = 0; s < (t.kt >> 5); ++s) tail_slice(acc, t, s, img + (unsigned)((s * (NW * 32) + row) * 128), lane, offH, offL);
+  __builtin_amdgcn_s_barrier();
+  __builtin_amdgcn_sched_barrier(0);
+  const int m = m_start + row;
+  tail_out(t, acc, m < m_end ? (long)m : -1L, lane);
+}
+
 template <int I, int N, typename F>
 __device__ __forceinline__ void fcp_static_for(F&& f) {
   if constexpr (I < N) {
@@ -448,9 +529,10 @@
   }
 }
 
-template <int TM, int TN, int WTM, int WTN>
+template <int TM, int TN, int WTM, int WTN, bool TAIL = false, int IMG_ROWS = 0>
 __device__ __forceinline__ void conv_epilogue_regs(const ConvK& p, f32x16 (&acc)[TM][TN], int m_start, int m_end, int tm_act, int co_tile,
-                                                   int co_end, int wm, int wn, int lane, int hw) {
+                                                   int co_end, int wm, int wn, int lane, int hw, const ConvTail& tl = ConvTail{},
+                                                   unsigned img = 0u) {
     const int lp = lane & 15, lg = lane >> 4;
   auto swap32 = [](float& x, float& y) {
     const auto r = __builtin_amdgcn_permlane32_swap(__float_as_uint(x), __float_as_uint(y), false, false);
@@ -477,7 +559,15 @@
         fcp_static_for<0, 2>([&](auto sc) {
           constexpr int set = decltype(sc)::value;
           const int mi = row_of(i, set);
-          if (i < tm_act && mi < m_end && co < co_end) store8(p.out, mi, p.out_ld, co, p.out_fmt, 0, pend_a[i - i0][set], pend_b[i - i0][set]);
+          bool wr = true;
+          if constexpr (TAIL) {
+            const int tc = co - tl.c0;
+            if ((unsigned)tc < (unsigned)tl.kt) {
+              tail_put(img, IMG_ROWS, mi - m_start, tc, pend_a[i - i0][set], pend_b[i - i0][set]);
+              wr = tl.write != 0;
+            }
+          }
+          if (wr && i < tm_act && mi < m_end && co < co_end) store8(p.out, mi, p.out_ld, co, p.out_fmt, 0, pend_a[i - i0][set], pend_b[i - i0][set]);
         });
       }
     });
@@ -598,9 +688,9 @@
 }
 
 int launch_f16x3(const ConvK& k, int tile_n, bool cin4, hipStream_t s);
-int launch_f16x3_dma(const ConvK& k, int tile_n, hipStream_t s);
-int launch_f16x3_halo(const ConvK& k, hipStream_t s);
-int launch_f16x3_halo_wide(const ConvK& k, hipStream_t s);
-int launch_f16x3_big(const ConvK& k, int tile_n, hipStream_t s);
-
-}
+int launch_f16x3_dma(const ConvK& k, int tile_n, hipStream_t s, const ConvTail* tl = nullptr);
+int launch_f16x3_halo(const ConvK& k, hipStream_t s, const ConvTail* tl = nullptr);
+int launch_f16x3_halo_wide(const ConvK& k, hipStream_t s, const ConvTail* tl = nullptr);
+int launch_f16x3_big(const ConvK& k, int tile_n, hipStream_t s, const ConvTail* tl = nullptr);
+
+}
diff --git a/face-crop-plus_amd/csrc/fcp_conv_f16x3_big.hip b/face-crop-plus_amd/csrc/fcp_conv_f16x3_big.hip
--- a/face-crop-plus_amd/csrc/fcp_conv_f16x3_big.hip
+++ b/face-crop-plus_amd/csrc/fcp_conv_f16x3_big.hip
@@ -11,8 +11,8 @@
 constexpr int ROWB = 128;
 constexpr int STAGE = 1 << 16;
 
-template <int BN>
-__global__ void __launch_bounds__(NT, 1) conv_igemm_f16x3_big(const ConvK p) {
+template <int BN, bool TAIL = false>
+__global__ void __launch_bounds__(NT, 1) conv_igemm_f16x3_big(const ConvK p, const TailArg<TAIL> tl) {
   constexpr int WAVES_N = BN == 256 ? 4 : 2;
   constexpr int WAVES_M = 8 / WAVES_N;
   constexpr int WTM = BMB / WAVES_M, WTN = BN / WAVES_N;
@@ -203,18 +203,34 @@
     vb += p.round_size;
     decode(vb);
     setup_tile();
-    prefetch_tile();
-  }
-  conv_epilogue_regs<TM, TN, WTM, WTN>(p, acc, e_m_start, e_m_end, e_tm_act, e_tile_n * BN,
-                                       (e_tile_n + 1) * BN < p.cout ? (e_tile_n + 1) * BN : p.cout, wm, wn, lane, hw);
+    if constexpr (!TAIL) prefetch_tile();
+  }
+  if constexpr (TAIL) {
+    conv_epilogue_regs<TM, TN, WTM, WTN, true, BMB>(p, acc, e_m_start, e_m_end, e_tm_act, e_tile_n * BN,
+                                                    (e_tile_n + 1) * BN < p.cout ? (e_tile_n + 1) * BN : p.cout, wm, wn, lane, hw, tl, lds0);
+    if (e_tile_n == tl.c0 / BN) tail_tile<8>(tl, lds0, wave_u, lane, e_m_start, e_m_end);
+    if (more) prefetch_tile();
+  } else {
+    conv_epilogue_regs<TM, TN, WTM, WTN>(p, acc, e_m_start, e_m_end, e_tm_act, e_tile_n * BN,
+                                         (e_tile_n + 1) * BN < p.cout ? (e_tile_n + 1) * BN : p.cout, wm, wn, lane, hw);
+  }
   if (!more) break;
   }
 }
 
+
 template <int BN>
-int launch(ConvK k, hipStream_t s) {
+int launch(ConvK k, const ConvTail* tl, hipStream_t s) {
   const size_t lds = 2 * (size_t)STAGE;
-  FCP_LDS_OPT_IN((&conv_igemm_f16x3_big<BN>), lds);
+  if (tl != nullptr) {
+    FCP_REQUIRE(k.out_fmt == 1, "conv(tail): the 256-row kernel hosts the tail on a split32 output");
+    FCP_REQUIRE(tl->c0 / BN == (tl->c0 + tl->kt - 1) / BN, "conv(tail): the tail's channels must lie in one N tile of the 256-row kernel (tile_n %d)", BN);
+    FCP_REQUIRE((size_t)(tl->kt / 32) * BMB * ROWB <= lds, "conv(tail): the operand image does not fit the 256-row kernel's LDS");
+    if constexpr (BN == 256) FCP_REQUIRE(false, "conv(tail): the 256 x 256 tile does not host a tail (use tile_n 128 / 192)");
+    else FCP_LDS_OPT_IN((&conv_igemm_f16x3_big<BN, true>), lds);
+  } else {
+    FCP_LDS_OPT_IN((&conv_igemm_f16x3_big<BN>), lds);
+  }
   k.grid_n = fcp_cdiv(k.cout, BN);
   int cus = k.cu_budget > 0 ? k.cu_budget : fcp_cu_count();
   cus = cus < 8 ? 8 : (cus & ~7);
@@ -242,7 +258,10 @@
   k.big_tiles = k.grid_m * k.grid_n;
   static const int persist_env = getenv("FCP_BIG_PERSIST") ? atoi(getenv("FCP_BIG_PERSIST")) : -1;
   k.big_persist = persist_env < 0 ? (k.cu_budget == 0) : (persist_env != 0);
-  hipLaunchKernelGGL((conv_igemm_f16x3_big<BN>), dim3(k.big_persist && k.big_tiles > k.round_size ? k.round_size : k.big_tiles), dim3(NT), lds, s, k);
+  const dim3 grid(k.big_persist && k.big_tiles > k.round_size ? k.round_size : k.big_tiles);
+  if (tl != nullptr) {
+    if constexpr (BN != 256) hipLaunchKernelGGL((conv_igemm_f16x3_big<BN, true>), grid, dim3(NT), lds, s, k, *tl);
+  } else hipLaunchKernelGGL((conv_igemm_f16x3_big<BN>), grid, dim3(NT), lds, s, k, NoTail{});
   FCP_LAUNCH_OK();
   return 0;
 }
@@ -251,8 +270,8 @@
 
 namespace fcp_conv {
 
-int launch_f16x3_big(const ConvK& k, int tile_n, hipStream_t s) {
-  return tile_n == 256 ? launch<256>(k, s) : tile_n == 192 ? launch<192>(k, s) : launch<128>(k, s);
-}
-
-}
+int launch_f16x3_big(const ConvK& k, int tile_n, hipStream_t s, const ConvTail* tl) {
+  return tile_n == 256 ? launch<256>(k, tl, s) : tile_n == 192 ? launch<192>(k, tl, s) : launch<128>(k, tl, s);
+}
+
+}
diff --git a/face-crop-plus_amd/csrc/fcp_conv_f16x3_dma.hip b/face-crop-plus_amd/csrc/fcp_conv_f16x3_dma.hip
--- a/face-crop-plus_amd/csrc/fcp_conv_f16x3_dma.hip
+++ b/face-crop-plus_amd/csrc/fcp_conv_f16x3_dma.hip
@@ -6,8 +6,8 @@
 
 constexpr int NST = 2;
 
-template <int BN, bool EP8>
-__global__ void __launch_bounds__(256, (BN == 128 ? 2 : 3)) conv_igemm_f16x3_dma(const ConvK p) {
+template <int BN, bool EP8, bool TAIL = false>
+__global__ void __launch_bounds__(256, (BN == 128 ? 2 : 3)) conv_igemm_f16x3_dma(const ConvK p, const TailArg<TAIL> tl) {
   constexpr int WAVES_N = (BN == 32) ? 1 : 2;
   constexpr int WAVES_M = 4 / WAVES_N;
   constexpr int WTM = BM / WAVES_M;
@@ -121,8 +121,15 @@
 
   if constexpr (EP8) {
     const int m_end = (tile_m + 1) * BM < p.M ? (tile_m + 1) * BM : p.M;
-    conv_epilogue_regs<TM, TN, WTM, WTN>(p, acc, tile_m * BM, m_end, TM, tile_n * BN, (tile_n + 1) * BN < p.cout ? (tile_n + 1) * BN : p.cout,
-                                         wm, wn, lane, hw);
+    if constexpr (TAIL) {
+      const unsigned img = (unsigned)(size_t)(__attribute__((address_space(3))) char*)lds;
+      conv_epilogue_regs<TM, TN, WTM, WTN, true, BM>(p, acc, tile_m * BM, m_end, TM, tile_n * BN, (tile_n + 1) * BN < p.cout ? (tile_n + 1) * BN : p.cout,
+                                                     wm, wn, lane, hw, tl, img);
+      if (tile_n == tl.c0 / BN) tail_tile<4>(tl, img, wave_u, lane, tile_m * BM, m_end);
+    } else {
+      conv_epilogue_regs<TM, TN, WTM, WTN>(p, acc, tile_m * BM, m_end, TM, tile_n * BN, (tile_n + 1) * BN < p.cout ? (tile_n + 1) * BN : p.cout,
+                                           wm, wn, lane, hw);
+    }
   } else {
     conv_epilogue<BN, TM, TN, WTM, WTN>(p, acc, smem, tile_m, tile_n, tid, lane, wm, wn, hw);
   }
@@ -134,12 +141,22 @@
   const size_t epi = EP8 ? 0 : (size_t)BM * BN * 4;
   if (lds < epi) lds = epi;
   FCP_LDS_OPT_IN((&conv_igemm_f16x3_dma<BN, EP8>), lds);
-  hipLaunchKernelGGL((conv_igemm_f16x3_dma<BN, EP8>), dim3(k.grid_m * k.grid_n), dim3(256), lds, s, k);
+  hipLaunchKernelGGL((conv_igemm_f16x3_dma<BN, EP8>), dim3(k.grid_m * k.grid_n), dim3(256), lds, s, k, NoTail{});
   FCP_LAUNCH_OK();
   return 0;
 }
 template <int BN>
-int launch(const ConvK& k, hipStream_t s) {
+int launch(const ConvK& k, const ConvTail* tl, hipStream_t s) {
+  if (tl != nullptr) {
+    const size_t lds = (size_t)NST * (BM + BN) * 128;
+    FCP_REQUIRE(k.out_fmt == 1, "conv(tail): the 128-row kernel hosts the tail on a split32 output");
+    FCP_REQUIRE(tl->c0 / BN == (tl->c0 + tl->kt - 1) / BN, "conv(tail): the tail's channels must lie in one N tile of the 128-row kernel (tile_n %d)", BN);
+    FCP_REQUIRE((size_t)(tl->kt / 32) * BM * 128 <= lds, "conv(tail): the operand image does not fit the 128-row kernel's LDS");
+    FCP_LDS_OPT_IN((&conv_igemm_f16x3_dma<BN, true, true>), lds);
+    hipLaunchKernelGGL((conv_igemm_f16x3_dma<BN, true, true>), dim3(k.grid_m * k.grid_n), dim3(256), lds, s, k, *tl);
+    FCP_LAUNCH_OK();
+    return 0;
+  }
   const bool ep8 = (k.out_fmt | k.res1_fmt | k.res2_fmt) != 0;
   return ep8 ? launch_ep<BN, true>(k, s) : launch_ep<BN, false>(k, s);
 }
@@ -148,11 +165,11 @@
 
 namespace fcp_conv {
 
-int launch_f16x3_dma(const ConvK& k, int tile_n, hipStream_t s) {
+int launch_f16x3_dma(const ConvK& k, int tile_n, hipStream_t s, const ConvTail* tl) {
   switch (tile_n) {
-    case 32: return launch<32>(k, s);
-    case 64: return launch<64>(k, s);
-    default: return launch<128>(k, s);
+    case 32: return launch<32>(k, tl, s);
+    case 64: return launch<64>(k, tl, s);
+    default: return launch<128>(k, tl, s);
   }
 }
 
diff --git a/face-crop-plus_amd/csrc/fcp_conv_f16x3_halo.hip b/face-crop-plus_amd/csrc/fcp_conv_f16x3_halo.hip
--- a/face-crop-plus_amd/csrc/fcp_conv_f16x3_halo.hip
+++ b/face-crop-plus_amd/csrc/fcp_conv_f16x3_halo.hip
@@ -60,8 +60,26 @@
   }
 }
 
-template <int TN>
-__global__ void __launch_bounds__(512, 1) conv3x3_halo_f16x3(const ConvK p) {
+__device__ __forceinline__ void halo_tail_mfma(f32x16 (&tacc)[2], const ConvTail& tl, int slice, unsigned cs0, int lane) {
+  asm volatile("" : "+v"(lane), "+v"(cs0));
+  int offH[2], offL[2];
+  frag_offsets(lane, offH, offL);
+#pragma unroll
+  for (int i = 0; i < 2; ++i) tail_slice(tacc[i], tl, slice, cs0 + (unsigned)((i * 32 + (lane & 31)) * 128), lane, offH, offL);
+}
+__device__ __forceinline__ void halo_tail_out(const f32x16 (&tacc)[2], const ConvTail& tl, const ConvK& p, int wave_u, int lane, int ni, int y0, int x0) {
+  asm volatile("" : "+v"(lane));
+#pragma unroll
+  for (int i = 0; i < 2; ++i) {
+    const int row = wave_u * 64 + i * 32 + (lane & 31);
+    const int y = y0 + (row >> 5), x = x0 + (row & 31);
+    tail_out(tl, tacc[i], y < p.out_h && x < p.out_w ? ((long)ni * p.out_h + y) * p.out_w + x : -1L, lane);
+  }
+}
+
+
+template <int TN, bool TAIL = false>
+__global__ void __launch_bounds__(512, 1) conv3x3_halo_f16x3(const ConvK p, const TailArg<TAIL> tl) {
   extern __shared__ __attribute__((aligned(16))) float smem[];
   char* lds = reinterpret_cast<char*>(smem);
   const unsigned lds0 = (unsigned)(size_t)(__attribute__((address_space(3))) char*)lds;
@@ -236,10 +254,17 @@
   auto epilogue = [&](int stage) {
     const unsigned cs0 = lds0 + (unsigned)(stage * A_BYTES + wave_u * 64 * 128);
     const int eq = lane & 3, er = lane >> 2;
+    f32x16 tacc[2];
+    if constexpr (TAIL) {
+#pragma unroll
+      for (int e = 0; e < 16; ++e) tacc[0][e] = tacc[1][e] = 0.f;
+    }
 #pragma unroll
     for (int n = 0; n < TN; ++n) {
       const int ccol = n * 32 + eq * 8;
       const bool cvalid = ccol < p.cout;
+      bool tin = false;
+      if constexpr (TAIL) tin = (unsigned)(n * 32 - tl.c0) < (unsigned)tl.kt;
       f32x4 b8[2], w8[2];
       halo_epi_consts(p, ccol, cvalid, b8, w8);
 #pragma unroll
@@ -284,12 +309,23 @@
             o0 = (unsigned)((m * p.out_ld + ccol) * 4);
             o1 = o0 + 16u;
           }
-          __builtin_amdgcn_raw_buffer_store_b128(s0, rs_out, ok ? o0 : 0xFFFFFFFFu, 0, 0);
-          __builtin_amdgcn_raw_buffer_store_b128(s1, rs_out, ok ? o1 : 0xFFFFFFFFu, 0, 0);
+          bool okw = ok;
+          if constexpr (TAIL) {
+            if (tin) {
+              tail_put(cs0, 64, row & 63, eq * 8, s0, s1);
+              okw = ok && tl.write != 0;
+            }
+          }
+          __builtin_amdgcn_raw_buffer_store_b128(s0, rs_out, okw ? o0 : 0xFFFFFFFFu, 0, 0);
+          __builtin_amdgcn_raw_buffer_store_b128(s1, rs_out, okw ? o1 : 0xFFFFFFFFu, 0, 0);
         }
       }
       __builtin_amdgcn_sched_barrier(0);
-    }
+      if constexpr (TAIL) {
+        if (tin) halo_tail_mfma(tacc, tl, (n * 32 - tl.c0) >> 5, cs0, lane);
+      }
+    }
+    if constexpr (TAIL) halo_tail_out(tacc, tl, p, wave_u, lane, e_ni, e_y0, e_x0);
     __builtin_amdgcn_s_barrier();
     __builtin_amdgcn_sched_barrier(0);
   };
@@ -337,8 +373,8 @@
 }
 
 
-template <int TN, bool RES, int BT, int RS>
-__global__ void __launch_bounds__(512, 1) conv3x3_halo_wide_f16x3(const ConvK p) {
+template <int TN, bool RES, int BT, int RS, bool TAIL = false>
+__global__ void __launch_bounds__(512, 1) conv3x3_halo_wide_f16x3(const ConvK p, const TailArg<TAIL> tl) {
   constexpr int TAPB = TN * 32 * ROWB;
   constexpr int PRE = RS - BT;
   constexpr bool SLACK2 = (RS - BT - 1) / BT >= 2;
@@ -552,22 +588,31 @@
     int e_ni, e_y0, e_x0;
     ts.coords(ts.tile(it), e_ni, e_y0, e_x0);
     const unsigned cs0 = lds0 + (unsigned)(A_BYTES + wave_u * 64 * 128);
-    const int eq = lane & 3, er = lane >> 2;
+    int el = lane;
+    if constexpr (TAIL) asm volatile("" : "+v"(el));
+    const int eq = el & 3, er = el >> 2, exl = TAIL ? el & 31 : xl, ehalf = TAIL ? el >> 5 : half;
     asm volatile("s_waitcnt lgkmcnt(0)" ::: "memory");
+    f32x16 tacc[2];
+    if constexpr (TAIL) {
+#pragma unroll
+      for (int e = 0; e < 16; ++e) tacc[0][e] = tacc[1][e] = 0.f;
+    }
 #pragma unroll
     for (int n = 0; n < TN; ++n) {
       asm volatile("" ::: "memory");
       __builtin_amdgcn_sched_barrier(0);
       const int ccol = n * 32 + eq * 8;
       const bool cvalid = ccol < p.cout;
+      bool tin = false;
+      if constexpr (TAIL) tin = (unsigned)(n * 32 - tl.c0) < (unsigned)tl.kt;
       f32x4 b8[2], w8[2];
       halo_epi_consts(p, ccol, cvalid, b8, w8);
 #pragma unroll
       for (int i = 0; i < 2; ++i)
 #pragma unroll
         for (int rr = 0; rr < 16; ++rr) {
-          const int row = i * 32 + mfma_c_row(rr, half);
-          lds_write32(cs0 + (unsigned)((row * 32 + xl) * 4), acc[n][i][rr]);
+          const int row = i * 32 + mfma_c_row(rr, ehalf);
+          lds_write32(cs0 + (unsigned)((row * 32 + exl) * 4), acc[n][i][rr]);
         }
       __builtin_amdgcn_sched_barrier(0);
 #pragma unroll
@@ -611,12 +656,23 @@
             o0 = (unsigned)((m * p.out_ld + ccol) * 4);
             o1 = o0 + 16u;
           }
-          __builtin_amdgcn_raw_buffer_store_b128(s0, rs_out, ok ? o0 : 0xFFFFFFFFu, 0, 0);
-          __builtin_amdgcn_raw_buffer_store_b128(s1, rs_out, ok ? o1 : 0xFFFFFFFFu, 0, 0);
+          bool okw = ok;
+          if constexpr (TAIL) {
+            if (tin) {
+              tail_put(cs0, 64, row & 63, eq * 8, s0, s1);
+              okw = ok && tl.write != 0;
+            }
+          }
+          __builtin_amdgcn_raw_buffer_store_b128(s0, rs_out, okw ? o0 : 0xFFFFFFFFu, 0, 0);
+          __builtin_amdgcn_raw_buffer_store_b128(s1, rs_out, okw ? o1 : 0xFFFFFFFFu, 0, 0);
         }
       }
       __builtin_amdgcn_sched_barrier(0);
-    }
+      if constexpr (TAIL) {
+        if (tin) halo_tail_mfma(tacc, tl, (n * 32 - tl.c0) >> 5, cs0, el);
+      }
+    }
+    if constexpr (TAIL) halo_tail_out(tacc, tl, p, wave_u, el, e_ni, e_y0, e_x0);
     __builtin_amdgcn_s_barrier();
     __builtin_amdgcn_sched_barrier(0);
   };
@@ -662,16 +718,25 @@
   return 0;
 }
 
-int launch_f16x3_halo(const ConvK& k, hipStream_t s) {
+static int halo_tail_ok(const ConvK& k, const ConvTail& tl) {
+  FCP_REQUIRE(k.out_fmt == 1 && tl.c0 + tl.kt <= k.cout, "conv(tail): the halo kernels host the tail on a split32 output, channels within cout");
+  return 0;
+}
+
+int launch_f16x3_halo(const ConvK& k, hipStream_t s, const ConvTail* tl) {
   const size_t lds = (size_t)LDS_TOTAL;
   unsigned grid = 0;
   if (const int e = halo_grid(k, &grid)) return e;
-  if (k.cout <= 32) {
+  if (tl != nullptr) {
+    if (const int e = halo_tail_ok(k, *tl)) return e;
+    FCP_LDS_OPT_IN((&conv3x3_halo_f16x3<2, true>), lds);
+    hipLaunchKernelGGL((conv3x3_halo_f16x3<2, true>), dim3(grid), dim3(512), lds, s, k, *tl);
+  } else if (k.cout <= 32) {
     FCP_LDS_OPT_IN(&conv3x3_halo_f16x3<1>, lds);
-    hipLaunchKernelGGL(conv3x3_halo_f16x3<1>, dim3(grid), dim3(512), lds, s, k);
+    hipLaunchKernelGGL(conv3x3_halo_f16x3<1>, dim3(grid), dim3(512), lds, s, k, NoTail{});
   } else {
     FCP_LDS_OPT_IN(&conv3x3_halo_f16x3<2>, lds);
-    hipLaunchKernelGGL(conv3x3_halo_f16x3<2>, dim3(grid), dim3(512), lds, s, k);
+    hipLaunchKernelGGL(conv3x3_halo_f16x3<2>, dim3(grid), dim3(512), lds, s, k, NoTail{});
   }
   FCP_LAUNCH_OK();
   return 0;
@@ -679,19 +744,28 @@
 
 constexpr int WIDE2_BT = 2;
 
-int launch_f16x3_halo_wide(const ConvK& k, hipStream_t s) {
+int launch_f16x3_halo_wide(const ConvK& k, hipStream_t s, const ConvTail* tl) {
   const int tn = k.cout <= 64 ? 2 : 4;
   const size_t lds = (size_t)(2 * A_BYTES + (tn == 2 ? 8 : 4) * tn * 32 * ROWB);
   unsigned grid = 0;
   if (const int e = halo_grid(k, &grid)) return e;
   FCP_REQUIRE(k.ctiles >= 2 && k.ctiles % 2 == 0 && k.cout <= 128, "conv(halo, wide): cin must be a multiple of 64, cout <= 128");
   FCP_REQUIRE(tn == 2 || (k.res1 == nullptr && k.res2 == nullptr), "conv(halo, wide): no residual inputs with more than 64 filters");
-  if (tn == 2) {
+  if (tl != nullptr) {
+    if (const int e = halo_tail_ok(k, *tl)) return e;
+    if (tn == 2) {
+      FCP_LDS_OPT_IN((&conv3x3_halo_wide_f16x3<2, true, WIDE2_BT, 8, true>), lds);
+      hipLaunchKernelGGL((conv3x3_halo_wide_f16x3<2, true, WIDE2_BT, 8, true>), dim3(grid), dim3(512), lds, s, k, *tl);
+    } else {
+      FCP_LDS_OPT_IN((&conv3x3_halo_wide_f16x3<4, false, 1, 4, true>), lds);
+      hipLaunchKernelGGL((conv3x3_halo_wide_f16x3<4, false, 1, 4, true>), dim3(grid), dim3(512), lds, s, k, *tl);
+    }
+  } else if (tn == 2) {
     FCP_LDS_OPT_IN((&conv3x3_halo_wide_f16x3<2, true, WIDE2_BT, 8>), lds);
-    hipLaunchKernelGGL((conv3x3_halo_wide_f16x3<2, true, WIDE2_BT, 8>), dim3(grid), dim3(512), lds, s, k);
+    hipLaunchKernelGGL((conv3x3_halo_wide_f16x3<2, true, WIDE2_BT, 8>), dim3(grid), dim3(512), lds, s, k, NoTail{});
   } else {
     FCP_LDS_OPT_IN((&conv3x3_halo_wide_f16x3<4, false, 1, 4>), lds);
-    hipLaunchKernelGGL((conv3x3_halo_wide_f16x3<4, false, 1, 4>), dim3(grid), dim3(512), lds, s, k);
+    hipLaunchKernelGGL((conv3x3_halo_wide_f16x3<4, false, 1, 4>), dim3(grid), dim3(512), lds, s, k, NoTail{});
   }
   FCP_LAUNCH_OK();
   return 0;
diff --git a/face-crop-plus_amd/engine.py b/face-crop-plus_amd/engine.py
--- a/face-crop-plus_amd/engine.py
+++ b/face-crop-plus_amd/engine.py
@@ -564,6 +564,47 @@
     return outs
 
 
+@dataclass
+class HeadTail:
+    pc: PackedConv
+    c0: int
+    map: Act
+    accumulate: bool = False
+    write: bool = False
+
+
+TAIL_REFUSED = object()
+
+
+def tail_hostable(tm: int, tn: int, cout: int, tail: HeadTail) -> bool:
+    c0, kt = tail.c0, tail.pc.cin
+    if tm == 1:
+        return cout > 32 and c0 + kt <= cout
+    one_tile = c0 // tn == (c0 + kt - 1) // tn
+    if tm == 256:
+        return tn in (128, 192) and one_tile
+    return one_tile and (kt // 32) * 128 * 128 <= 2 * (128 + tn) * 128
+
+
+def _tail_desc(tail: HeadTail, map_: Act) -> N.ConvTail:
+    t = N.ConvTail()
+    t.w, t.wscale, t.map = N.ptr(tail.pc.w), N.ptr(tail.pc.wscale), map_.ptr()
+    t.bias = None if tail.accumulate else N.ptr(tail.pc.bias)
+    t.c0, t.kt, t.map_ld = tail.c0, tail.pc.cin, map_.ld
+    t.accumulate, t.write_out = int(tail.accumulate), int(tail.write)
+    return t
+
+
+class _NoOut:
+    fmt, c0, buf = 1, 0, None
+
+    def __init__(self, n, h, w, c):
+        self.n, self.h, self.w, self.c, self.ld = n, h, w, c, c
+
+    def ptr(self):
+        return None
+
+
 def _conv_desc(pc: PackedConv, x: Act, out: Act, x2, x2_stride, res1, res1_pre, res2, alpha, alpha2, act_slope, in_up2, band,
                tile_m, tile_n, flags, cu_budget) -> N.ConvDesc:
     in_h, in_w = (x.h * 2, x.w * 2) if in_up2 else (x.h, x.w)
@@ -602,14 +643,24 @@
          res2: Act | None = None, alpha2: float = 1.0, in_up2: bool = False,
          tile_n: int | None = None, out_fmt: int = 0, tile_m: int | None = None,
          x2: Act | None = None, x2_stride: int = 1, flat: bool = False, balance_tail: bool = False,
-         band: tuple[int, int] = (0, 0)) -> Act:
+         band: tuple[int, int] = (0, 0), tail: HeadTail | None = None) -> Act:
     assert x.c + (x2.c if x2 is not None else 0) == pc.cin, f"conv expects {pc.cin} input channels, got {x.c}"
     in_h, in_w = (x.h * 2, x.w * 2) if in_up2 else (x.h, x.w)
     oh = (in_h - band[0] - band[1] + 2 * pc.pad - pc.kh) // pc.stride + 1
     ow = (in_w + 2 * pc.pad - pc.kw) // pc.stride + 1
-    if out is None:
-        out = Act.empty(x.n, oh, ow, pc.cout, x.buf.device, out_fmt)
-    assert (out.n, out.h, out.w, out.c) == (x.n, oh, ow, pc.cout), "conv: bad output view"
+    no_out = tail is not None and not tail.write and tail.c0 == 0 and tail.pc.cin == pc.cout
+    if tail is not None:
+        assert pc.precision == 1 and tail.pc.precision == 1 and tail.pc.cout == 32 and tail.pc.cin in (64, 128) and x.fmt == 1
+        assert (tail.pc.kh, tail.pc.kw, tail.pc.stride, tail.pc.pad) == (1, 1, 1, 0) and tail.c0 % 32 == 0 and tail.c0 + tail.pc.cin <= pc.cout
+        assert tail.map.fmt == 0 and (tail.map.n, tail.map.h, tail.map.w, tail.map.c) == (x.n, oh, ow, 32)
+        assert res1 is None and res2 is None and x2 is None
+    if no_out:
+        out = _NoOut(x.n, oh, ow, pc.cout)
+    elif out is None:
+        out = Act.empty(x.n, oh, ow, pc.cout, x.buf.device, 1 if tail is not None else out_fmt)
+    out_c = tail.c0 if (tail is not None and not tail.write and not no_out and tail.c0 + tail.pc.cin == pc.cout) else pc.cout
+    assert (out.n, out.h, out.w, out.c) == (x.n, oh, ow, out_c), "conv: bad output view"
+    assert tail is None or out.fmt == 1
     if (x.fmt or out.fmt or (res1 is not None and res1.fmt) or (res2 is not None and res2.fmt)) and pc.precision != 1:
         raise ValueError("split32 tensors can only be used with filters packed for the fp16x3 path")
     assert x2 is None or (x2.fmt == 1 and x.fmt == 1 and x2.n == x.n), "two-source convs take split32 tensors"
@@ -630,13 +681,20 @@
     if tile_n is None and tile_m is None and (pc.cout > 64 or halo_ok):
         key = (pc.cin, pc.cout, pc.kh, pc.kw, pc.stride, m, int(in_up2), res1 is not None, res2 is not None,
                pc.precision, x.fmt, out.fmt, None if x2 is None else (x2.c, x2_stride), cu)
-        best = Autotune.choose(key, tile_candidates(pc.cout, halo_ok, wide_ok, big_ok),
-                               lambda: desc(_alias_safe_out(out, x, x2, res1, res2)))
+        trial_out = lambda: (Act.empty(x.n, oh, ow, pc.cout, x.buf.device, 1) if (no_out or (tail is not None and not tail.write))
+                             else _alias_safe_out(out, x, x2, res1, res2))
+        best = Autotune.choose(key, tile_candidates(pc.cout, halo_ok, wide_ok, big_ok), lambda: desc(trial_out()))
         if best is not None:
             tm, tn = best[0], best[1]
             flags |= best[2] if len(best) > 2 else 0
 
+    if tail is not None and not tail_hostable(tm, tn, pc.cout, tail):
+        return TAIL_REFUSED
+
     def go():
+        if tail is not None:
+            _c_launch("fcp_conv2d_tail_f16x3", C.byref(desc(out)), C.byref(_tail_desc(tail, tail.map)))
+            return (None if no_out else out,)
         if T.ENABLED:
             T.load().conv2d_out(x.buf, x.c0, pc.cin, pc.w, pc.bias, pc.wscale, None if res1 is None else res1.buf,
                                 0 if res1 is None else res1.c0, None if res2 is None else res2.buf, 0 if res2 is None else res2.c0,
@@ -654,13 +712,30 @@
                     + x.n * in_h * in_w * x.c // (4 if in_up2 else 1) + (m * x2.c if x2 is not None else 0)
                     + pc.cout * pc.cin * pc.kh * pc.kw)
         head = f"conv {pc.kh}x{pc.kw} s{pc.stride} {pc.cin}->{pc.cout} @{oh}x{ow}"
-        return (f"{head} tile {tm}x{tn}{' bal' if flags & N.CONV_BALANCE_TAIL else ''}{' +res' if res1 is not None else ''}",
-                head, pc.flops_per_pixel * m, byts)
+        flops, tl = pc.flops_per_pixel * m, ""
+        if tail is not None:
+            kt = tail.pc.cin
+            flops += tail.pc.flops_per_pixel * m
+            byts += 4 * (m * (32 * (2 if tail.accumulate else 1) - (0 if tail.write else kt)) + 32 * kt)
+            tl = f" +head{kt}@{tail.c0}{'+' if tail.accumulate else '='}{'w' if tail.write else ''}"
+        return (f"{head} tile {tm}x{tn}{' bal' if flags & N.CONV_BALANCE_TAIL else ''}{' +res' if res1 is not None else ''}{tl}",
+                head, flops, byts)
 
     def relaunch(o):
+        if tail is not None:
+            mp = Act.empty(x.n, oh, ow, 32, x.buf.device) if tail.accumulate else tail.map
+            o = out if no_out else o
+            return "fcp_conv2d_tail_f16x3", (C.byref(desc(o)), C.byref(_tail_desc(tail, mp))), (pc, tail, x, o, mp)
         o = _alias_safe_out(o, x, x2, res1, res2)
         return "fcp_conv2d_nhwc_f32", (C.byref(desc(o)),), (pc, x, x2, res1, res2, o)
     return _accounted(go, describe, relaunch)[0]
+
+
+_conv_entry = conv
+
+
+def conv_tapped() -> bool:
+    return conv is not _conv_entry
 
 
 def tile_candidates(cout: int, halo_ok: bool, wide_ok: bool, big_ok: bool):
diff --git a/face-crop-plus_amd/retinaface.py b/face-crop-plus_amd/retinaface.py
--- a/face-crop-plus_amd/retinaface.py
+++ b/face-crop-plus_amd/retinaface.py
@@ -27,6 +27,7 @@
         self._p = None
         self.precision = 0
         self.fused_chain = True
+        self.fused_heads = True
         self.streams = int(os.environ.get("FCP_DET_STREAMS", "2"))
         self.min_images_per_stream = 6
         self._tls = threading.local()
@@ -132,6 +133,10 @@
             hw = np.concatenate([sd[f"{h}.{i}.conv1x1.weight"].numpy() for h in ("ClassHead", "BboxHead", "LandmarkHead")])
             hb = np.concatenate([sd[f"{h}.{i}.conv1x1.bias"].numpy() for h in ("ClassHead", "BboxHead", "LandmarkHead")])
             p[f"head{k}"] = pc(hw, hb, None, 1, 0, dev, cin_perm=head_perm)
+            if E.DEFAULT_PRECISION == 1:
+                p[f"head{k}.A"] = pc(hw[:, 0:128], hb, None, 1, 0, dev)
+                p[f"head{k}.C"] = pc(hw[:, 128:192], None, None, 1, 0, dev)
+                p[f"head{k}.E"] = pc(hw[:, 192:256], None, None, 1, 0, dev)
         return p
 
     def forward_heads(self, x4: E.Act | None, images_u8: torch.Tensor | None = None, heads_out=None):
@@ -198,6 +203,10 @@
         o2 = E.conv(p["fpn.merge2"], o2, act_slope=0.0, out_fmt=f)
         o1 = E.conv(p["fpn.output1"], feats[0], act_slope=0.0, res1=o2, res1_pre=False, out_fmt=f)
         o1 = E.conv(p["fpn.merge1"], o1, act_slope=0.0, out_fmt=f)
+        if (self.fused_heads and f == 1 and "head1.A" in p and E.RangeMonitor.active is None
+                and getattr(self, "_debug_feats", None) is None and not E.conv_tapped()):
+            return [self._ssh_heads_fused(k, ft, None if heads_out is None else heads_out[k - 1])
+                    for k, ft in zip((1, 2, 3), (o1, o2, o3))]
         heads = []
         for k, ft in zip((1, 2, 3), (o1, o2, o3)):
             s = E.Act.empty(ft.n, ft.h, ft.w, 384, ft.buf.device, f)
@@ -207,6 +216,25 @@
             heads.append(E.conv(p[f"head{k}"], s.slice(64, 256),
                                 None if heads_out is None else heads_out[k - 1]))
         return heads
+
+    def _ssh_heads_fused(self, k: int, ft: E.Act, hmap: E.Act | None) -> E.Act:
+        p, dev = self._p, ft.buf.device
+        hA, hC, hE = (p[f"head{k}.{q}"] for q in "ACE")
+        if hmap is None:
+            hmap = E.Act.empty(ft.n, ft.h, ft.w, 32, dev)
+        bd = E.Act.empty(ft.n, ft.h, ft.w, 128, dev, 1)
+        b = bd.slice(0, 64)
+        if E.conv(p[f"ssh{k}.ab"], ft, b, act_slope=0.0, tail=E.HeadTail(hA, 64, hmap)) is E.TAIL_REFUSED:
+            ba = E.conv(p[f"ssh{k}.ab"], ft, act_slope=0.0, out_fmt=1)
+            b = ba.slice(0, 64)
+            E.conv(hA, ba.slice(64, 128), hmap)
+        if E.conv(p[f"ssh{k}.cd"], b, bd, act_slope=0.0, tail=E.HeadTail(hC, 0, hmap, accumulate=True)) is E.TAIL_REFUSED:
+            bd = E.conv(p[f"ssh{k}.cd"], b, act_slope=0.0, out_fmt=1)
+            E.conv(hC, bd.slice(0, 64), hmap, res1=hmap, res1_pre=False)
+        d = bd.slice(64, 64)
+        if E.conv(p[f"ssh{k}.e"], d, act_slope=0.0, tail=E.HeadTail(hE, 0, hmap, accumulate=True)) is E.TAIL_REFUSED:
+            E.conv(hE, E.conv(p[f"ssh{k}.e"], d, act_slope=0.0, out_fmt=1), hmap, res1=hmap, res1_pre=False)
+        return hmap
 
     def _side_streams(self, dev, k):
         main = E.thread_streams(dev)["main"]
diff --git a/include/fcp_hip.h b/include/fcp_hip.h
--- a/include/fcp_hip.h
+++ b/include/fcp_hip.h
@@ -46,6 +46,19 @@
 
 int fcp_conv2d_nhwc_f32(const fcp_conv_desc* desc, fcp_stream_t stream);
 
+typedef struct fcp_conv_tail {
+  const void* w;
+  const float* wscale;
+  const float* bias;
+  float* map;
+  int32_t c0, kt;
+  int32_t map_ld;
+  int32_t accumulate;
+  int32_t write_out;
+} fcp_conv_tail;
+
+int fcp_conv2d_tail_f16x3(const fcp_conv_desc* desc, const fcp_conv_tail* tail, fcp_stream_t stream);
+
 typedef struct fcp_chain_desc {
   const float* t1;
   const void* w2;  const float* ws2;  const float* b2;
```
